# Aleksoid1978/VideoRenderer

Hardware: AMD Instinct MI355X
Metric: 4K frames/sec/GPU (P010->Lanczos3 2x->PQ-SDR->dither); % HBM roofline (higher is better)
Workload: dtype f32 (u16 in, u8 out)

## Files before the change

### include/mpcvr.h

```cpp
#ifndef MPCVR_H
#define MPCVR_H

#include <stddef.h>
#include <stdint.h>

#ifdef __cplusplus
extern "C" {
#endif

#define MPCVR_S_OK            0
#define MPCVR_S_FALSE         1
#define MPCVR_E_FAIL          ((int32_t)0x80004005)
#define MPCVR_E_POINTER       ((int32_t)0x80004003)
#define MPCVR_E_INVALIDARG    ((int32_t)0x80070057)
#define MPCVR_E_UNEXPECTED    ((int32_t)0x8000FFFF)
#define MPCVR_E_NOTIMPL       ((int32_t)0x80004001)
#define MPCVR_E_OUTOFMEMORY   ((int32_t)0x8007000E)
#define MPCVR_E_NOT_VALID_STATE ((int32_t)0x8007139F)

enum mpcvr_cformat {
    MPCVR_CF_NONE = 0,
    MPCVR_CF_NV12 = 1, MPCVR_CF_P010 = 2, MPCVR_CF_P016 = 3,
    MPCVR_CF_YUY2 = 4, MPCVR_CF_UYVY = 5,
    MPCVR_CF_P210 = 6, MPCVR_CF_P216 = 7,
// ... 95 lines not shown
typedef struct mpcvr_dovi_metadata {
    uint8_t  bl_bit_depth, coef_log2_denom;
    uint16_t source_max_pq;
    uint8_t  l1_present, l3_present;
    uint16_t l1_min_pq, l1_max_pq, l1_avg_pq, l3_min_pq_offset, l3_max_pq_offset, l3_avg_pq_offset;
    uint32_t n_l2;
    mpcvr_dovi_l2 l2[32];
    double   ycc_to_rgb_matrix[9], ycc_to_rgb_offset[3], rgb_to_lms_matrix[9];
    mpcvr_dovi_curve curves[3];
} mpcvr_dovi_metadata;
int32_t mpcvr_set_dovi_metadata(mpcvr_ctx *ctx, const mpcvr_dovi_metadata *md);

#define MPCVR_CORR_FIX_BT2020            1
#define MPCVR_CORR_FIX_YCGCO             2
#define MPCVR_CORR_FIXCONVERT_PQ_TO_SDR  3
#define MPCVR_CORR_FIXCONVERT_HLG_TO_SDR 4
#define MPCVR_CORR_CONVERT_PQ_TO_SDR     5
#define MPCVR_CORR_CONVERT_HLG_TO_PQ     6
int32_t mpcvr_correction_pass(int32_t kind, const void *src, int32_t src_pitch, int32_t src_fmt,
                              void *dst, int32_t dst_pitch, int32_t dst_fmt, int32_t w, int32_t h, int32_t sdr_nits, void *stream);
int32_t mpcvr_plan_correction_matrices(float fix_bt2020_16[16], float fix_ycgco_16[16], float gamut9[9]);

int32_t mpcvr_plan_encode(int32_t out_cformat, int32_t src_fmt, uint32_t extfmt, int32_t coef9[9], int32_t off3[3], int32_t *shift,
                          int32_t *siting, uint32_t *extfmt_out);
int32_t mpcvr_encode_pass(const void *src, int32_t src_pitch, int32_t src_fmt, int32_t w, int32_t h, int32_t out_cformat, uint32_t extfmt,
                          void *y_plane, int32_t y_pitch, void *uv_plane, int32_t uv_pitch, void *stream);
int32_t mpcvr_render_yuv(mpcvr_ctx *ctx, int32_t field, int32_t out_cformat, uint32_t extfmt, void *y_plane, int32_t y_pitch,
                         void *uv_plane, int32_t uv_pitch);

#define MPCVR_HIST_BINS 1024
int32_t mpcvr_measure_pass(const void *src, int32_t src_pitch, int32_t src_fmt, int32_t w, int32_t h,
                           const mpcvr_rect *rect, uint32_t *hist_dev, void *stream);
int32_t mpcvr_measure_backbuffer(mpcvr_ctx *ctx, uint32_t *hist_dev);
typedef struct mpcvr_light_level { uint64_t pixels; int32_t min_code, max_code; double max_nits, avg_nits; } mpcvr_light_level;
int32_t mpcvr_light_level_from_histogram(const uint32_t hist[MPCVR_HIST_BINS], int32_t src_fmt, mpcvr_light_level *out);
int32_t mpcvr_histogram_percentile(const uint32_t hist[MPCVR_HIST_BINS], uint32_t ppm, int32_t *code);

enum { MPCVR_TENSOR_F32 = 0, MPCVR_TENSOR_F16 = 1, MPCVR_TENSOR_BF16 = 2 };
enum { MPCVR_TENSOR_PLANAR = 0 , MPCVR_TENSOR_INTERLEAVED = 1  };
enum { MPCVR_TENSOR_RGB = 0, MPCVR_TENSOR_BGR = 1 };
typedef struct mpcvr_tensor_desc {
    int32_t dtype, layout, channel_order, reserved;
    int64_t row_pitch;
    int64_t plane_pitch;
    float   scale[3], bias[3];
} mpcvr_tensor_desc;
int32_t mpcvr_plan_tensor_value(int32_t dtype, int32_t src_fmt, uint32_t code, float scale, float bias, uint32_t *bits);
int32_t mpcvr_tensor_pass(const void *src, int32_t src_pitch, int32_t src_fmt, int32_t w, int32_t h, const mpcvr_tensor_desc *desc,
                          void *dst, void *stream);
int32_t mpcvr_render_tensor(mpcvr_ctx *ctx, int32_t field, const mpcvr_tensor_desc *desc, void *dst);

int32_t mpcvr_plan_sample_code(int32_t dtype, int32_t cformat, uint32_t element_bits, float scale, float bias, uint32_t *code);
int32_t mpcvr_sample_pass(const void *tensor, const mpcvr_tensor_desc *desc, int32_t w, int32_t h, int32_t cformat, void *sample,
                          int32_t pitch, void *stream);
int32_t mpcvr_copy_sample_tensor(mpcvr_ctx *ctx, const void *tensor, const mpcvr_tensor_desc *desc);

enum { MPCVR_DEINT_ADAPTIVE_EXT = 0, MPCVR_DEINT_ADAPTIVE_NOCHECK_EXT = 1 };
typedef struct mpcvr_deint_plane { size_t offset; int32_t pitch, comps, lines, bytes, cs, mask; } mpcvr_deint_plane;
int32_t mpcvr_plan_deint_planes(int32_t cformat, int32_t w, int32_t h, int32_t pitch, int32_t *planes, mpcvr_deint_plane out[3]);
int32_t mpcvr_deint_plane_host(const void *prev, const void *cur, const void *next, int64_t src_pitch, int32_t comps, int32_t lines,
                               int32_t bytes, int32_t cs, int32_t mask, int32_t keep, int32_t first, int32_t mode, void *dst, int64_t dst_pitch);
int32_t mpcvr_deint_pass(const void *prev, const void *cur, const void *next, int32_t cformat, int32_t w, int32_t h, int32_t pitch,
                         int32_t keep, int32_t first, int32_t mode, void *dst, int32_t dst_pitch, void *stream);
int32_t mpcvr_copy_sample_fields(mpcvr_ctx *ctx, const void *prev, const void *cur, const void *next, int32_t field_order, int32_t field, int32_t mode);

int32_t mpcvr_plan_lut3d_entries(const float *rgb, int32_t n, uint16_t *entries);
int32_t mpcvr_plan_lut3d_value(int32_t src_fmt, int32_t dst_fmt, const uint16_t *entries_host, int32_t n, uint32_t texel, uint32_t *out);
int32_t mpcvr_lut3d_pass(const void *src, int32_t src_pitch, int32_t src_fmt, int32_t w, int32_t h, const void *lut_dev, int32_t n,
                         void *dst, int32_t dst_pitch, int32_t dst_fmt, void *stream);
int32_t mpcvr_render_lut3d(mpcvr_ctx *ctx, int32_t field, const void *lut_dev, int32_t n, void *dst, int32_t dst_pitch, int32_t dst_fmt);

typedef struct mpcvr_deband_params {
    int32_t range;
    int32_t iterations;
    int32_t threshold;
    int32_t dither;
} mpcvr_deband_params;
int32_t mpcvr_deband_params_default(int32_t src_fmt, mpcvr_deband_params *params);
int32_t mpcvr_deband_host(const void *src_host, int64_t src_pitch, int32_t src_fmt, int32_t w, int32_t h, const mpcvr_deband_params *params,
                          uint32_t seed, void *dst_host, int64_t dst_pitch, int32_t dst_fmt);
int32_t mpcvr_plan_deband(int32_t src_fmt, const mpcvr_deband_params *params, int32_t w, int32_t h, int32_t *halo, int32_t *placement);
int32_t mpcvr_deband_pass(const void *src, int32_t src_pitch, int32_t src_fmt, int32_t w, int32_t h, const mpcvr_deband_params *params,
                          uint32_t seed, void *dst, int32_t dst_pitch, int32_t dst_fmt, void *stream);
int32_t mpcvr_render_deband(mpcvr_ctx *ctx, int32_t field, const mpcvr_deband_params *params, uint32_t seed, void *dst, int32_t dst_pitch, int32_t dst_fmt);

int32_t mpcvr_configure(mpcvr_ctx *ctx, const mpcvr_settings *settings);

int32_t mpcvr_set_procamp(mpcvr_ctx *ctx, uint32_t flags, float brightness, float contrast,
                          float hue, float saturation);

int32_t mpcvr_copy_sample(mpcvr_ctx *ctx, const void *data, int32_t pitch, int32_t mem_kind);

int32_t mpcvr_process(mpcvr_ctx *ctx, void *dst_dev, int32_t dst_pitch, const mpcvr_rect *src_rect,
                      const mpcvr_rect *dst_rect, int32_t second_field);

int32_t mpcvr_process_frames(mpcvr_ctx *ctx, int32_t n, const void *const *samples, int32_t pitch, int32_t mem_kind, void *const *dsts_dev, int32_t dst_pitch);

int32_t mpcvr_render(mpcvr_ctx *ctx, int32_t field);
int32_t mpcvr_get_backbuffer(mpcvr_ctx *ctx, void **dev_ptr, int32_t *pitch, int32_t *width, int32_t *height);

int32_t mpcvr_get_current_image(mpcvr_ctx *ctx, void *host_bgra, size_t *size);
int32_t mpcvr_get_displayed_image(mpcvr_ctx *ctx, void *host_pixels, size_t *size, int32_t deep_color, int32_t *width, int32_t *height, int32_t *bits_per_pixel);

int32_t mpcvr_flush(mpcvr_ctx *ctx);
int32_t mpcvr_reset(mpcvr_ctx *ctx);

int32_t mpcvr_process_batch(mpcvr_ctx *ctx, int32_t n, const void *const *srcs, void *const *dsts,
                            int32_t dst_pitch);
int32_t mpcvr_process_batch_dovi(mpcvr_ctx *ctx, int32_t n, const void *const *srcs, void *const *dsts,
                                 int32_t dst_pitch, const mpcvr_dovi_metadata *rpus);

#define MPCVR_BATCH_YUV_DEFAULT_BUDGET ((size_t)4 << 30)
int32_t mpcvr_plan_batch_yuv(int32_t window_w, int32_t window_h, int32_t n, size_t budget_bytes,
                             int32_t *surface_pitch, size_t *frame_stride, int32_t *frames_per_chunk, int32_t *chunks);
int32_t mpcvr_set_batch_yuv_budget(mpcvr_ctx *ctx, size_t bytes);
int32_t mpcvr_process_batch_yuv(mpcvr_ctx *ctx, int32_t n, const void *const *srcs, int32_t out_cformat, uint32_t extfmt,
                                void *const *y_planes, int32_t y_pitch, void *const *uv_planes, int32_t uv_pitch);
int32_t mpcvr_process_batch_yuv_stats(mpcvr_ctx *ctx, int32_t n, const void *const *srcs, int32_t out_cformat, uint32_t extfmt,
                                      void *const *y_planes, int32_t y_pitch, void *const *uv_planes, int32_t uv_pitch,
                                      uint32_t *hist_dev );
int32_t mpcvr_plan_batch_tensor(int32_t window_w, int32_t window_h, int32_t n, size_t budget_bytes,
                                int32_t *surface_pitch, size_t *frame_stride, int32_t *frames_per_chunk, int32_t *chunks);
int32_t mpcvr_process_batch_tensor(mpcvr_ctx *ctx, int32_t n, const void *const *srcs, const mpcvr_tensor_desc *desc, void *const *dsts);
int32_t mpcvr_plan_batch_from_tensors(int32_t pitch, int32_t h, int32_t n, size_t budget_bytes,
                                      size_t *frame_stride, int32_t *frames_per_chunk, int32_t *chunks);
int32_t mpcvr_process_batch_from_tensors(mpcvr_ctx *ctx, int32_t n, const void *const *tensors, const mpcvr_tensor_desc *desc,
                                         void *const *dsts, int32_t dst_pitch);
int32_t mpcvr_plan_batch_deint(int32_t pitch, int32_t lines, int32_t n_out, size_t budget_bytes,
                               size_t *frame_stride, int32_t *frames_per_chunk, int32_t *chunks);
int32_t mpcvr_process_batch_deint(mpcvr_ctx *ctx, int32_t n, const void *const *frames , int32_t field_order,
                                  int32_t fields_per_frame , int32_t mode, void *const *dsts ,
                                  int32_t dst_pitch);
int32_t mpcvr_plan_batch_lut3d(int32_t window_w, int32_t window_h, int32_t n, size_t budget_bytes,
                               int32_t *surface_pitch, size_t *frame_stride, int32_t *frames_per_chunk, int32_t *chunks);
int32_t mpcvr_process_batch_lut3d(mpcvr_ctx *ctx, int32_t n, const void *const *srcs, const void *lut_dev, int32_t lut_n,
                                  void *const *dsts, int32_t dst_pitch, int32_t dst_fmt);
int32_t mpcvr_plan_batch_deband(int32_t window_w, int32_t window_h, int32_t n, size_t budget_bytes,
                                int32_t *surface_pitch, size_t *frame_stride, int32_t *frames_per_chunk, int32_t *chunks);
int32_t mpcvr_process_batch_deband(mpcvr_ctx *ctx, int32_t n, const void *const *srcs, const mpcvr_deband_params *params, uint32_t seed,
                                   void *const *dsts, int32_t dst_pitch, int32_t dst_fmt);

int32_t mpcvr_get_param_blob(mpcvr_ctx *ctx, void *buf, size_t *size);
int32_t mpcvr_set_param_blob(mpcvr_ctx *ctx, const void *buf, size_t size);
int32_t mpcvr_broadcast_param_blob_begin(mpcvr_ctx *ctx, void *nccl_comm, int32_t root, int32_t rank);
int32_t mpcvr_broadcast_param_blob_end(mpcvr_ctx *ctx);
int32_t mpcvr_broadcast_param_blob(mpcvr_ctx *ctx, void *nccl_comm, int32_t root, int32_t rank);

int32_t mpcvr_get_color_matrix(mpcvr_ctx *ctx, float out12[12]);
int32_t mpcvr_get_extfmt(mpcvr_ctx *ctx, uint32_t *extfmt);
int32_t mpcvr_get_frame_bytes(mpcvr_ctx *ctx, size_t *bytes, int32_t *pitch);
int32_t mpcvr_get_fused_tables(mpcvr_ctx *ctx, void *buf, size_t *size);
int32_t mpcvr_get_path_info(mpcvr_ctx *ctx, char *buf, size_t buf_size);
int32_t mpcvr_get_last_batch_info(mpcvr_ctx *ctx, char *buf, size_t buf_size);
const char *mpcvr_last_error(mpcvr_ctx *ctx);
const char *mpcvr_version(void);

int32_t mpcvr_get_last_process_ms(mpcvr_ctx *ctx, float *ms);
int32_t mpcvr_get_last_timings(mpcvr_ctx *ctx, float *copy_host_ms, float *upload_ms, float *process_ms, float *readback_ms);

int32_t mpcvr_plan_frame_layout(int32_t cformat, int32_t width, int32_t height, int32_t *pitch, size_t *bytes);
int32_t mpcvr_plan_color_matrix(int32_t cformat, int32_t rect_w, int32_t rect_h, uint32_t extfmt,
                                float brightness, float contrast, float hue, float saturation,
                                float out12[12], uint32_t *extfmt_out);
int32_t mpcvr_plan_gamut_2020_to_709(float out9[9]);
int32_t mpcvr_plan_pq_lut(float lum_scale, float out4096[4096]);
int32_t mpcvr_plan_final_pass_multiplier(int32_t quant, int32_t maxv, uint32_t *multiplier);
int32_t mpcvr_plan_dovi(const mpcvr_dovi_metadata *md, int32_t display_nits, float *cb705, int32_t *has_mmr,
                        float lms9[9], float l2k[5], int32_t *l2_enabled, uint32_t l1_nits[3], int32_t *l1_present);
int32_t mpcvr_plan_upscale_weights(int32_t iUpscaling, float t, float w6[6]);
int32_t mpcvr_plan_axis_taps(int32_t kind, int32_t method, int32_t src_l, int32_t src_len, int32_t n_out,
                             int32_t tex_len, uint32_t flags, int32_t cap_taps, int32_t *idx, float *w,
                             float *wsum, int32_t *ntaps, int32_t *normalise);
int32_t mpcvr_plan_strip(int32_t kind_x, int32_t method_x, int32_t kind_y, int32_t method_y, int32_t src_w, int32_t src_h,
                         int32_t out_w, int32_t out_h, uint32_t flags, int32_t out8[8], int32_t *yrange, int32_t *xstrip,
                         int32_t *xi_t, float *xw_t, int32_t *yi, float *yw);
int32_t mpcvr_plan_period(int32_t method, int32_t src_w, int32_t src_h, int32_t out_w, int32_t out_h, uint32_t flags,
                          int32_t out6[6], int32_t *xi_t, float *xw_t, float *yw, int32_t *xstrip, int32_t *strip_w);
#define MPCVR_DRAW_TABLES_HEADER_WORDS 64
int32_t mpcvr_plan_draw_tables(const mpcvr_settings *s, int32_t cformat, int32_t src_w, int32_t src_h, const mpcvr_rect *src_rect,
                               const mpcvr_rect *video_rect, int32_t window_w, int32_t window_h, int32_t rotation, int32_t flip,
                               void *buf, size_t *size);
int32_t mpcvr_plan_hdr10_params(float min_mastering, float max_mastering, float max_cll, float max_fall, float display_max,
                                int32_t selection, uint32_t out6[6]);
int32_t mpcvr_plan_pq_eotf_table(float *out, int32_t capacity, int32_t *count);
int32_t mpcvr_plan_pq_eotf_lut(float out[4096]);
int32_t mpcvr_plan_describe(const mpcvr_settings *s, int32_t cformat, int32_t rect_w, int32_t rect_h,
                            const mpcvr_rect *video_rect, int32_t window_w, int32_t window_h,
                            char *buf, size_t buf_size);

int32_t mpcvr_bandwidth_probe(const void *src_dev, void *dst_dev, size_t src_bytes, int32_t fan, void *stream);
int32_t mpcvr_bandwidth_probe_up2x(int32_t mode, int32_t n, const void *const *srcs_dev, void *const *dsts_dev, int32_t src_w, int32_t src_h,
                                   int32_t seg_rows, int32_t strip_cols, void *stream);

int32_t mpcvr_eval_transcendental(int32_t fn, const float *x_dev, const float *y_dev, float *out_dev, size_t n, void *stream);
int32_t mpcvr_eval_dovi_tail(int32_t stage, const float *rgb_dev, float *out_dev, size_t n, const float lms9[9], const float l2k5[5], int32_t l2_enabled,
                             float lum_scale, void *stream);
int32_t mpcvr_eval_transcendental_host(int32_t fn, const float *x, const float *y, float *out, size_t n);

#ifdef __cplusplus
}
#endif
#endif
```

### videorenderer_amd/api.py

```python
import ctypes as C
import os
import sys

HERE = os.path.dirname(os.path.abspath(__file__))
LIB_PATH = os.path.join(HERE, "libmpcvr.so")

S_OK, S_FALSE = 0, 1
E_FAIL = -2147467259
E_POINTER = -2147467261
E_INVALIDARG = -2147024809
E_UNEXPECTED = -2147418113
E_NOTIMPL = -2147467263
E_OUTOFMEMORY = -2147024882
E_NOT_VALID_STATE = -2147019873

CF_NV12, CF_P010, CF_P016 = 1, 2, 3
CF_YUY2, CF_UYVY = 4, 5
CF_P210, CF_P216 = 6, 7
CF_Y210, CF_Y216, CF_V210, CF_AYUV, CF_Y410, CF_Y416 = 8, 9, 10, 11, 12, 13
CF_GBRP8, CF_GBRP10, CF_GBRP16 = 26, 27, 28
CF_Y8, CF_Y10, CF_Y16 = 37, 38, 39
CF_RGB24, CF_XRGB32, CF_ARGB32, CF_r210, CF_RGB48, CF_BGR48, CF_BGRA64, CF_B64A = 29, 30, 31, 32, 33, 34, 35, 36
CF_YV12, CF_YV16, CF_YV24 = 14, 15, 16
CF_YUV420P8, CF_YUV422P8, CF_YUV444P8 = 17, 18, 19
# ... 2 lines not shown
TEXFMT_AUTOINT, TEXFMT_8INT, TEXFMT_10INT, TEXFMT_16FLOAT = 0, 8, 10, 16
CHROMA_Nearest, CHROMA_Bilinear, CHROMA_CatmullRom = 0, 1, 2
UPSCALE_Nearest, UPSCALE_Mitchell, UPSCALE_CatmullRom, UPSCALE_Lanczos2, UPSCALE_Lanczos3, UPSCALE_Jinc2 = range(6)
UPSCALE_Spline36_EXT = 6
DOWNSCALE_Box, DOWNSCALE_Bilinear, DOWNSCALE_Hamming, DOWNSCALE_Bicubic, DOWNSCALE_BicubicSharp, DOWNSCALE_Lanczos = range(6)
OUT_BGRA8, OUT_RGB10A2 = 0, 1
DITHER_None, DITHER_Ordered, DITHER_ErrorDiffusion_EXT = 0, 1, 2
FLAG_LANCZOS3_FIXED, FLAG_NO_FUSED, FLAG_NO_LUT, FLAG_NO_FAST_CONVERT, FLAG_FUSED_VALU, FLAG_FUSED_MFMA, FLAG_NO_STRIP = 1, 2, 4, 8, 16, 32, 64
FLAG_NO_PERIOD = 128
FLAG_FORCE_PERIOD = 256
FLAG_NO_FRAME_LANES = 512
MEM_HOST, MEM_DEVICE, MEM_HOST_PINNED = 0, 1, 2
PROCAMP_BRIGHTNESS, PROCAMP_CONTRAST, PROCAMP_HUE, PROCAMP_SATURATION = 1, 2, 4, 8

CHROMA_LOC_MPEG1, CHROMA_LOC_MPEG2, CHROMA_LOC_COSITED = 1, 5, 7
RANGE_0_255, RANGE_16_235 = 1, 2
MATRIX_BT709, MATRIX_BT601, MATRIX_SMPTE240M, MATRIX_BT2020, MATRIX_YCGCO = 1, 2, 3, 4, 7
PRIM_BT709, PRIM_BT2020 = 2, 9
TRC_22, TRC_709, TRC_SRGB, TRC_PQ, TRC_HLG = 4, 5, 7, 15, 16


def make_extfmt(chroma=0, nominal_range=0, matrix=0, lighting=0, primaries=0, transfer=0, sample_format=0):
    return ((sample_format & 0xff) | ((chroma & 0xf) << 8) | ((nominal_range & 0x7) << 12) |
            ((matrix & 0x7) << 15) | ((lighting & 0xf) << 18) | ((primaries & 0x1f) << 22) |
            ((transfer & 0x1f) << 27))


class Settings(C.Structure):
    _fields_ = [("iTexFormat", C.c_int32), ("iChromaScaling", C.c_int32), ("iUpscaling", C.c_int32),
                ("iDownscaling", C.c_int32), ("bInterpolateAt50pct", C.c_int32), ("bUseDither", C.c_int32),
                ("bDeintBlend", C.c_int32), ("bConvertToSdr", C.c_int32), ("iSDRDisplayNits", C.c_int32),
                ("output_format", C.c_int32), ("flags", C.c_uint32)]

    def copy(self, **kw):
        s = Settings()
        C.memmove(C.byref(s), C.byref(self), C.sizeof(Settings))
        for k, v in kw.items():
            setattr(s, k, v)
        return s


class Rect(C.Structure):
    _fields_ = [("left", C.c_int32), ("top", C.c_int32), ("right", C.c_int32), ("bottom", C.c_int32)]


class DoviCurve(C.Structure):
    _fields_ = [
        ("num_pivots", C.c_uint8), ("mapping_idc", C.c_uint8 * 8), ("poly_order", C.c_uint8 * 8),
        ("mmr_order", C.c_uint8 * 8), ("pivots", C.c_uint16 * 9),
        ("poly_coef", (C.c_int64 * 3) * 8), ("mmr_constant", C.c_int64 * 8), ("mmr_coef", ((C.c_int64 * 7) * 3) * 8),
    ]


class DoviL2(C.Structure):
    _fields_ = [(n, C.c_uint16) for n in ("target_max_pq", "trim_slope", "trim_offset", "trim_power",
                                          "trim_chroma_weight", "trim_saturation_gain")]


class DoviMetadata(C.Structure):
    _fields_ = [
        ("bl_bit_depth", C.c_uint8), ("coef_log2_denom", C.c_uint8), ("source_max_pq", C.c_uint16),
        ("l1_present", C.c_uint8), ("l3_present", C.c_uint8),
        ("l1_min_pq", C.c_uint16), ("l1_max_pq", C.c_uint16), ("l1_avg_pq", C.c_uint16),
        ("l3_min_pq_offset", C.c_uint16), ("l3_max_pq_offset", C.c_uint16), ("l3_avg_pq_offset", C.c_uint16),
        ("n_l2", C.c_uint32), ("l2", DoviL2 * 32),
        ("ycc_to_rgb_matrix", C.c_double * 9), ("ycc_to_rgb_offset", C.c_double * 3), ("rgb_to_lms_matrix", C.c_double * 9),
        ("curves", DoviCurve * 3),
    ]

    @classmethod
    def from_dict(cls, d):
        st = cls()
        for k in ("bl_bit_depth", "coef_log2_denom", "source_max_pq", "l1_present", "l3_present", "l1_min_pq",
                  "l1_max_pq", "l1_avg_pq", "l3_min_pq_offset", "l3_max_pq_offset", "l3_avg_pq_offset"):
            setattr(st, k, int(d.get(k, 0)))
        l2 = d.get("l2", [])
        st.n_l2 = len(l2)
        for i, e in enumerate(l2[:32]):
            for k, v in e.items():
                setattr(st.l2[i], k, int(v))
        for k in ("ycc_to_rgb_matrix", "ycc_to_rgb_offset", "rgb_to_lms_matrix"):
            getattr(st, k)[:] = [float(x) for x in d[k]]
        for c, cv in enumerate(d["curves"]):
            o = st.curves[c]
            o.num_pivots = cv.get("num_pivots", len(cv["pivots"]))
            o.pivots[:len(cv["pivots"])] = [int(x) for x in cv["pivots"]]
            for i, piece in enumerate(cv["pieces"]):
                if "poly" in piece:
                    o.mapping_idc[i] = piece.get("idc", 0)
                    o.poly_order[i] = piece["order"]
                    for j, x in enumerate(piece["poly"]):
                        o.poly_coef[i][j] = int(x)
                else:
                    o.mapping_idc[i] = piece.get("idc", 1)
                    o.mmr_order[i] = piece["order"]
                    o.mmr_constant[i] = int(piece["constant"])
                    for j, row in enumerate(piece["mmr"]):
                        for k, x in enumerate(row):
                            o.mmr_coef[i][j][k] = int(x)
        return st


HIST_BINS = 1024


class LightLevel(C.Structure):
    _fields_ = [("pixels", C.c_uint64), ("min_code", C.c_int32), ("max_code", C.c_int32), ("max_nits", C.c_double), ("avg_nits", C.c_double)]


TENSOR_F32, TENSOR_F16, TENSOR_BF16 = 0, 1, 2
TENSOR_PLANAR, TENSOR_INTERLEAVED = 0, 1
TENSOR_RGB, TENSOR_BGR = 0, 1


class TensorDesc(C.Structure):
    _fields_ = [("dtype", C.c_int32), ("layout", C.c_int32), ("channel_order", C.c_int32), ("reserved", C.c_int32),
                ("row_pitch", C.c_int64), ("plane_pitch", C.c_int64), ("scale", C.c_float * 3), ("bias", C.c_float * 3)]


def tensor_desc(dtype, layout, row_pitch, plane_pitch=0, scale=(1 / 255,) * 3, bias=(0,) * 3, channel_order=TENSOR_RGB):
    d = TensorDesc(int(dtype), int(layout), int(channel_order), 0, int(row_pitch), int(plane_pitch))
    for k in range(3):
        d.scale[k], d.bias[k] = float(scale[k]), float(bias[k])
    return d


DEINT_ADAPTIVE_EXT, DEINT_ADAPTIVE_NOCHECK_EXT = 0, 1
FIELD_ORDER_TFF, FIELD_ORDER_BFF = 1, 2


class DeintPlane(C.Structure):
    _fields_ = [("offset", C.c_size_t), ("pitch", C.c_int32), ("comps", C.c_int32), ("lines", C.c_int32), ("bytes", C.c_int32),
                ("cs", C.c_int32), ("mask", C.c_int32)]


class DebandParams(C.Structure):
    _fields_ = [("range", C.c_int32), ("iterations", C.c_int32), ("threshold", C.c_int32), ("dither", C.c_int32)]


class MpcvrError(RuntimeError):
    def __init__(self, hr, msg):
        super().__init__(f"HRESULT 0x{hr & 0xffffffff:08X}: {msg}")
        self.hr = hr


EXPORTS = [
    "mpcvr_settings_default", "mpcvr_create", "mpcvr_destroy", "mpcvr_set_stream", "mpcvr_synchronize",
    "mpcvr_set_input", "mpcvr_set_video_rect", "mpcvr_set_window_rect", "mpcvr_set_rotation", "mpcvr_set_error_diffusion_patience", "mpcvr_set_flip", "mpcvr_set_sample_format", "mpcvr_set_hdr_output", "mpcvr_set_hdr_metadata",
    "mpcvr_set_dovi_metadata", "mpcvr_plan_dovi", "mpcvr_correction_pass", "mpcvr_plan_correction_matrices",
    "mpcvr_configure", "mpcvr_set_procamp", "mpcvr_copy_sample", "mpcvr_process", "mpcvr_process_frames", "mpcvr_render",
    "mpcvr_get_backbuffer", "mpcvr_get_current_image", "mpcvr_get_displayed_image", "mpcvr_flush", "mpcvr_reset", "mpcvr_process_batch", "mpcvr_process_batch_dovi",
    "mpcvr_get_param_blob", "mpcvr_set_param_blob", "mpcvr_broadcast_param_blob_begin", "mpcvr_broadcast_param_blob_end",
    "mpcvr_broadcast_param_blob", "mpcvr_get_color_matrix", "mpcvr_get_extfmt",
    "mpcvr_get_frame_bytes", "mpcvr_get_fused_tables", "mpcvr_get_path_info", "mpcvr_get_last_batch_info", "mpcvr_last_error", "mpcvr_version",
    "mpcvr_get_last_process_ms", "mpcvr_get_last_timings",
    "mpcvr_plan_frame_layout", "mpcvr_plan_color_matrix", "mpcvr_plan_gamut_2020_to_709", "mpcvr_plan_pq_lut",
    "mpcvr_plan_upscale_weights", "mpcvr_plan_axis_taps", "mpcvr_plan_describe", "mpcvr_plan_final_pass_multiplier",
    "mpcvr_plan_strip", "mpcvr_plan_pq_eotf_table", "mpcvr_plan_pq_eotf_lut", "mpcvr_bandwidth_probe", "mpcvr_plan_period", "mpcvr_plan_hdr10_params", "mpcvr_plan_draw_tables",
    "mpcvr_eval_transcendental", "mpcvr_eval_transcendental_host", "mpcvr_bandwidth_probe_up2x", "mpcvr_eval_dovi_tail",
    "mpcvr_plan_encode", "mpcvr_encode_pass", "mpcvr_render_yuv",
    "mpcvr_plan_batch_yuv", "mpcvr_set_batch_yuv_budget", "mpcvr_process_batch_yuv",
    "mpcvr_measure_pass", "mpcvr_measure_backbuffer", "mpcvr_process_batch_yuv_stats",
    "mpcvr_light_level_from_histogram", "mpcvr_histogram_percentile",
    "mpcvr_plan_tensor_value", "mpcvr_tensor_pass", "mpcvr_render_tensor", "mpcvr_plan_batch_tensor", "mpcvr_process_batch_tensor",
    "mpcvr_plan_sample_code", "mpcvr_sample_pass", "mpcvr_copy_sample_tensor", "mpcvr_plan_batch_from_tensors", "mpcvr_process_batch_from_tensors",
    "mpcvr_plan_deint_planes", "mpcvr_deint_plane_host", "mpcvr_deint_pass", "mpcvr_copy_sample_fields", "mpcvr_plan_batch_deint", "mpcvr_process_batch_deint",
    "mpcvr_plan_lut3d_entries", "mpcvr_plan_lut3d_value", "mpcvr_lut3d_pass", "mpcvr_render_lut3d", "mpcvr_plan_batch_lut3d", "mpcvr_process_batch_lut3d",
    "mpcvr_deband_params_default", "mpcvr_deband_host", "mpcvr_plan_deband", "mpcvr_deband_pass", "mpcvr_render_deband", "mpcvr_plan_batch_deband", "mpcvr_process_batch_deband",
]

_lib = None


def load_library():
    global _lib
    if _lib is not None:
        return _lib
    lib_path = os.environ.get("MPCVR_LIB") or LIB_PATH
    if not os.path.exists(lib_path):
        raise RuntimeError(f"{lib_path} is missing: run `python -m videorenderer_amd.build` "
                           "(or __graft_entry__.build()); there is no CPU fallback")
    if "torch" not in sys.modules and not os.environ.get("MPCVR_NO_TORCH_IMPORT"):
        try:
            import importlib.util
            if importlib.util.find_spec("torch") is not None:
                import torch
        except Exception:
            pass
    L = C.CDLL(lib_path)
    vp, i32, u32, f = C.c_void_p, C.c_int32, C.c_uint32, C.c_float
    P = C.POINTER
    sig = {
        "mpcvr_settings_default": [P(Settings)],
        "mpcvr_create": [P(Settings), i32, P(vp)],
        "mpcvr_destroy": [vp],
        "mpcvr_set_stream": [vp, vp],
        "mpcvr_synchronize": [vp],
        "mpcvr_set_input": [vp, i32, i32, i32, i32, P(Rect), u32],
        "mpcvr_set_video_rect": [vp, P(Rect)],
        "mpcvr_set_window_rect": [vp, P(Rect)],
        "mpcvr_set_rotation": [vp, i32],
        "mpcvr_set_error_diffusion_patience": [vp, i32],
        "mpcvr_set_flip": [vp, i32],
        "mpcvr_set_sample_format": [vp, i32],
        "mpcvr_set_hdr_output": [vp, i32, i32, f],
        "mpcvr_set_hdr_metadata": [vp, f, f, f, f],
        "mpcvr_set_dovi_metadata": [vp, P(DoviMetadata)],
        "mpcvr_plan_dovi": [P(DoviMetadata), i32, P(f), P(i32), P(f), P(f), P(i32), P(u32), P(i32)],
        "mpcvr_correction_pass": [i32, vp, i32, i32, vp, i32, i32, i32, i32, i32, vp],
        "mpcvr_plan_correction_matrices": [P(f), P(f), P(f)],
        "mpcvr_configure": [vp, P(Settings)],
        "mpcvr_set_procamp": [vp, u32, f, f, f, f],
        "mpcvr_copy_sample": [vp, vp, i32, i32],
        "mpcvr_process": [vp, vp, i32, P(Rect), P(Rect), i32],
        "mpcvr_render": [vp, i32],
        "mpcvr_process_frames": [vp, i32, P(C.c_void_p), i32, i32, P(C.c_void_p), i32],
        "mpcvr_get_backbuffer": [vp, P(vp), P(i32), P(i32), P(i32)],
        "mpcvr_get_displayed_image": [vp, C.c_void_p, P(C.c_size_t), i32, P(i32), P(i32), P(i32)],
        "mpcvr_get_current_image": [vp, vp, P(C.c_size_t)],
        "mpcvr_flush": [vp],
        "mpcvr_reset": [vp],
        "mpcvr_process_batch": [vp, i32, P(vp), P(vp), i32],
        "mpcvr_process_batch_dovi": [vp, i32, P(vp), P(vp), i32, P(DoviMetadata)],
        "mpcvr_get_param_blob": [vp, vp, P(C.c_size_t)],
        "mpcvr_set_param_blob": [vp, vp, C.c_size_t],
        "mpcvr_broadcast_param_blob_begin": [vp, vp, i32, i32],
        "mpcvr_broadcast_param_blob_end": [vp],
        "mpcvr_broadcast_param_blob": [vp, vp, i32, i32],
        "mpcvr_get_color_matrix": [vp, P(f)],
        "mpcvr_get_extfmt": [vp, P(u32)],
        "mpcvr_get_frame_bytes": [vp, P(C.c_size_t), P(i32)],
        "mpcvr_get_fused_tables": [vp, vp, P(C.c_size_t)],
        "mpcvr_get_path_info": [vp, C.c_char_p, C.c_size_t],
        "mpcvr_get_last_batch_info": [vp, C.c_char_p, C.c_size_t],
        "mpcvr_get_last_process_ms": [vp, P(f)],
        "mpcvr_get_last_timings": [vp, P(f), P(f), P(f), P(f)],
        "mpcvr_plan_frame_layout": [i32, i32, i32, P(i32), P(C.c_size_t)],
        "mpcvr_plan_color_matrix": [i32, i32, i32, u32, f, f, f, f, P(f), P(u32)],
        "mpcvr_plan_gamut_2020_to_709": [P(f)],
        "mpcvr_plan_pq_lut": [f, P(f)],
        "mpcvr_plan_final_pass_multiplier": [i32, i32, P(u32)],
        "mpcvr_plan_upscale_weights": [i32, f, P(f)],
        "mpcvr_plan_axis_taps": [i32, i32, i32, i32, i32, i32, u32, i32, P(i32), P(f), P(f), P(i32), P(i32)],
        "mpcvr_plan_strip": [i32, i32, i32, i32, i32, i32, i32, i32, u32, P(i32), P(i32), P(i32), P(i32), P(f), P(i32), P(f)],
        "mpcvr_plan_hdr10_params": [f, f, f, f, f, i32, P(u32)],
        "mpcvr_plan_period": [i32, i32, i32, i32, i32, u32, P(i32), P(i32), P(f), P(f), P(i32), P(i32)],
        "mpcvr_plan_pq_eotf_table": [P(f), i32, P(i32)],
        "mpcvr_plan_pq_eotf_lut": [P(f)],
        "mpcvr_bandwidth_probe": [C.c_void_p, C.c_void_p, C.c_size_t, i32, C.c_void_p],
        "mpcvr_bandwidth_probe_up2x": [i32, i32, P(C.c_void_p), P(C.c_void_p), i32, i32, i32, i32, C.c_void_p],
        "mpcvr_eval_transcendental": [i32, C.c_void_p, C.c_void_p, C.c_void_p, C.c_size_t, C.c_void_p],
        "mpcvr_eval_dovi_tail": [i32, C.c_void_p, C.c_void_p, C.c_size_t, P(f), P(f), i32, f, C.c_void_p],
        "mpcvr_eval_transcendental_host": [i32, C.c_void_p, C.c_void_p, C.c_void_p, C.c_size_t],
        "mpcvr_plan_describe": [P(Settings), i32, i32, i32, P(Rect), i32, i32, C.c_char_p, C.c_size_t],
        "mpcvr_plan_draw_tables": [P(Settings), i32, i32, i32, P(Rect), P(Rect), i32, i32, i32, i32, C.c_void_p, P(C.c_size_t)],
        "mpcvr_plan_encode": [i32, i32, u32, P(i32), P(i32), P(i32), P(i32), P(u32)],
        "mpcvr_encode_pass": [vp, i32, i32, i32, i32, i32, u32, vp, i32, vp, i32, vp],
        "mpcvr_render_yuv": [vp, i32, i32, u32, vp, i32, vp, i32],
        "mpcvr_plan_batch_yuv": [i32, i32, i32, C.c_size_t, P(i32), P(C.c_size_t), P(i32), P(i32)],
        "mpcvr_set_batch_yuv_budget": [vp, C.c_size_t],
        "mpcvr_process_batch_yuv": [vp, i32, P(vp), i32, u32, P(vp), i32, P(vp), i32],
        "mpcvr_measure_pass": [vp, i32, i32, i32, i32, P(Rect), vp, vp],
        "mpcvr_measure_backbuffer": [vp, vp],
        "mpcvr_process_batch_yuv_stats": [vp, i32, P(vp), i32, u32, P(vp), i32, P(vp), i32, vp],
        "mpcvr_light_level_from_histogram": [vp, i32, P(LightLevel)],
        "mpcvr_histogram_percentile": [vp, u32, P(i32)],
        "mpcvr_plan_tensor_value": [i32, i32, u32, f, f, P(u32)],
        "mpcvr_tensor_pass": [vp, i32, i32, i32, i32, P(TensorDesc), vp, vp],
        "mpcvr_render_tensor": [vp, i32, P(TensorDesc), vp],
        "mpcvr_plan_batch_tensor": [i32, i32, i32, C.c_size_t, P(i32), P(C.c_size_t), P(i32), P(i32)],
        "mpcvr_process_batch_tensor": [vp, i32, P(vp), P(TensorDesc), P(vp)],
        "mpcvr_plan_sample_code": [i32, i32, u32, f, f, P(u32)],
        "mpcvr_sample_pass": [vp, P(TensorDesc), i32, i32, i32, vp, i32, vp],
        "mpcvr_copy_sample_tensor": [vp, vp, P(TensorDesc)],
        "mpcvr_plan_batch_from_tensors": [i32, i32, i32, C.c_size_t, P(C.c_size_t), P(i32), P(i32)],
        "mpcvr_process_batch_from_tensors": [vp, i32, P(vp), P(TensorDesc), P(vp), i32],
        "mpcvr_plan_deint_planes": [i32, i32, i32, i32, P(i32), P(DeintPlane)],
        "mpcvr_deint_plane_host": [vp, vp, vp, C.c_int64, i32, i32, i32, i32, i32, i32, i32, i32, vp, C.c_int64],
        "mpcvr_deint_pass": [vp, vp, vp, i32, i32, i32, i32, i32, i32, i32, vp, i32, vp],
        "mpcvr_copy_sample_fields": [vp, vp, vp, vp, i32, i32, i32],
        "mpcvr_plan_batch_deint": [i32, i32, i32, C.c_size_t, P(C.c_size_t), P(i32), P(i32)],
        "mpcvr_process_batch_deint": [vp, i32, P(vp), i32, i32, i32, P(vp), i32],
        "mpcvr_plan_lut3d_entries": [vp, i32, vp],
        "mpcvr_plan_lut3d_value": [i32, i32, vp, i32, u32, P(u32)],
        "mpcvr_lut3d_pass": [vp, i32, i32, i32, i32, vp, i32, vp, i32, i32, vp],
        "mpcvr_render_lut3d": [vp, i32, vp, i32, vp, i32, i32],
        "mpcvr_plan_batch_lut3d": [i32, i32, i32, C.c_size_t, P(i32), P(C.c_size_t), P(i32), P(i32)],
        "mpcvr_process_batch_lut3d": [vp, i32, P(vp), vp, i32, P(vp), i32, i32],
        "mpcvr_deband_params_default": [i32, P(DebandParams)],
        "mpcvr_deband_host": [vp, C.c_int64, i32, i32, i32, P(DebandParams), u32, vp, C.c_int64, i32],
        "mpcvr_plan_deband": [i32, P(DebandParams), i32, i32, P(i32), P(i32)],
        "mpcvr_deband_pass": [vp, i32, i32, i32, i32, P(DebandParams), u32, vp, i32, i32, vp],
        "mpcvr_render_deband": [vp, i32, P(DebandParams), u32, vp, i32, i32],
        "mpcvr_plan_batch_deband": [i32, i32, i32, C.c_size_t, P(i32), P(C.c_size_t), P(i32), P(i32)],
        "mpcvr_process_batch_deband": [vp, i32, P(vp), P(DebandParams), u32, P(vp), i32, i32],
    }
    for name, args in sig.items():
        if lib_path != LIB_PATH and not hasattr(L, name):
            continue
        fn = getattr(L, name)
        fn.argtypes = args
        fn.restype = i32
    L.mpcvr_last_error.argtypes = [vp]
    L.mpcvr_last_error.restype = C.c_char_p
    L.mpcvr_version.argtypes = []
    L.mpcvr_version.restype = C.c_char_p
    _lib = L
    return L


def default_settings(**kw):
    s = Settings()
    load_library().mpcvr_settings_default(C.byref(s))
    for k, v in kw.items():
        setattr(s, k, v)
    return s


def plan_frame_layout(cformat, width, height):
    pitch, nbytes = C.c_int32(), C.c_size_t()
    hr = load_library().mpcvr_plan_frame_layout(cformat, width, height, C.byref(pitch), C.byref(nbytes))
    if hr < 0:
        raise MpcvrError(hr, "mpcvr_plan_frame_layout")
    return nbytes.value, pitch.value


def plan_color_matrix(cformat, rect_w, rect_h, extfmt=0, brightness=0.0, contrast=1.0, hue=0.0, saturation=1.0):
    out = (C.c_float * 12)()
    ex = C.c_uint32()
    hr = load_library().mpcvr_plan_color_matrix(cformat, rect_w, rect_h, extfmt, brightness, contrast, hue,
                                                saturation, out, C.byref(ex))
    if hr < 0:
        raise MpcvrError(hr, "mpcvr_plan_color_matrix")
    return list(out), ex.value


def plan_gamut_2020_to_709():
    out = (C.c_float * 9)()
    load_library().mpcvr_plan_gamut_2020_to_709(out)
    return list(out)


def plan_pq_lut(lum_scale):
    out = (C.c_float * 4096)()
    load_library().mpcvr_plan_pq_lut(lum_scale, out)
    return list(out)


def plan_final_pass_multiplier(quant, maxv):
    m = C.c_uint32(0)
    load_library().mpcvr_plan_final_pass_multiplier(quant, maxv, C.byref(m))
    return m.value


def plan_dovi(md, display_nits=1000):
    st = md if isinstance(md, DoviMetadata) else DoviMetadata.from_dict(md)
    cb = (C.c_float * 705)(); lms = (C.c_float * 9)(); l2k = (C.c_float * 5)(); l1 = (C.c_uint32 * 3)()
    has_mmr, l2on, l1on = C.c_int32(0), C.c_int32(0), C.c_int32(0)
    hr = load_library().mpcvr_plan_dovi(C.byref(st), int(display_nits), cb, C.byref(has_mmr), lms, l2k, C.byref(l2on),
                                        l1, C.byref(l1on))
    if hr:
        raise MpcvrError(hr, "mpcvr_plan_dovi")
    import numpy as np
    return dict(cb=np.array(cb, dtype=np.float32).reshape(3, 235), has_mmr=has_mmr.value,
                lms=np.array(lms, dtype=np.float32), l2k=np.array(l2k, dtype=np.float32), l2_enabled=l2on.value,
                l1_nits=np.array(l1, dtype=np.uint32), l1_present=l1on.value)


CORR_FIX_BT2020, CORR_FIX_YCGCO, CORR_FIXCONVERT_PQ_TO_SDR, CORR_FIXCONVERT_HLG_TO_SDR, CORR_CONVERT_PQ_TO_SDR, CORR_CONVERT_HLG_TO_PQ = range(1, 7)


def plan_correction_matrices():
    a, b, g = (C.c_float * 16)(), (C.c_float * 16)(), (C.c_float * 9)()
    hr = load_library().mpcvr_plan_correction_matrices(a, b, g)
    if hr:
        raise MpcvrError(hr, "mpcvr_plan_correction_matrices")
    return list(a), list(b), list(g)


def correction_pass(kind, src, src_pitch, src_fmt, dst, dst_pitch, dst_fmt, w, h, sdr_nits=125, stream=None):
    hr = load_library().mpcvr_correction_pass(int(kind), C.c_void_p(_ptr(src)), int(src_pitch), int(src_fmt), C.c_void_p(_ptr(dst)),
                                              int(dst_pitch), int(dst_fmt), int(w), int(h), int(sdr_nits),
                                              C.c_void_p(stream) if stream else None)
    if hr:
        raise MpcvrError(hr, "mpcvr_correction_pass")


def plan_encode(out_cformat, src_fmt, extfmt=0):
    import numpy as np
    coef, off = (C.c_int32 * 9)(), (C.c_int32 * 3)()
    shift, siting, ex = C.c_int32(), C.c_int32(), C.c_uint32()
    hr = load_library().mpcvr_plan_encode(int(out_cformat), int(src_fmt), int(extfmt), coef, off, C.byref(shift), C.byref(siting), C.byref(ex))
    if hr:
        raise MpcvrError(hr, "mpcvr_plan_encode")
    return dict(coef=np.array(coef, dtype=np.int32).reshape(3, 3), off=np.array(off, dtype=np.int32), shift=shift.value,
                siting=siting.value, extfmt=ex.value)


def encode_pass(src, src_pitch, src_fmt, w, h, out_cformat, extfmt, y_plane, y_pitch, uv_plane, uv_pitch, stream=None):
    hr = load_library().mpcvr_encode_pass(C.c_void_p(_ptr(src)), int(src_pitch), int(src_fmt), int(w), int(h), int(out_cformat), int(extfmt),
                                          C.c_void_p(_ptr(y_plane)), int(y_pitch), C.c_void_p(_ptr(uv_plane)), int(uv_pitch),
                                          C.c_void_p(stream) if stream else None)
    if hr:
        raise MpcvrError(hr, "mpcvr_encode_pass")


def measure_pass(src, src_pitch, src_fmt, w, h, hist, rect=None, stream=None):
    r = Rect(*[int(v) for v in rect]) if rect is not None else None
    hr = load_library().mpcvr_measure_pass(C.c_void_p(_ptr(src)), int(src_pitch), int(src_fmt), int(w), int(h), C.byref(r) if r is not None else None,
                                           C.c_void_p(_ptr(hist)), C.c_void_p(stream) if stream else None)
    if hr:
        raise MpcvrError(hr, "mpcvr_measure_pass")


def _host_hist(hist):
    import numpy as np
    h = np.ascontiguousarray(hist, dtype=np.uint32).reshape(-1)
    if h.size != HIST_BINS:
        raise ValueError("a histogram has %d bins" % HIST_BINS)
    return h


def light_level_from_histogram(hist, src_fmt):
    h = _host_hist(hist)
    out = LightLevel()
    hr = load_library().mpcvr_light_level_from_histogram(C.c_void_p(h.ctypes.data), int(src_fmt), C.byref(out))
    if hr:
        raise MpcvrError(hr, "mpcvr_light_level_from_histogram")
    return dict(pixels=out.pixels, min_code=out.min_code, max_code=out.max_code, max_nits=out.max_nits, avg_nits=out.avg_nits)


def histogram_percentile(hist, ppm):
    h = _host_hist(hist)
    code = C.c_int32()
    hr = load_library().mpcvr_histogram_percentile(C.c_void_p(h.ctypes.data), int(ppm), C.byref(code))
    if hr:
        raise MpcvrError(hr, "mpcvr_histogram_percentile")
    return code.value


def plan_tensor_value(dtype, src_fmt, code, scale, bias):
    bits = C.c_uint32()
    hr = load_library().mpcvr_plan_tensor_value(int(dtype), int(src_fmt), int(code), float(scale), float(bias), C.byref(bits))
    if hr:
        raise MpcvrError(hr, "mpcvr_plan_tensor_value")
    return bits.value


def tensor_pass(src, src_pitch, src_fmt, w, h, desc, dst, stream=None):
    hr = load_library().mpcvr_tensor_pass(C.c_void_p(_ptr(src)), int(src_pitch), int(src_fmt), int(w), int(h),
                                          C.byref(desc) if desc is not None else None, C.c_void_p(_ptr(dst)), C.c_void_p(stream) if stream else None)
    if hr:
        raise MpcvrError(hr, "mpcvr_tensor_pass")


def plan_batch_tensor(window_w, window_h, n, budget_bytes=0):
    pitch, fpc, chunks, stride = C.c_int32(), C.c_int32(), C.c_int32(), C.c_size_t()
    hr = load_library().mpcvr_plan_batch_tensor(int(window_w), int(window_h), int(n), int(budget_bytes), C.byref(pitch), C.byref(stride), C.byref(fpc), C.byref(chunks))
    if hr:
        raise MpcvrError(hr, "mpcvr_plan_batch_tensor")
    return dict(surface_pitch=pitch.value, frame_stride=stride.value, frames_per_chunk=fpc.value, chunks=chunks.value)


def plan_lut3d_entries(rgb, n):
    import numpy as np
    n = int(n)
    rgb = np.ascontiguousarray(rgb, dtype=np.float32).reshape(-1, 3)
    if rgb.shape[0] != n ** 3:
        raise ValueError("a table of size %d takes %d triplets, not %d" % (n, n ** 3, rgb.shape[0]))
    out = np.empty((rgb.shape[0], 4), dtype=np.uint16)
    hr = load_library().mpcvr_plan_lut3d_entries(C.c_void_p(rgb.ctypes.data), n, C.c_void_p(out.ctypes.data))
    if hr != S_OK:
        raise MpcvrError(hr, "mpcvr_plan_lut3d_entries")
    return out


def plan_lut3d_value(src_fmt, dst_fmt, entries, n, texel):
    import numpy as np
    entries = np.ascontiguousarray(entries, dtype=np.uint16)
# ... 582 lines not shown
    def GetCurentImage(self):
        import numpy as np
        size = C.c_size_t(0)
        self._check(self._L.mpcvr_get_current_image(self._ctx, None, C.byref(size)))
        buf = np.empty(size.value, dtype=np.uint8)
        self._check(self._L.mpcvr_get_current_image(self._ctx, C.c_void_p(buf.ctypes.data), C.byref(size)))
        return buf

    def GetDisplayedImage(self, deep_color=False):
        import numpy as np
        size, w, h, bits = C.c_size_t(0), C.c_int32(), C.c_int32(), C.c_int32()
        self._check(self._L.mpcvr_get_displayed_image(self._ctx, None, C.byref(size), int(deep_color), C.byref(w), C.byref(h), C.byref(bits)))
        buf = np.empty(size.value, dtype=np.uint8)
        self._check(self._L.mpcvr_get_displayed_image(self._ctx, C.c_void_p(buf.ctypes.data), C.byref(size), int(deep_color), C.byref(w), C.byref(h), C.byref(bits)))
        return buf, w.value, h.value, bits.value

    def CopySampleTensor(self, t, scale=(255.0,) * 3, bias=(0,) * 3, channel_order="rgb"):
        d, w, h = _frame_tensor_desc(t, scale, bias, channel_order)
        if not t.is_cuda:
            raise ValueError("a device tensor")
        self._keep = (t, d)
        return self._check(self._L.mpcvr_copy_sample_tensor(self._ctx, C.c_void_p(t.data_ptr()), C.byref(d)))

    def ProcessBatchFromTensors(self, ts, dsts, rt_pitch, scale=(255.0,) * 3, bias=(0,) * 3, channel_order="rgb"):
        frames = [ts[i] for i in range(len(ts))]
        n = len(frames)
        if n < 1 or n != len(dsts):
            raise ValueError("as many tensors as render targets, at least one")
        d, w, h = _frame_tensor_desc(frames[0], scale, bias, channel_order)
        for t in frames:
            if not t.is_cuda or t.dtype != frames[0].dtype or tuple(t.shape) != tuple(frames[0].shape) or t.stride() != frames[0].stride():
                raise ValueError("every frame a device tensor of one dtype, shape and strides")
        arr = C.c_void_p * n
        keep = (arr(*[t.data_ptr() for t in frames]), arr(*[_ptr(x) for x in dsts]), d, (ts, dsts))
        self._keep = keep
        return self._check(self._L.mpcvr_process_batch_from_tensors(self._ctx, n, keep[0], C.byref(d), keep[1], int(rt_pitch)))

    def CopySampleFields(self, prev, cur, nxt, field_order, field, mode=DEINT_ADAPTIVE_EXT):
        self._keep = (prev, cur, nxt)
        return self._check(self._L.mpcvr_copy_sample_fields(self._ctx, C.c_void_p(_ptr(prev)), C.c_void_p(_ptr(cur)), C.c_void_p(_ptr(nxt)),
                                                            int(field_order), int(field), int(mode)))

    def ProcessBatchDeint(self, frames, dsts, rt_pitch, field_order, fields_per_frame=2, mode=DEINT_ADAPTIVE_EXT):
        n = len(frames) - 2
        if n < 1 or len(dsts) != n * fields_per_frame:
            raise ValueError("n + 2 samples for n * fields_per_frame render targets, n at least one")
        keep = ((C.c_void_p * (n + 2))(*[_ptr(x) for x in frames]), (C.c_void_p * len(dsts))(*[_ptr(x) for x in dsts]), (frames, dsts))
        self._keep = keep
        return self._check(self._L.mpcvr_process_batch_deint(self._ctx, n, keep[0], int(field_order), int(fields_per_frame), int(mode), keep[1], int(rt_pitch)))

    def ProcessBatch(self, srcs, dsts, rt_pitch):
        if isinstance(srcs, PreparedBatch):
            return self._check(self._L.mpcvr_process_batch(self._ctx, srcs.n, srcs.sa, srcs.da, rt_pitch))
        b = self.PrepareBatch(srcs, dsts)
        self._keep = b
        return self._check(self._L.mpcvr_process_batch(self._ctx, b.n, b.sa, b.da, rt_pitch))

    def SetBatchYuvBudget(self, nbytes):
        return self._check(self._L.mpcvr_set_batch_yuv_budget(self._ctx, int(nbytes)))

    def ProcessBatchYuv(self, srcs, out_cformat, extfmt, y_planes, y_pitch, uv_planes, uv_pitch):
        n = len(srcs)
        assert n == len(y_planes) == len(uv_planes) and n > 0
        arr = C.c_void_p * n
        keep = (arr(*[_ptr(s) for s in srcs]), arr(*[_ptr(p) for p in y_planes]), arr(*[_ptr(p) for p in uv_planes]), (srcs, y_planes, uv_planes))
        self._keep = keep
        return self._check(self._L.mpcvr_process_batch_yuv(self._ctx, n, keep[0], int(out_cformat), int(extfmt), keep[1], int(y_pitch), keep[2], int(uv_pitch)))

    def ProcessBatchYuvStats(self, srcs, out_cformat, extfmt, y_planes, y_pitch, uv_planes, uv_pitch, hist):
        n = len(srcs)
        assert n == len(y_planes) == len(uv_planes) and n > 0
        arr = C.c_void_p * n
        keep = (arr(*[_ptr(s) for s in srcs]), arr(*[_ptr(p) for p in y_planes]), arr(*[_ptr(p) for p in uv_planes]), (srcs, y_planes, uv_planes, hist))
        self._keep = keep
        return self._check(self._L.mpcvr_process_batch_yuv_stats(self._ctx, n, keep[0], int(out_cformat), int(extfmt), keep[1], int(y_pitch), keep[2],
                                                                 int(uv_pitch), C.c_void_p(_ptr(hist))))

    def ProcessBatchDovi(self, srcs, dsts, rt_pitch, rpus):
        b = srcs if isinstance(srcs, PreparedBatch) else self.PrepareBatch(srcs, dsts)
        self._keep = b
        assert len(rpus) == b.n
        arr = (DoviMetadata * b.n)(*[m if isinstance(m, DoviMetadata) else DoviMetadata.from_dict(m) for m in rpus])
        return self._check(self._L.mpcvr_process_batch_dovi(self._ctx, b.n, b.sa, b.da, rt_pitch, arr))

    @staticmethod
    def PrepareBatch(srcs, dsts):
        n = len(srcs)
        assert n == len(dsts) and n > 0
        return PreparedBatch(n, (C.c_void_p * n)(*[_ptr(s) for s in srcs]), (C.c_void_p * n)(*[_ptr(d) for d in dsts]), (srcs, dsts))

    def Flush(self):
        return self._check(self._L.mpcvr_flush(self._ctx))

    def Reset(self):
        return self._check(self._L.mpcvr_reset(self._ctx))

    def GetParamBlob(self):
        size = C.c_size_t(0)
        self._check(self._L.mpcvr_get_param_blob(self._ctx, None, C.byref(size)))
        buf = (C.c_uint8 * size.value)()
        self._check(self._L.mpcvr_get_param_blob(self._ctx, buf, C.byref(size)))
        return bytes(buf)

    def GetFusedTables(self):
        size = C.c_size_t(0)
        self._check(self._L.mpcvr_get_fused_tables(self._ctx, None, C.byref(size)))
        buf = (C.c_uint8 * size.value)()
        self._check(self._L.mpcvr_get_fused_tables(self._ctx, buf, C.byref(size)))
        return bytes(buf)

    def SetParamBlob(self, blob):
        buf = (C.c_uint8 * len(blob)).from_buffer_copy(blob)
        return self._check(self._L.mpcvr_set_param_blob(self._ctx, buf, len(blob)))

    def GetColorMatrix(self):
        out = (C.c_float * 12)()
        self._check(self._L.mpcvr_get_color_matrix(self._ctx, out))
        return list(out)

    def GetExtFmt(self):
        v = C.c_uint32()
        self._check(self._L.mpcvr_get_extfmt(self._ctx, C.byref(v)))
        return v.value

    def GetFrameBytes(self):
        n, p = C.c_size_t(), C.c_int32()
        self._check(self._L.mpcvr_get_frame_bytes(self._ctx, C.byref(n), C.byref(p)))
        return n.value, p.value

    def GetVPInfo(self):
        buf = C.create_string_buffer(256)
        self._check(self._L.mpcvr_get_path_info(self._ctx, buf, 256))
        return buf.value.decode()

    def GetLastBatchInfo(self):
        buf = C.create_string_buffer(512)
        self._check(self._L.mpcvr_get_last_batch_info(self._ctx, buf, 512))
        d = dict(kv.split("=", 1) for kv in buf.value.decode().split(";"))
        out = dict(frames=int(d["frames"]), launches=int(d["launches"]), dovi_runs=d.get("dovi_runs", ""), lane=int(d.get("lane", -1)), waits=int(d.get("waits", 0)), uploads=int(d.get("uploads", -1)))
        if "yuv_chunks" in d:
            out.update(yuv_chunks=int(d["yuv_chunks"]), yuv_lanes=[int(x) for x in d["yuv_lanes"].split(",") if x])
        if "tensor_chunks" in d:
            out.update(tensor_chunks=int(d["tensor_chunks"]), tensor_lanes=[int(x) for x in d["tensor_lanes"].split(",") if x])
        if "sample_chunks" in d:
            out.update(sample_chunks=int(d["sample_chunks"]))
        if "deint_chunks" in d:
            out.update(deint_chunks=int(d["deint_chunks"]))
        if "lut3d_chunks" in d:
            out.update(lut3d_chunks=int(d["lut3d_chunks"]), lut3d_lanes=[int(x) for x in d["lut3d_lanes"].split(",") if x], lut3d_table=d.get("lut3d_table", ""))
        if "deband_chunks" in d:
            out.update(deband_chunks=int(d["deband_chunks"]), deband_lanes=[int(x) for x in d["deband_lanes"].split(",") if x], deband_taps=d.get("deband_taps", ""))
        return out

    def GetLastProcessMs(self):
        ms = C.c_float()
        self._check(self._L.mpcvr_get_last_process_ms(self._ctx, C.byref(ms)))
        return ms.value

    def GetLastTimings(self):
        v = [C.c_float(-1.0) for _ in range(4)]
        self._check(self._L.mpcvr_get_last_timings(self._ctx, *(C.byref(x) for x in v)))
        return dict(zip(("copy_host_ms", "upload_ms", "process_ms", "readback_ms"), (x.value for x in v)))
```

### videorenderer_amd/build.py

```python
import os
import shutil
import subprocess
import sys

HERE = os.path.dirname(os.path.abspath(__file__))
CSRC = os.path.join(HERE, "csrc")
OUT = os.path.join(HERE, "libmpcvr.so")
BUILD = os.path.join(HERE, "_build")
ARCH = "gfx950"

SOURCES = [
    ("vp_plan.cpp", ["-ffp-contract=off"]),
    ("vp_plan_tables.cpp", ["-ffp-contract=off"]),
    ("vp_dovi.cpp", ["-ffp-contract=off", "-std=c++20"]),
    ("hip_video_processor.cpp", []),
    ("hip_video_processor_ext.cpp", []),
    ("vp_lanes.cpp", []),
    ("mpcvr_capi.cpp", []),
    ("vp_kernels.hip", ["-ffp-contract=off", "-DMPCVR_EXACT_FP"]),
    ("vp_fused.hip", []),
    ("vp_fused_up2x_nt4.hip", []),
    ("vp_fused_up2x_nt5.hip", []),
    ("vp_fused_up2x_nt6.hip", []),
    ("vp_fused_strip.hip", []),
    ("vp_fused_strip_nt4.hip", []),
    ("vp_fused_strip_nt6.hip", []),
    ("vp_fused_strip_nt8.hip", []),
    ("vp_fused_strip_nt16.hip", []),
    ("vp_fused_period.hip", []),
    ("vp_fused_period_4_3.hip", []),
    ("vp_fused_period_3_2.hip", []),
    ("vp_fused_period_2_3.hip", []),
    ("vp_fused_period_1_2.hip", []),
    ("vp_fused_period_3_1.hip", []),
    ("vp_jinc.hip", []),
    ("vp_fused_jinc.hip", []),
    ("vp_errdiff.hip", []),
    ("vp_encode.hip", []),
    ("vp_measure.hip", []),
    ("vp_tensor.hip", []),
    ("vp_tensor_in.hip", []),
    ("vp_deint.hip", []),
    ("vp_lut3d.hip", []),
    ("vp_deband.hip", []),
    ("vp_probe.hip", []),
]


def _hipcc():
    for cand in (os.environ.get("HIPCC"), shutil.which("hipcc"), "/opt/rocm/bin/hipcc"):
        if cand and os.path.exists(cand):
            return cand
    raise RuntimeError("hipcc not found")


def _newer(src, dst):
    return not os.path.exists(dst) or os.path.getmtime(src) > os.path.getmtime(dst)


def _project_deps(path, seen=None):
    import re
    seen = set() if seen is None else seen
    try:
        text = open(path, encoding="utf-8", errors="replace").read()
    except OSError:
        return seen
    for inc in re.findall(r'^\s*#\s*include\s+"([^"]+)"', text, flags=re.M):
        dep = os.path.normpath(os.path.join(os.path.dirname(path), inc))
        if os.path.exists(dep) and dep not in seen:
            seen.add(dep)
            _project_deps(dep, seen)
    return seen


def build(force=False, verbose=False):
    hipcc = _hipcc()
    os.makedirs(BUILD, exist_ok=True)
    objs = []
    common = ["-O3", "-std=c++17", "-fPIC", f"--offload-arch={ARCH}", "-Wall", "-Wno-unused-function"]
    jobs = []
    for name, extra in SOURCES:
        src = os.path.join(CSRC, name)
        obj = os.path.join(BUILD, name + ".o")
        objs.append(obj)
        if force or _newer(src, obj) or any(_newer(h, obj) for h in _project_deps(src)):
            cmd = [hipcc, "-x", "hip", "-c", src, "-o", obj] + common + extra
            if verbose:
                print(" ".join(cmd), file=sys.stderr)
            jobs.append(cmd)
    if jobs:
        from concurrent.futures import ThreadPoolExecutor
        with ThreadPoolExecutor(max_workers=min(len(jobs), os.cpu_count() or 1)) as pool:
            for rc in pool.map(lambda c: subprocess.run(c).returncode, jobs):
                if rc != 0:
                    raise subprocess.CalledProcessError(rc, "hipcc")
    if force or any(_newer(o, OUT) for o in objs):
        cmd = [hipcc, "-shared", "-fPIC", f"--offload-arch={ARCH}", "-o", OUT] + objs
        if verbose:
            print(" ".join(cmd), file=sys.stderr)
        subprocess.check_call(cmd)
    return OUT


if __name__ == "__main__":
    print(build(force="--force" in sys.argv, verbose=True))
```

### videorenderer_amd/csrc/hip_video_processor.cpp

```cpp
#include "hip_video_processor.h"

#include <hip/hip_runtime.h>

#include <dlfcn.h>

#include <algorithm>
#include <cstdlib>

#include <cmath>
#include <chrono>
#include <cstdio>
#include <cstring>

namespace mpcvr {

static const uint16_t kDitherTable[1024] = {
#include "dither_table.inc"
};

struct ParamBlob {
    uint32_t magic;
    uint32_t version;
    float cm[12];
    float lum_scale;
// ... 730 lines not shown
    }
    if (u.inFlight && (hr = CheckHip(hipEventSynchronize(u.consumedRecorded ? u.consumed : u.uploaded), "upload slot wait"))) return hr;
    return CheckHip(u.dev.CheckCreate(bytes), "upload buffer");
}

HRESULT CHipVideoProcessor::PublishUploadSlot(int si, hipStream_t recordedOn)
{
    UploadSlot &u = m_up[si];
    HRESULT hr;
    if ((hr = CheckHip(hipEventRecord(u.uploaded, recordedOn), "upload event"))) return hr;
    if (recordedOn != m_stream && (hr = CheckHip(hipStreamWaitEvent(m_stream, u.uploaded, 0), "stream wait"))) return hr;
    u.inFlight = true; u.consumedRecorded = false;
    m_curSlot = si;
    return PrepareSample((const uint8_t *)u.dev.ptr, &m_curSample);
}

void CHipVideoProcessor::MarkConsumed()
{
    if (m_curSlot < 0) return;
    UploadSlot &u = m_up[m_curSlot];
    if (!u.consumed) return;
    hipStream_t const s = m_lastRun ? m_lastRun : m_stream;
    if (u.consumedRecorded && u.consumedOn != s) (void)hipStreamWaitEvent(s, u.consumed, 0);
    if (hipEventRecord(u.consumed, s) == hipSuccess) { u.consumedRecorded = true; u.consumedOn = s; }
}

FusedParams CHipVideoProcessor::ConvertOutputParams(const uint8_t *sample, void *out, int inflight) const
{
    const int pitch = (int)(m_srcRectWidth * SurfBytesPerPixel(m_plan.internal_fmt));
    FusedParams fp{};
    FillFusedParams(sample, out, pitch, &fp, inflight);
    fp.store = MakeStore(out, pitch, m_plan.internal_fmt, false);
    fp.dst_aligned16 = 1;
    fp.exact_convert = 1;
    return fp;
}

HRESULT CHipVideoProcessor::ConvertColorPass(const uint8_t *sample, const RunOn &on)
{
    ConvertParams P;
    FillConvertParams(sample, &P);
    Surface out{m_TexConvertOutput.ptr, (int)(m_srcRectWidth * SurfBytesPerPixel(m_plan.internal_fmt)),
                m_srcRectWidth, m_srcRectHeight, m_plan.internal_fmt};
    if (!(m_cfg.flags & MPCVR_FLAG_NO_FUSED)) {
        const FusedParams fp = ConvertOutputParams(sample, out.ptr, on.inflight);
        if (ConvertBlocksSupported(fp, false))
            return CheckHip(LaunchConvertBlocks(fp, LaunchFrames::One(sample, out.ptr), on.stream), "k_convert_blocks");
    }
    return CheckHip(LaunchConvert(P, out, on.stream, (m_cfg.flags & MPCVR_FLAG_NO_FUSED) != 0), "k_convert");
}

HRESULT CHipVideoProcessor::ResizeShaderPass(const uint8_t *sample, void *rt, int rtPitch, const DrawFrames &df, const RunOn &on)
{
    const int w1 = m_srcRectWidth, h1 = m_srcRectHeight, w2 = m_videoRect.Width(), h2 = m_videoRect.Height();
    Surface conv{df.conv, (int)(w1 * SurfBytesPerPixel(m_plan.internal_fmt)), w1, h1, m_plan.internal_fmt};
    if (!m_plan.convert)
        conv = Surface{(void *)sample, TexPitch(), m_srcWidth, m_srcHeight, RgbTexFmt(*m_srcParams)};
    const StoreParams final = MakeStore(rt, rtPitch, m_plan.swap_fmt, true);
    Surface post{df.post, (int)(w2 * SurfBytesPerPixel(m_plan.internal_fmt)), w2, h2, m_plan.internal_fmt};
    const StoreParams last = m_plan.hdr_tonemap ? MakeStore(post.ptr, post.pitch, m_plan.internal_fmt, false) : final;
    ResizeBatch b; b.n = df.n; b.in_stride = df.convStride; b.frames = df.lastTab; b.dst_aligned8 = df.aligned;
    HRESULT hr = MPCVR_S_OK;
    bool drawn = true;
    const bool plain = (m_cfg.flags & MPCVR_FLAG_NO_FUSED) != 0;
    const bool jfast = !(m_cfg.flags & (MPCVR_FLAG_NO_FUSED | MPCVR_FLAG_NO_FAST_CONVERT));
    FusedStripParams ssp{};
    const bool surfStrip = m_stripSurf && FillStripSurfParams(conv, last, &ssp);
    if (m_stripSurf) m_fusedAside = !surfStrip;
    if (surfStrip) {
        ssp.surf_stride = df.convStride;
        if (df.lastTab) ssp.fp.dst_aligned16 = df.aligned;
        const LaunchFrames frames = df.lastTab ? LaunchFrames::Device(df.lastTab, df.n) : LaunchFrames::One((const uint8_t *)conv.ptr, last.dst);
        hr = CheckHip(LaunchFusedStrip(ssp, frames, on.stream), "k_fused_strip<surface>");
    } else if (m_plan.two_pass && !plain && !m_tables.firstJinc && !m_tables.secondJinc && m_tables.firstAxis == 0 && !m_tables.firstSwap &&
        Resize2DSupported(conv, m_tapsX, m_tapsY, last)) {
        hr = CheckHip(LaunchResize2D(conv, m_tapsX, m_tapsY, m_otherX, m_plan.mid_h, w2, h2, last, on.stream, &b), "k_resize_2d");
    } else if (m_plan.two_pass) {
        Surface mid{df.mid, w2 * 8, w2, m_plan.mid_h, SF_RGBA16F};
        StoreParams st = MakeStore(mid.ptr, mid.pitch, SF_RGBA16F, false);
        ResizeBatch b1; b1.n = df.n; b1.in_stride = df.convStride; b1.dst_stride = df.midStride;
        if (m_tables.firstJinc) hr = CheckHip(LaunchJinc2(conv, m_tables.firstCoords, w2, m_plan.mid_h, st, on.stream, m_jincFirstTab, jfast, &b1, m_jincFirstCtr), "k_jinc2");
        else hr = CheckHip(LaunchResize(m_tables.firstAxis, m_tables.firstSwap, conv, m_tapsX, m_otherX, w2, m_plan.mid_h, st, on.stream, plain, &b1), "k_resize<first>");
        if (hr) return hr;
        ResizeBatch b2 = b; b2.in_stride = df.midStride;
        if (m_tables.secondJinc) hr = CheckHip(LaunchJinc2(mid, m_tables.secondCoords, w2, h2, last, on.stream, m_jincSecondTab, jfast, &b2, m_jincSecondCtr), "k_jinc2");
        else hr = CheckHip(LaunchResize(1, false, mid, m_tapsY, m_otherY, w2, h2, last, on.stream, plain, &b2), "k_resize<Y>");
    } else if (m_plan.one_pass) {
        if (m_tables.firstJinc) hr = CheckHip(LaunchJinc2(conv, m_tables.firstCoords, w2, h2, last, on.stream, m_jincFirstTab, jfast, &b, m_jincFirstCtr), "k_jinc2");
        else hr = CheckHip(LaunchResize(m_tables.firstAxis, m_tables.firstSwap, conv, m_tapsX, m_otherX, w2, h2, last, on.stream, plain, &b), "k_resize<one>");
    } else {
        drawn = false;
        if (!m_plan.convert) {
            const int bpp = conv.fmt == SF_RGBA16 ? 8 : 4;
            conv.ptr = (uint8_t *)conv.ptr + (size_t)m_srcRect.top * conv.pitch + (size_t)m_srcRect.left * bpp;
            conv.w = w1; conv.h = h1;
        }
        if (!m_plan.hdr_tonemap) {
            StoreParams direct = final;
            if (!m_plan.convert) direct.mid_fmt = conv.fmt;
            return CheckHip(LaunchCopy(conv, w2, h2, direct, on.stream), "k_copy");
        }
    }
    if (hr || !m_plan.hdr_tonemap) return hr;
    ResizeBatch tb; tb.n = df.n; tb.in_stride = drawn ? df.postStride : df.convStride; tb.frames = df.rtTab;
    return CheckHip(LaunchHdr10ToneMap(drawn ? post : conv, m_hdrTm, w2, h2, final, on.stream, &tb), "k_hdr10_tonemap");
}

bool CHipVideoProcessor::FillStripTables(const StoreParams &store, int perForce, FusedStripParams *sp) const
{
    sp->fp.store = store;
    sp->ran_period = &m_stripRan;
    if (!m_tables.stripPlanned) return false;
    const int32_t *tab = (const int32_t *)m_stripTab.ptr;
    const size_t *so = m_tables.stripPack.stripOff, *po = m_tables.stripPack.periodOff;
    sp->yrange = tab + so[0]; sp->xstrip = tab + so[1];
    sp->xi_t = tab + so[2]; sp->xw_t = tab + so[3];
    sp->yi = tab + so[4]; sp->yw = tab + so[5];
    sp->out_w = m_videoRect.Width(); sp->out_h = m_videoRect.Height();
    sp->nt = m_tables.strip.nt; sp->pxl = m_tables.strip.pxl; sp->strip_w = m_tables.strip.strip_w; sp->ring = m_tables.strip.ring; sp->acols = m_tables.strip.acols;
    sp->per_P = 0;
    if (m_tables.period.P && !(m_cfg.flags & MPCVR_FLAG_NO_PERIOD)) {
        sp->per_P = m_tables.period.P; sp->per_Q = m_tables.period.Q; sp->per_nt = m_tables.period.nt; sp->per_acols = m_tables.period.acols; sp->per_strip_w = m_tables.period.strip_w; sp->per_own = m_tables.period.own; sp->per_force = perForce;
        sp->per_xi_t = tab + po[0]; sp->per_xw_t = tab + po[1]; sp->per_yw = tab + po[2]; sp->per_xstrip = tab + po[3];
    }
    return FusedStripSupported(*sp) && FusedStripLdsBytes(*sp) <= DeviceLdsLimit();
}

bool CHipVideoProcessor::FillStripParams(const uint8_t *sample, void *dst, int dstPitch, const StoreParams &store, FusedStripParams *sp, int inflight) const
{
    FillFusedParams(sample, dst, dstPitch, &sp->fp, inflight);
    sp->fp.dst_aligned16 = (((uintptr_t)dst) & 7) == 0;
    return FillStripTables(store, (m_cfg.flags & MPCVR_FLAG_FORCE_PERIOD) ? 1 : 0, sp);
}

bool CHipVideoProcessor::FillStripSurfParams(const Surface &src, const StoreParams &store, FusedStripParams *sp) const
{
    *sp = FusedStripParams{};
    sp->fp.dst_aligned16 = (((uintptr_t)store.dst) & 7) == 0;
    sp->surface_mode = 1;
    sp->surf = src;
    sp->other = m_tapsX.other_identity ? nullptr : m_otherX;
    sp->mid_h = m_plan.mid_h;
    return FillStripTables(store, 1, sp);
}

HRESULT CHipVideoProcessor::ProcessOne(const uint8_t *sample, void *rt, int rtPitch, const RunOn &on)
{
    HRESULT hr;
    m_fusedAside = false;
    if (m_plan.fused_up2x) {
        FusedParams fp{};
        FillFusedParams(sample, rt, rtPitch, &fp, on.inflight);
        if (StoreRowsFit32(fp.store, fp.out_h))
            return CheckHip(LaunchFusedUp2x(fp, LaunchFrames::One(sample, rt), on.stream), "k_fused_up2x");
        m_fusedAside = true;
    }
    if (m_strip) {
        const int w2 = m_videoRect.Width(), h2 = m_videoRect.Height();
        Surface post{m_TexPost.ptr, (int)(w2 * SurfBytesPerPixel(m_plan.internal_fmt)), w2, h2, m_plan.internal_fmt};
        const StoreParams final = MakeStore(rt, rtPitch, m_plan.swap_fmt, true);
        const StoreParams last = m_plan.hdr_tonemap ? MakeStore(post.ptr, post.pitch, m_plan.internal_fmt, false) : final;
        FusedStripParams sp{};
        if (FillStripParams(sample, last.dst, last.dst_pitch, last, &sp, on.inflight)) {
            if ((hr = CheckHip(LaunchFusedStrip(sp, LaunchFrames::One(sample, last.dst), on.stream), "k_fused_strip"))) return hr;
            if (!m_plan.hdr_tonemap) return MPCVR_S_OK;
            return CheckHip(LaunchHdr10ToneMap(post, m_hdrTm, w2, h2, final, on.stream), "k_hdr10_tonemap");
        }
        m_fusedAside = true;
    }
    if (m_plan.direct_convert) {
        FusedParams fp{};
        FillFusedParams(sample, rt, rtPitch, &fp, on.inflight);
        if (ConvertBlocksSupported(fp, true))
            return CheckHip(LaunchConvertBlocks(fp, LaunchFrames::One(sample, rt), on.stream), "k_convert_blocks");
        ConvertParams P;
        FillConvertParams(sample, &P);
        return CheckHip(LaunchConvertDirect(P, MakeStore(rt, rtPitch, m_plan.swap_fmt, true), on.stream), "k_convert_direct");
    }
    if (m_plan.convert && (hr = ConvertColorPass(sample, on))) return hr;
    return ResizeShaderPass(sample, rt, rtPitch, DrawFrames{m_TexConvertOutput.ptr, m_TexResize.ptr, m_TexPost.ptr}, on);
}

HRESULT CHipVideoProcessor::CheckTargetLayout(int n, void *const *dsts, int rtPitch)
{
    if (rtPitch & 3) return Fail(MPCVR_E_INVALIDARG, "render-target pitch is not a multiple of 4");
    for (int i = 0; i < n; i++)
        if ((uintptr_t)dsts[i] & 3) return Fail(MPCVR_E_INVALIDARG, "render target does not start on a multiple of 4 bytes");
    return MPCVR_S_OK;
}

HRESULT CHipVideoProcessor::ProcessFrame(void *pRenderTarget, int rtPitch, const CRect *srcRect, const CRect *dstRect, size_t clearBytes, bool onContextStream)
{
    if (!m_bInit || !m_srcParams) return Fail(MPCVR_E_NOT_VALID_STATE, "InitMediaType has not been called");
    if (!pRenderTarget) return Fail(MPCVR_E_POINTER, "null render target");
    if (HRESULT bad = CheckTargetLayout(1, &pRenderTarget, rtPitch)) return bad;
    if (!m_curSample) return Fail(MPCVR_E_NOT_VALID_STATE, "no sample: call CopySample first");
    if (srcRect && !srcRect->IsRectNull() && *srcRect != m_srcRect)
        return Fail(MPCVR_E_INVALIDARG, "src_rect must equal the input's source rect");
    (void)hipSetDevice(m_device);
    HRESULT hr;
    if (dstRect && !dstRect->IsRectNull()) { if ((hr = SetVideoRect(*dstRect))) return hr; }
    if (rtPitch < m_windowRect.Width() * 4) return Fail(MPCVR_E_INVALIDARG, "render-target pitch smaller than a row");
    if (m_planDirty && (hr = UpdatePlan())) return hr;
    const RtSpan span = TargetSpan(pRenderTarget, rtPitch);
    const bool rows32 = StoreRowsFit32(MakeStore(pRenderTarget, rtPitch, m_plan.swap_fmt, true), m_videoRect.Height());
    const int lane = (onContextStream || !rows32 || !FrameLanesUsable()) ? -1 : m_lanes.PickFrameLane(span);
    const RunOn on{lane >= 0 ? m_lanes.Stream(lane) : m_stream, lane >= 0 ? FrameLanes::Count() : 1};
    if (lane >= 0) {
        m_lanes.LaneWaitsForStream(lane, m_stream);
        if (m_curSlot >= 0 && m_up[m_curSlot].uploaded) (void)hipStreamWaitEvent(on.stream, m_up[m_curSlot].uploaded, 0);
    } else OrderOnContextStream();
    if (clearBytes) (void)hipMemsetAsync(m_BackBuffer.ptr, 0, clearBytes, on.stream);
    static const int every = [] { const char *e = std::getenv("MPCVR_LANE_TIMING_EVERY"); const int v = e && *e ? std::atoi(e) : 8; return v < 1 ? 1 : v; }();
    const bool timeIt = lane < 0 || every == 1 || (m_laneFrames++ % (unsigned)every) == 0 || !m_timed;
    if (timeIt) (void)hipEventRecord(m_evStart, on.stream);
    if (m_plan.errdiff) {
        if (!(hr = PrepareErrDiff(1)) && !(hr = ProcessOne(m_curSample, m_edBase, m_edPitch, on)))
            hr = ErrDiffPass(LaunchFrames::One(m_edBase, pRenderTarget), rtPitch, on.stream);
    } else
        hr = ProcessOne(m_curSample, pRenderTarget, rtPitch, on);
    if (timeIt) (void)hipEventRecord(m_evStop, on.stream);
    m_lastRun = on.stream;
    MarkConsumed();
    if (lane >= 0) m_lanes.NoteLaneFrame(lane, span);
    m_timed = true;
    return hr;
}

HRESULT CHipVideoProcessor::CheckBatchArgs(int n, const void *const *srcs, void *const *dsts, int rtPitch)
{
    if (!m_bInit || !m_srcParams) return Fail(MPCVR_E_NOT_VALID_STATE, "InitMediaType has not been called");
    if (n <= 0 || !srcs || !dsts) return Fail(MPCVR_E_INVALIDARG, "empty batch");
    if (rtPitch < m_windowRect.Width() * 4) return Fail(MPCVR_E_INVALIDARG, "render-target pitch smaller than a row");
    if (HRESULT bad = CheckTargetLayout(n, dsts, rtPitch)) return bad;
    for (int i = 0; i < n; i++)
        if (!srcs[i] || !dsts[i]) return Fail(MPCVR_E_POINTER, "null frame in batch");
    return MPCVR_S_OK;
}

HRESULT CHipVideoProcessor::ProcessBatch(int n, const void *const *srcs, void *const *dsts, int rtPitch)
{
    const BatchRecord record(*this, n);
    if (HRESULT bad = CheckBatchArgs(n, srcs, dsts, rtPitch)) return bad;
    BatchRun run{n, srcs, dsts, rtPitch};
    return RunBatch(run);
}

HRESULT CHipVideoProcessor::RunBatch(BatchRun &run)
{
    (void)hipSetDevice(m_device);
    if (HRESULT bad = m_planDirty ? UpdatePlan() : MPCVR_S_OK) return bad;
    return m_plan.errdiff ? ProcessBatchErrDiff(run) : ProcessBatchRoutes(run);
}

HRESULT CHipVideoProcessor::ProcessBatchRoutes(BatchRun &run)
{
    BatchRoutePlan rp = ClassifyBatch(run);
    std::vector<RtSpan> targets((size_t)run.n);
    for (int i = 0; i < run.n; i++) targets[i] = TargetSpan(run.dsts[i], run.rtPitch);
    const int bl = PlaceBatch(rp, run, std::move(targets));
    const HRESULT hr = RunBatchRoute(rp, run);
    NoteBatchQueued(bl);
    return hr;
}

int CHipVideoProcessor::PlaceBatch(const BatchRoutePlan &rp, BatchRun &run, std::vector<RtSpan> &&writes)
{
    const int bl = BatchLaneEligible(rp, run) ? m_lanes.PickBatchLane(std::move(writes), &m_lastBatchWaits) : -1;
    run.on = RunOn{bl >= 0 ? m_lanes.Stream(bl) : m_stream};
    if (bl >= 0) {
        m_lastBatchLane = bl;
        m_lanes.LaneWaitsForStream(bl, m_stream);
    } else OrderOnContextStream();
    return bl;
}

bool CHipVideoProcessor::BatchLaneEligible(const BatchRoutePlan &rp, const BatchRun &run) const
{
    static const bool lanesOff = [] { const char *e = std::getenv("MPCVR_NO_BATCH_LANES"); return e && *e && *e != '0'; }();
    const bool laneRoute = rp.route == BatchRoute::FusedUp2x || rp.route == BatchRoute::Strip || rp.route == BatchRoute::DirectConvert;
    return laneRoute && !rp.repackSlot && !lanesOff && m_ownStream && run.n >= 2 && !m_doviValid && !run.dvFrames && !m_plan.errdiff && !m_plan.hdr_tonemap &&
           !(m_cfg.flags & (MPCVR_FLAG_NO_FRAME_LANES | MPCVR_FLAG_NO_FUSED | MPCVR_FLAG_NO_FAST_CONVERT | MPCVR_FLAG_NO_STRIP));
}

CHipVideoProcessor::BatchRoutePlan CHipVideoProcessor::ClassifyBatch(const BatchRun &run) const
{
    const int n = run.n, rtPitch = run.rtPitch;
    const void *const *const srcs = run.srcs;
    void *const *const dsts = run.dsts;
    BatchRoutePlan rp;
    const bool v210 = m_srcParams->cformat == MPCVR_CF_V210, rgb = m_srcParams->layout == LAY_RGB;
    const bool fast = !(m_cfg.flags & (MPCVR_FLAG_NO_FUSED | MPCVR_FLAG_NO_FAST_CONVERT)), fastStrip = fast && !(m_cfg.flags & MPCVR_FLAG_NO_STRIP);
    const size_t slot = ((size_t)TexPitch() * m_srcHeight + 255) & ~(size_t)255;
    if (v210 && n > 1 && fast && slot * (size_t)n <= ((size_t)1 << 30)) rp.repackSlot = slot;
    for (int i = 0; i < n; i++) {
        if (!rp.repackSlot && ((uintptr_t)srcs[i] & 15) != 0) rp.src16 = false;
        if (!rp.repackSlot && ((uintptr_t)srcs[i] & 3) != 0) rp.src4 = false;
        if (((uintptr_t)dsts[i] & 15) != 0) rp.aligned = false;
        if (((uintptr_t)dsts[i] & 7) != 0) rp.aligned8 = false;
    }
    if ((v210 && !rp.repackSlot) || rgb) rp.src4 = false;
    const uint8_t *const sample0 = rp.repackSlot ? nullptr : (const uint8_t *)srcs[0];
    const StoreParams target = MakeStore(dsts[0], rtPitch, m_plan.swap_fmt, true);
    FusedStripParams sp{};
    const bool up2x = m_plan.fused_up2x && StoreRowsFit32(target, m_videoRect.Height());
    const bool strip = m_strip && !up2x && !m_plan.hdr_tonemap && rp.src4 && !run.dvFrames && FillStripParams(sample0, dsts[0], rtPitch, target, &sp);
    m_fusedAside = m_plan.fused_up2x ? !up2x : (m_strip && !m_plan.hdr_tonemap && !strip);
    const bool batchable = !up2x && !strip && n > 1 && rp.src4 && fast && !(run.dvFrames && (!run.dvTab || m_plan.hdr_tonemap)) &&
                           BatchPlan(sample0, dsts[0], rtPitch, rp.aligned, rp.repackSlot != 0, rp.src16, &rp.conv, &rp.direct);
    auto take = [&rp](BatchRoute r) { rp.route = r; return rp; };
    if (batchable && m_plan.direct_convert) return take(BatchRoute::DirectConvert);
    if (rgb && !m_plan.convert && m_stripSurf && m_plan.two_pass && !m_plan.hdr_tonemap && n > 1 && fastStrip &&
        FillStripSurfParams(Surface{nullptr, TexPitch(), m_srcWidth, m_srcHeight, RgbTexFmt(*m_srcParams)}, target, &sp)) {
        rp.strip = sp;
        return take(BatchRoute::RgbSurfaceStrip);
    }
    if (m_plan.hdr_tonemap && m_strip && !up2x && rp.src4 && n > 1 && fastStrip) {
        const int postPitch = (int)(m_videoRect.Width() * SurfBytesPerPixel(m_plan.internal_fmt));
        if (FillStripParams(sample0, nullptr, postPitch, MakeStore(nullptr, postPitch, m_plan.internal_fmt, false), &sp)) {
            rp.strip = sp;
            return take(BatchRoute::StripToneMap);
        }
    }
    if ((!up2x && !strip && !batchable) || !rp.src4 || n == 1) return take(BatchRoute::FrameByFrame);
    if (batchable) return take(BatchRoute::WholeBatchLaunches);
    if (strip) {
        rp.strip = sp;
        return take(BatchRoute::Strip);
    }
    return take(BatchRoute::FusedUp2x);
}

HRESULT CHipVideoProcessor::RunBatchRoute(BatchRoutePlan &rp, BatchRun &run)
{
    const int n = run.n, rtPitch = run.rtPitch;
    const void *const *srcs = run.srcs;
    void *const *const dsts = run.dsts;
    hipStream_t const stream = run.on.stream;
    HRESULT hr = MPCVR_S_OK;
    bool started = run.started;
    auto start = [&] { if (!started) (void)hipEventRecord(m_evStart, stream); started = true; };
    std::vector<const void *> slots;
    if (rp.repackSlot) {
        if ((hr = CheckHip(m_batchTex.CheckCreate(rp.repackSlot * n), "batch source texture"))) return hr;
        start();
        if ((hr = CheckHip(LaunchRepackV210(nullptr, m_srcPitch, (uint8_t *)m_batchTex.ptr, TexPitch(), m_srcHeight, stream, srcs, n, rp.repackSlot), "k_repack_v210"))) return hr;
        m_batchTexZeroed = false;
        slots.resize(n);
        for (int i = 0; i < n; i++) slots[i] = (uint8_t *)m_batchTex.ptr + (size_t)i * rp.repackSlot;
        srcs = slots.data();
    }
    if (run.dvFrames && (rp.route == BatchRoute::DirectConvert || rp.route == BatchRoute::WholeBatchLaunches)) {
        run.usedTables = true;
        rp.direct.conv.dovi = rp.conv.conv.dovi = run.dvTab; rp.direct.dovi_cm = rp.conv.dovi_cm = run.dvCm;
    }
    SlotLease table;
    FusedFrame rows[kHostTableMax]; LaunchFrames frames;
    switch (rp.route) {
    case BatchRoute::DirectConvert:
        if ((hr = BatchFrames(n, srcs, dsts, ConvertBlocksByValueMax(rp.direct), stream, rows, &table, &frames))) break;
        start();
        hr = CheckHip(LaunchConvertBlocks(rp.direct, frames, stream), "k_convert_blocks");
        break;
    case BatchRoute::RgbSurfaceStrip: {
        const int tp = TexPitch();
        const size_t texBytes = (size_t)tp * m_srcHeight;
        const int chunk = FramesPerChunk(n, texBytes, (size_t)1 << 30);
        const bool fresh = m_batchTex.size < texBytes * chunk || !m_batchTex.ptr || !m_batchTexZeroed;
        if ((hr = CheckHip(m_batchTex.CheckCreate(texBytes * chunk), "batch source texture"))) break;
        if (fresh && (hr = CheckHip(hipMemsetAsync(m_batchTex.ptr, 0, texBytes * chunk, stream), "clear batch texture"))) break;
        m_batchTexZeroed = true;
        if ((hr = UploadFrameTable(n, srcs, dsts, nullptr, 0, stream, &table))) break;
        rp.strip.surf.ptr = m_batchTex.ptr;
        rp.strip.surf_stride = texBytes;
        rp.strip.fp.dst_aligned16 = rp.aligned8 ? 1 : 0;
        start();
        for (int at = 0; at < n && !hr; at += chunk) {
            const int m = std::min(chunk, n - at);
            hr = CheckHip(LaunchRepackRgb(m_srcParams->repack, nullptr, m_srcBottomUp ? -m_srcPitch : m_srcPitch, (uint8_t *)m_batchTex.ptr, tp,
                                          m_srcWidth, m_srcHeight, stream, srcs + at, m, texBytes), "k_repack_rgb");
            if (!hr) hr = CheckHip(LaunchFusedStrip(rp.strip, LaunchFrames::Device(table.frames() + at, m), stream), "k_fused_strip<surface>");
        }
        break;
    }
    case BatchRoute::StripToneMap: {
        const int w2 = m_videoRect.Width(), h2 = m_videoRect.Height();
        const size_t postStride = PostStride();
        const int chunk = FramesPerChunk(n, postStride, (size_t)4 << 30);
        if ((hr = CheckHip(m_batchPost.CheckCreate(postStride * chunk), "batch post-scale textures"))) break;
        const Surface post{m_batchPost.ptr, (int)(w2 * SurfBytesPerPixel(m_plan.internal_fmt)), w2, h2, m_plan.internal_fmt};
        rp.strip.fp.store.dst = post.ptr;
        rp.strip.fp.dst_aligned16 = 1;
        start();
        for (int at = 0; at < n && !hr; at += chunk) {
            const int m = std::min(chunk, n - at);
            SlotLease drawTab, realTab;
            if ((hr = UploadFrameTable(m, srcs + at, nullptr, (uint8_t *)m_batchPost.ptr, postStride, stream, &drawTab))) break;
            if ((hr = UploadFrameTable(m, srcs + at, dsts + at, nullptr, 0, stream, &realTab))) break;
            ResizeBatch tb; tb.n = m; tb.in_stride = postStride; tb.frames = realTab.frames();
            if (!(hr = CheckHip(LaunchFusedStrip(rp.strip, LaunchFrames::Device(drawTab.frames(), m), stream), "k_fused_strip")))
                hr = CheckHip(LaunchHdr10ToneMap(post, m_hdrTm, w2, h2, MakeStore(dsts[at], rtPitch, m_plan.swap_fmt, true), stream, &tb), "k_hdr10_tonemap");
        }
        break;
    }
    case BatchRoute::FrameByFrame:
        start();
        for (int i = 0; i < n && !hr; i++) {
            const uint8_t *tex = (const uint8_t *)srcs[i];
            if (!rp.repackSlot && (hr = PrepareSample((const uint8_t *)srcs[i], &tex))) break;
            if (run.dvFrames && (hr = ApplyDoviFrame(run.dvFrames[i]))) break;
            hr = ProcessOne(tex, dsts[i], rtPitch, run.on);
        }
        break;
    case BatchRoute::WholeBatchLaunches:
        if ((hr = UploadFrameTable(n, srcs, dsts, nullptr, 0, stream, &table))) break;
        start();
        hr = ProcessBatchLaunches(run, table.frames(), rp.aligned, rp.conv);
        break;
    case BatchRoute::Strip:
        if ((hr = UploadFrameTable(n, srcs, dsts, nullptr, 0, stream, &table))) break;
        rp.strip.fp.dst_aligned16 = rp.aligned8 ? 1 : 0;
        start();
        hr = CheckHip(LaunchFusedStrip(rp.strip, LaunchFrames::Device(table.frames(), n), stream), "k_fused_strip");
        break;
    case BatchRoute::FusedUp2x: {
        FusedParams fp{};
        FillFusedParams((const uint8_t *)srcs[0], nullptr, rtPitch, &fp);
        fp.dst_aligned16 = rp.aligned ? 1 : 0;
        if ((hr = BatchFrames(n, srcs, dsts, FusedUp2xByValueMax(fp), stream, rows, &table, &frames))) break;
        start();
        hr = CheckHip(LaunchFusedUp2x(fp, frames, stream), "k_fused_up2x");
        break;
    }
    }
    (void)hipEventRecord(m_evStop, stream);
    m_timed = true;
    return hr;
}

HRESULT CHipVideoProcessor::PrepareErrDiff(int frames)
{
    m_edPitch = (m_windowRect.Width() * 4 + 255) & ~255;
    m_edStride = (size_t)m_edPitch * (size_t)m_windowRect.Height();
    const HRESULT hr = CheckHip(m_edPost.CheckCreate(m_edStride * (size_t)frames + 512), "error-diffusion intermediates");
    m_edBase = hr ? nullptr : (uint8_t *)m_edPost.ptr + 256;
    return hr;
}

HRESULT CHipVideoProcessor::ErrDiffPass(const LaunchFrames &frames, int rtPitch, hipStream_t s)
{
    ErrDiffParams P{};
    P.x0 = std::max((int)m_videoRect.left, 0); P.y0 = std::max((int)m_videoRect.top, 0);
    P.x1 = std::min((int)m_videoRect.right, m_windowRect.Width()); P.y1 = std::min((int)m_videoRect.bottom, m_windowRect.Height());
    if (P.x1 <= P.x0 || P.y1 <= P.y0) return MPCVR_S_OK;
    P.src_pitch = m_edPitch; P.dst_pitch = rtPitch;
    static const int order = [] { const char *e = std::getenv("MPCVR_ERRDIFF_ORDER"); return e ? std::atoi(e) : 1; }();
    P.order = order;
    const char *stall = std::getenv("MPCVR_ERRDIFF_TEST_STALL"), *spin = std::getenv("MPCVR_ERRDIFF_SPIN");
    P.test_stall = stall && *stall && *stall != '0' ? 1 : 0;
    P.spin_limit = spin && *spin ? std::atoi(spin) : m_edPatience;
    HRESULT hr;
    if (!m_edStatus) {
        if ((hr = CheckHip(hipHostMalloc((void **)&m_edStatus, sizeof(int), hipHostMallocDefault), "error-diffusion status word"))) return hr;
        *m_edStatus = 0;
    }
    if (*m_edStatus) { *m_edStatus = 0; return Fail(MPCVR_E_FAIL, "error diffusion: a band of an earlier pass gave up waiting for the band above"); }
    if (s != m_stream) (void)hipStreamSynchronize(m_stream);
    const size_t need = ErrorDiffusionHandoffBytes(P, frames.n);
    if ((hr = CheckHip(m_edHandoff.CheckCreate(need), "error-diffusion hand-off rows"))) return hr;
    P.handoff = (uint32_t *)m_edHandoff.ptr; P.status = m_edStatus;
    const EdLayout key{P.x0, P.x1, P.y0, P.y1, frames.n, (const void *)P.handoff};
    if (!(key == m_edKey) || m_edGen >= 4095 || m_edGen <= 0 || P.test_stall) { P.gen = 0; m_edGen = 1; m_edKey = P.test_stall ? EdLayout{} : key; }
    else P.gen = ++m_edGen;
    return CheckHip(LaunchErrorDiffusion(P, frames, s), "k_error_diffusion");
}

HRESULT CHipVideoProcessor::ProcessBatchErrDiff(BatchRun &run)
{
    const int n = run.n;
    HRESULT hr;
    const size_t one = ((size_t)((m_windowRect.Width() * 4 + 255) & ~255)) * (size_t)m_windowRect.Height();
    static const int cap = [] { const char *e = std::getenv("MPCVR_ERRDIFF_CHUNK"); return e ? std::atoi(e) : 0; }();
    int most = FramesPerChunk(n, one, (size_t)4 << 30);
    if (cap > 0) most = std::min(most, cap);
    const int chunks = (n + most - 1) / most;
    const int chunk = (n + chunks - 1) / chunks;
    if ((hr = PrepareErrDiff(chunk))) return hr;
    std::vector<void *> mids(chunk);
    for (int i = 0; i < chunk; i++) mids[i] = m_edBase + (size_t)i * m_edStride;
    (void)JoinFrameLanes(false);
    (void)hipEventRecord(m_evStart, m_stream);
    for (int at = 0; at < n; at += chunk) {
        const int m = std::min(chunk, n - at);
        BatchRun part = run.Slice(at, m);
        part.dsts = mids.data(); part.rtPitch = m_edPitch; part.started = true;
        hr = ProcessBatchRoutes(part);
        run.usedTables = run.usedTables || part.usedTables;
        if (hr) return hr;
        SlotLease tab;
        if ((hr = UploadFrameTable(m, (const void *const *)mids.data(), run.dsts + at, nullptr, 0, m_stream, &tab))) return hr;
        if ((hr = ErrDiffPass(LaunchFrames::Device(tab.frames(), m), run.rtPitch, m_stream))) return hr;
    }
    (void)hipEventRecord(m_evStop, m_stream);
    m_timed = true;
    return MPCVR_S_OK;
}

void CHipVideoProcessor::TableRing::Release()
{
    for (Slot &slot : m_slots) {
        slot.dev.Release();
        if (slot.pinned) (void)hipHostFree(slot.pinned);
        if (slot.done) (void)hipEventDestroy(slot.done);
    }
}

HRESULT CHipVideoProcessor::TableRing::Next(size_t bytes, size_t atLeast, void **pinned)
{
    Slot &slot = m_slots[m_sent % m_slots.size()];
    HRESULT hr = slot.done ? m_owner->CheckHip(hipEventSynchronize(slot.done), "table slot wait")
                           : m_owner->CheckHip(hipEventCreateWithFlags(&slot.done, hipEventDisableTiming), "table slot event");
    if (hr) return hr;
    if (bytes > slot.cap) {
        if (slot.pinned) (void)hipHostFree(slot.pinned);
        slot.pinned = nullptr; slot.cap = 0;
        const size_t cap = std::max(bytes, atLeast);
        if ((hr = m_owner->CheckHip(hipHostMalloc(&slot.pinned, cap, hipHostMallocDefault), "table slot pinned"))) return hr;
        if ((hr = m_owner->CheckHip(slot.dev.CheckCreate(cap), "table slot"))) return hr;
        slot.cap = cap;
    }
    *pinned = slot.pinned;
    return MPCVR_S_OK;
}

HRESULT CHipVideoProcessor::TableRing::Send(size_t bytes, hipStream_t stream, const char *what, SlotLease *lease)
{
    Slot &slot = m_slots[m_sent % m_slots.size()];
    *lease = SlotLease(slot.dev.ptr, slot.done, stream);
    if (HRESULT hr = m_owner->CheckHip(hipMemcpyAsync(slot.dev.ptr, slot.pinned, bytes, hipMemcpyHostToDevice, stream), what)) return hr;
    m_sent++;
    return MPCVR_S_OK;
}

HRESULT CHipVideoProcessor::UploadFrameTable(int n, const void *const *srcs, void *const *dsts, uint8_t *dst_base, size_t dst_stride, hipStream_t stream, SlotLease *lease)
{
    return m_tableRing.SendRows<FusedFrame>(n, stream, "frame table", lease, [&](FusedFrame *fr) {
        for (int i = 0; i < n; i++) { fr[i].src = srcs ? (const uint8_t *)srcs[i] : nullptr; fr[i].dst = dsts ? dsts[i] : (void *)(dst_base + (size_t)i * dst_stride); }
    });
}

HRESULT CHipVideoProcessor::BatchFrames(int n, const void *const *srcs, void *const *dsts, int byValueMax, hipStream_t stream, FusedFrame *rows, SlotLease *lease, LaunchFrames *frames)
{
    if (n <= byValueMax) {
        for (int i = 0; i < n; i++) rows[i] = FusedFrame{(const uint8_t *)srcs[i], dsts[i]};
        *frames = LaunchFrames::Host(rows, n);
        return MPCVR_S_OK;
    }
    const HRESULT hr = UploadFrameTable(n, srcs, dsts, nullptr, 0, stream, lease);
    if (!hr) *frames = LaunchFrames::Device(lease->frames(), n);
    return hr;
}

void BakeFusedTables(const uint16_t *dither, const float *lut, void *out)
{
    auto half_bits_to_float = [](uint16_t h) {
        const uint32_t sign = (uint32_t)(h & 0x8000u) << 16, e = (h >> 10) & 31u, m = h & 1023u;
        float mag;
        if (e == 31) { uint32_t b = 0x7f800000u | (m << 13); std::memcpy(&mag, &b, 4); }
        else if (e == 0) mag = (float)m * (1.0f / 16777216.0f);
        else { uint32_t b = ((e + 112u) << 23) | (m << 13); std::memcpy(&mag, &b, 4); }
        uint32_t b;
        std::memcpy(&b, &mag, 4);
        b |= sign;
        std::memcpy(&mag, &b, 4);
        return mag;
    };
    unsigned char *o = (unsigned char *)out;
    uint16_t *D = (uint16_t *)o;
    uint32_t *Di = (uint32_t *)(o + 1024 * 2);
    float *T = (float *)(o + kBakedDitherBytes);
    for (int i = 0; i < 1024; i++) {
        D[i] = dither[i];
        const float x = half_bits_to_float(dither[i]) * 1024.0f + 0.5f;
        const uint32_t j = x >= 4294967296.0f ? 0xffffffffu : x > 0.0f ? (uint32_t)x : 0u;
// ... 16 lines not shown
    m_fusedTabHost.resize(kBakedTableBytes);
    BakeFusedTables(m_ditherHost, host, m_fusedTabHost.data());
    HRESULT hr;
    if ((hr = CheckHip(m_fusedTab.CheckCreate(kBakedTableBytes), "fused tables"))) return hr;
    if ((hr = CheckHip(hipMemcpy(m_fusedTab.ptr, m_fusedTabHost.data(), kBakedTableBytes, hipMemcpyHostToDevice), "fused tables upload"))) return hr;
    m_fusedTabValid = true;
    return MPCVR_S_OK;
}

HRESULT CHipVideoProcessor::GetFusedTables(void *buf, size_t *size)
{
    if (!size) return Fail(MPCVR_E_POINTER, "null size");
    if (!m_srcParams) return Fail(MPCVR_E_NOT_VALID_STATE, "InitMediaType has not been called");
    if (!buf) { *size = kBakedTableBytes; return MPCVR_S_OK; }
    if (*size < (size_t)kBakedTableBytes) { *size = kBakedTableBytes; return Fail(MPCVR_E_INVALIDARG, "buffer too small"); }
    HRESULT hr;
    if (m_planDirty && (hr = UpdatePlan())) return hr;
    if (!m_fusedTabValid) return Fail(MPCVR_E_NOT_VALID_STATE, "no baked tables");
    std::memcpy(buf, m_fusedTabHost.data(), kBakedTableBytes);
    *size = kBakedTableBytes;
    return MPCVR_S_OK;
}

bool CHipVideoProcessor::BatchPlan(const uint8_t *sample0, void *rt0, int rtPitch, bool aligned, bool repacked, bool src16, FusedParams *conv, FusedParams *direct) const
{
    if (!m_plan.convert) return false;
    if ((m_srcParams->cformat == MPCVR_CF_V210 && !repacked) || m_srcParams->layout == LAY_RGB) return false;
    if (m_plan.direct_convert) {
        FillFusedParams(sample0, rt0, rtPitch, direct);
        direct->dst_aligned16 = aligned ? 1 : 0;
        direct->src_aligned16 = src16 ? 1 : 0;
        return ConvertBlocksSupported(*direct, true);
    }
    if (!m_plan.two_pass && !m_plan.one_pass && !m_plan.hdr_tonemap) return false;
    *conv = ConvertOutputParams(sample0, nullptr);
    conv->src_aligned16 = src16 ? 1 : 0;
    return ConvertBlocksSupported(*conv, false);
}

HRESULT CHipVideoProcessor::ProcessBatchLaunches(const BatchRun &run, const FusedFrame *table, bool aligned, FusedParams conv)
{
    const int n = run.n;
    HRESULT hr;
    const bool hdr = m_plan.hdr_tonemap;
    const size_t postStride = hdr ? PostStride() : 0;
    const size_t per = m_convBytes + m_midBytes + postStride;
    const int chunk = FramesPerChunk(n, per, (size_t)4 << 30);
    if ((hr = CheckHip(m_batchConv.CheckCreate(m_convBytes * chunk), "batch convert output"))) return hr;
    if (m_midBytes && (hr = CheckHip(m_batchMid.CheckCreate(m_midBytes * chunk), "batch resize texture"))) return hr;
    if (hdr && (hr = CheckHip(m_batchPost.CheckCreate(postStride * chunk), "batch post-scale textures"))) return hr;
    DrawFrames df{m_batchConv.ptr, m_batchMid.ptr, m_batchPost.ptr, m_convBytes, m_midBytes, postStride};
    SlotLease postTab;
    if (hdr) {
        if ((hr = UploadFrameTable(chunk, nullptr, nullptr, (uint8_t *)m_batchPost.ptr, postStride, run.on.stream, &postTab))) return hr;
        df.lastTab = postTab.frames();
        aligned = true;
    }
    df.aligned = aligned ? 1 : 0;
    for (int at = 0; at < n; at += chunk) {
        const int m = std::min(chunk, n - at);
        conv.store.dst = m_batchConv.ptr;
        const BatchRun part = run.Slice(at, m);
        if (part.dvTab) { conv.conv.dovi = part.dvTab; conv.dovi_cm = part.dvCm; }
        if ((hr = CheckHip(LaunchConvertBlocks(conv, LaunchFrames::Device(table + at, m), run.on.stream, m_convBytes), "k_convert_blocks"))) return hr;
        df.n = m;
        df.rtTab = table + at;
        if (!hdr) df.lastTab = df.rtTab;
        if ((hr = ResizeShaderPass(nullptr, run.dsts[0], run.rtPitch, df, run.on))) return hr;
    }
    return MPCVR_S_OK;
}

void CHipVideoProcessor::SaveDoviWalk(DoviWalkState *s) const
{
    s->valid = m_doviValid; s->l1Present = m_doviL1Present; s->l2Present = m_doviL2Present; s->blobOverride = m_blobOverride; s->planDirty = m_planDirty;
    s->md = m_doviMd; s->host = m_doviHost;
    std::memcpy(s->l1, m_doviL1, sizeof(m_doviL1)); std::memcpy(s->l2raw, m_doviL2Raw, sizeof(m_doviL2Raw)); std::memcpy(s->cm, m_cm, sizeof(m_cm));
    s->tail = m_tail; s->gamma = m_gamma; s->tm = m_hdrTm;
}
void CHipVideoProcessor::RestoreDoviWalk(const DoviWalkState &s)
{
    m_doviValid = s.valid; m_doviL1Present = s.l1Present; m_doviL2Present = s.l2Present; m_blobOverride = s.blobOverride; m_planDirty = s.planDirty;
    m_doviMd = s.md; m_doviHost = s.host;
    std::memcpy(m_doviL1, s.l1, sizeof(m_doviL1)); std::memcpy(m_doviL2Raw, s.l2raw, sizeof(m_doviL2Raw)); std::memcpy(m_cm, s.cm, sizeof(m_cm));
    m_tail = s.tail; m_gamma = s.gamma; m_hdrTm = s.tm;
}

HRESULT CHipVideoProcessor::ApplyDoviFrame(const DoviFrameState &f)
{
    m_doviHost = f.p;
    std::memcpy(m_cm, f.cm, sizeof(m_cm));
    m_hdrTm = f.tm;
    return UploadDoviParams();
}

HRESULT CHipVideoProcessor::UploadDoviTables(BatchRun *run, hipStream_t stream, SlotLease *lease)
{
    const int n = run->n;
    const size_t each = sizeof(DoviParams) + 12 * sizeof(float), need = each * n;
    DoviParams *tp;
    if (HRESULT hr = m_dvTableRing.Next(need, each * 64, (void **)&tp)) return hr;
    float *tc = (float *)(tp + n);
    for (int i = 0; i < n; i++) {
        tp[i] = run->dvFrames[i].p;
        std::memcpy(tc + (size_t)12 * i, run->dvFrames[i].cm, 12 * sizeof(float));
    }
    if (HRESULT hr = m_dvTableRing.Send(need, stream, "dovi tables upload", lease)) return hr;
    run->dvTab = (const DoviParams *)lease->dev;
    run->dvCm = (const float *)(run->dvTab + n);
    return MPCVR_S_OK;
}

HRESULT CHipVideoProcessor::ProcessBatchDovi(int n, const void *const *srcs, void *const *dsts, int rtPitch, const mpcvr_dovi_metadata *rpus)
{
    const BatchRecord record(*this, n);
    if (HRESULT bad = CheckBatchArgs(n, rpus ? srcs : nullptr, dsts, rtPitch)) return bad;
    for (int i = 0; i < n; i++)
        if (!CheckDoviCurves(rpus[i])) return Fail(MPCVR_E_INVALIDARG, "Dolby Vision curves: num_pivots outside [2,9], mapping_idc > 1 or more than 32 level-2 blocks");
    (void)hipSetDevice(m_device);
    HRESULT hr = MPCVR_S_OK;
    std::vector<DoviFrameState> fs((size_t)n);
    auto collect = [&](int i) { fs[i].p = m_doviHost; std::memcpy(fs[i].cm, m_cm, sizeof(m_cm)); fs[i].tm = m_hdrTm; };
    DoviWalkState back;
    for (int i = 0; i < n && !hr;) {
        if ((hr = ApplyDoviMetadata(&rpus[i]))) break;
        if (m_planDirty && (hr = UpdatePlan())) break;
        collect(i);
        if ((hr = UploadDoviParams())) break;
        int j = i + 1;
        for (; j < n; j++) {
            SaveDoviWalk(&back);
            if ((hr = ApplyDoviMetadata(&rpus[j]))) break;
            if (m_planDirty || m_doviHost.l2_enabled != fs[i].p.l2_enabled) { RestoreDoviWalk(back); break; }
            collect(j);
        }
        if (hr) break;
        const int len = j - i;
        BatchRun run{len, srcs + i, dsts + i, rtPitch, fs.data() + i};
        SlotLease tables;
        if (len > 1 && !m_plan.hdr_tonemap) hr = UploadDoviTables(&run, m_stream, &tables);
        if (!hr) hr = RunBatch(run);
        m_dvLastInfo += (m_dvLastInfo.empty() ? "" : ",") + std::to_string(len) + (run.usedTables ? ":tables" : ":frames");
        if (!hr && run.usedTables) hr = UploadDoviParams();
        i = j;
    }
    return hr;
}

std::string CHipVideoProcessor::GetLastBatchInfo() const
{
    std::string s = "frames=" + std::to_string(m_lastBatchFrames) + ";launches=" + std::to_string(m_lastBatchLaunches) + ";lane=" + std::to_string(m_lastBatchLane) + ";waits=" + std::to_string(m_lastBatchWaits) +
                    ";uploads=" + std::to_string(m_lastBatchUploads);
    if (!m_dvLastInfo.empty()) s += ";dovi_runs=" + m_dvLastInfo;
    s += m_yuvLastInfo;
    return s;
}

HRESULT CHipVideoProcessor::RenderBackBuffer(bool onContextStream)
{
    if (!m_bInit || !m_srcParams) return Fail(MPCVR_E_NOT_VALID_STATE, "InitMediaType has not been called");
    if (!m_curSample) return MPCVR_S_FALSE;
    (void)hipSetDevice(m_device);
    const int w = m_windowRect.Width(), h = m_windowRect.Height();
    const size_t bytes = (size_t)w * 4 * h;
    HRESULT hr;
    const bool fresh = m_BackBuffer.size < bytes || !m_BackBuffer.ptr;
    if ((hr = CheckHip(m_BackBuffer.CheckCreate(bytes), "back buffer"))) return hr;
    const size_t clearBytes = (fresh || m_videoRect != CRect(0, 0, w, h)) ? bytes : 0;
    hr = ProcessFrame(m_BackBuffer.ptr, w * 4, nullptr, nullptr, clearBytes, onContextStream);
    if (hr >= 0) { m_backW = w; m_backH = h; m_backFmt = m_cfg.output_format; }
    return hr;
}

HRESULT CHipVideoProcessor::GetBackBuffer(void **ptr, int *pitch, int *w, int *h)
{
    if (!m_BackBuffer.ptr) return Fail(MPCVR_E_NOT_VALID_STATE, "Render has not been called");
    if (ptr) *ptr = m_BackBuffer.ptr;
    if (pitch) *pitch = m_windowRect.Width() * 4;
    if (w) *w = m_windowRect.Width();
    if (h) *h = m_windowRect.Height();
    return MPCVR_S_OK;
}

HRESULT CHipVideoProcessor::GetDisplayedImage(void *hostPixels, size_t *size, bool deepColor, int *width, int *height, int *bits)
{
    if (!size) return Fail(MPCVR_E_POINTER, "null size");
    if (!m_BackBuffer.ptr || m_backW <= 0 || m_backH <= 0) return Fail(MPCVR_E_NOT_VALID_STATE, "Render has not been called");
    const int w = m_backW, h = m_backH;
    const bool ten = m_backFmt == MPCVR_OUT_RGB10A2;
    const int bpp = (ten && deepColor) ? 48 : 32;
    const size_t dibPitch = (((size_t)w * bpp + 31) & ~(size_t)31) / 8, need = dibPitch * h;
    if (width) *width = w;
    if (height) *height = h;
    if (bits) *bits = bpp;
    if (!hostPixels) { *size = need; return MPCVR_S_OK; }
    if (*size < need) { *size = need; return Fail(MPCVR_E_INVALIDARG, "buffer too small"); }
    HRESULT hr = Synchronize();
    if (hr) return hr;
    const size_t srcPitch = (size_t)w * 4;
    if (!ten) {
        if ((hr = CheckHip(hipMemcpy(hostPixels, m_BackBuffer.ptr, need, hipMemcpyDeviceToHost), "displayed image read-back"))) return hr;
    } else {
        std::vector<uint32_t> staging((size_t)w * h);
        if ((hr = CheckHip(hipMemcpy(staging.data(), m_BackBuffer.ptr, srcPitch * h, hipMemcpyDeviceToHost), "displayed image read-back"))) return hr;
        for (int y = 0; y < h; y++) {
            const uint32_t *src = staging.data() + (size_t)y * w;
            uint8_t *row = (uint8_t *)hostPixels + (size_t)y * dibPitch;
            if (bpp == 32) {
                uint32_t *d = (uint32_t *)row;
                for (int x = 0; x < w; x++) {
                    const uint32_t t = src[x];
                    d[x] = ((t & 0x3fc00000u) >> 22) | ((t & 0x000ff000u) >> 4) | ((t & 0x000003fcu) << 14) | 0xff000000u;
                }
            } else {
                uint16_t *d = (uint16_t *)row;
                for (int x = 0; x < w; x++) {
                    const uint32_t t = src[x];
                    *d++ = (uint16_t)((t & 0x3ff00000u) >> 14); *d++ = (uint16_t)((t & 0x000ffc00u) >> 4); *d++ = (uint16_t)((t & 0x000003ffu) << 6);
                }
            }
        }
    }
    *size = need;
    return MPCVR_S_OK;
}

HRESULT CHipVideoProcessor::GetCurentImage(void *hostBGRA, size_t *size)
{
    if (!size) return Fail(MPCVR_E_POINTER, "null size");
    if (!m_bInit || !m_srcParams) return Fail(MPCVR_E_NOT_VALID_STATE, "InitMediaType has not been called");
    int w = m_srcRectWidth, h = m_srcRectHeight;
    if (m_iRotation == 90 || m_iRotation == 270) std::swap(w, h);
    const size_t need = (size_t)w * 4 * h;
    if (!hostBGRA) { *size = need; return MPCVR_S_OK; }
    if (*size < need) { *size = need; return Fail(MPCVR_E_INVALIDARG, "buffer too small"); }
    if (!m_curSample) return Fail(MPCVR_E_NOT_VALID_STATE, "no sample");
    (void)hipSetDevice(m_device);
    HRESULT hr;
    if ((hr = CheckHip(m_Snapshot.CheckCreate(need), "snapshot"))) return hr;
    const CRect backupVid = m_videoRect, backupWnd = m_windowRect;
    const int backupOut = m_cfg.output_format;
    const bool backupHdr = m_hdrOutput;
    const bool backupOverride = m_blobOverride;
    struct { float cm[12]; float lum; float gamut[9]; int tail; float gamma; Up2xWeights ux, uy; } keep{};
    std::vector<uint16_t> keepDither;
    std::vector<float> keepLut;
    if (m_hdrOutput && backupOverride) {
        std::memcpy(keep.cm, m_cm, sizeof(m_cm)); keep.lum = m_lumScale; std::memcpy(keep.gamut, m_gamut, sizeof(m_gamut));
        keep.tail = m_tail; keep.gamma = m_gamma; keep.ux = m_upX; keep.uy = m_upY;
        keepDither.assign(m_ditherHost, m_ditherHost + sizeof(m_ditherHost) / sizeof(m_ditherHost[0]));
        keepLut.assign(m_pqLutHost, m_pqLutHost + sizeof(m_pqLutHost) / sizeof(m_pqLutHost[0]));
    }
    if (m_hdrOutput) { m_hdrOutput = false; m_blobOverride = false; SetShaderConvertColorParams(); UpdateHdrToneMapParams(); }
    m_videoRect = CRect(0, 0, w, h); m_windowRect = m_videoRect; m_cfg.output_format = MPCVR_OUT_BGRA8;
    m_planDirty = true;
    hr = ProcessFrame(m_Snapshot.ptr, w * 4, nullptr, nullptr, 0, true);
    m_videoRect = backupVid; m_windowRect = backupWnd; m_cfg.output_format = backupOut;
    if (backupHdr) {
        m_hdrOutput = true; SetShaderConvertColorParams(); UpdateHdrToneMapParams();
        if (backupOverride) {
            std::memcpy(m_cm, keep.cm, sizeof(m_cm)); m_lumScale = keep.lum; std::memcpy(m_gamut, keep.gamut, sizeof(m_gamut));
            m_tail = keep.tail; m_gamma = keep.gamma; m_upX = keep.ux; m_upY = keep.uy;
            std::memcpy(m_ditherHost, keepDither.data(), sizeof(m_ditherHost));
            std::memcpy(m_pqLutHost, keepLut.data(), sizeof(m_pqLutHost));
            m_blobOverride = true;
        }
    }
    m_planDirty = true;
    if (hr) return hr;
    if (!m_evRb0 && ((hr = CheckHip(hipEventCreate(&m_evRb0), "read-back timer")) || (hr = CheckHip(hipEventCreate(&m_evRb1), "read-back timer")))) return hr;
    (void)hipEventRecord(m_evRb0, m_stream);
    if ((hr = CheckHip(hipMemcpyAsync(hostBGRA, m_Snapshot.ptr, need, hipMemcpyDeviceToHost, m_stream), "readback"))) return hr;
    (void)hipEventRecord(m_evRb1, m_stream);
    m_rbTimed = true;
    if ((hr = CheckHip(hipStreamSynchronize(m_stream), "readback sync"))) return hr;
    if (m_edStatus && *m_edStatus) { *m_edStatus = 0; return Fail(MPCVR_E_FAIL, "error diffusion: a band gave up waiting for the band above"); }
    *size = need;
    return MPCVR_S_OK;
}

void CHipVideoProcessor::Flush()
{
    if (m_bInit) { (void)hipSetDevice(m_device); (void)JoinFrameLanes(true); (void)hipStreamSynchronize(m_stream); }
    m_curSample = nullptr;
    m_doviL1Present = m_doviL2Present = false;
    std::memset(m_doviL1, 0, sizeof(m_doviL1));
}

HRESULT CHipVideoProcessor::Reset()
{
    Flush();
    m_planDirty = true;
    return MPCVR_S_OK;
}

HRESULT CHipVideoProcessor::GetParamBlob(void *buf, size_t *size)
{
    if (!size) return Fail(MPCVR_E_POINTER, "null size");
    if (!m_srcParams) return Fail(MPCVR_E_NOT_VALID_STATE, "InitMediaType has not been called");
    if (!buf) { *size = sizeof(ParamBlob); return MPCVR_S_OK; }
    if (*size < sizeof(ParamBlob)) { *size = sizeof(ParamBlob); return Fail(MPCVR_E_INVALIDARG, "buffer too small"); }
    HRESULT hr;
    if (m_planDirty && (hr = UpdatePlan())) return hr;
    ParamBlob b{};
    b.magic = kBlobMagic; b.version = 1;
    std::memcpy(b.cm, m_cm, sizeof(m_cm));
// ... 166 lines not shown
```

### videorenderer_amd/csrc/hip_video_processor.h

```cpp
#pragma once
#include <hip/hip_runtime_api.h>

#include <string>
#include <utility>
#include <vector>

#include "../../include/mpcvr.h"
#include "vp_encode.h"
#include "vp_lanes.h"
#include "vp_measure.h"
#include "vp_tensor.h"
#include "vp_tensor_in.h"
#include "vp_deint.h"
#include "vp_lut3d.h"
#include "vp_deband.h"
#include "vp_launch.h"
#include "vp_params.h"
#include "vp_plan.h"
#include "vp_plan_tables.h"

namespace mpcvr {

typedef int32_t HRESULT;

// ... 77 lines not shown
    HRESULT ProcessBatchDeint(int n, const void *const *frames, int fieldOrder, int fieldsPerFrame, int mode, void *const *dsts, int rtPitch);
    HRESULT RenderLut3d(int field, const void *lutDev, int n, void *dst, int dstPitch, int dstFmt);
    HRESULT ProcessBatchLut3d(int n, const void *const *srcs, const void *lutDev, int lutN, void *const *dsts, int dstPitch, int dstFmt);
    HRESULT RenderDeband(int field, const mpcvr_deband_params *params, uint32_t seed, void *dst, int dstPitch, int dstFmt);
    HRESULT ProcessBatchDeband(int n, const void *const *srcs, const mpcvr_deband_params *params, uint32_t seed, void *const *dsts, int dstPitch, int dstFmt);
    HRESULT SetBatchYuvBudget(size_t bytes) { m_yuvBudget = bytes; return MPCVR_S_OK; }
    std::string GetLastBatchInfo() const;
    HRESULT ProcessBatchDovi(int n, const void *const *srcs, void *const *dsts, int rtPitch, const mpcvr_dovi_metadata *rpus);
    void Flush();
    HRESULT Reset();

    HRESULT GetParamBlob(void *buf, size_t *size);
    HRESULT SetParamBlob(const void *buf, size_t size);
    HRESULT GetFusedTables(void *buf, size_t *size);
    HRESULT BroadcastParamBlobBegin(void *ncclComm, int root, int rank);
    HRESULT BroadcastParamBlobEnd();
    HRESULT GetColorMatrix(float out[12]);
    HRESULT GetExtFmt(uint32_t *v);
    HRESULT GetFrameBytes(size_t *bytes, int *pitch);
    std::string GetPathInfo();
    HRESULT GetLastProcessMs(float *ms);
    HRESULT GetLastTimings(float *copy_host_ms, float *upload_ms, float *process_ms, float *readback_ms);
    const char *LastError() const { return m_lastError.c_str(); }

private:
    HRESULT Fail(HRESULT hr, const std::string &msg);
    HRESULT RenderBackBuffer(bool onContextStream);
    HRESULT CheckHip(hipError_t e, const char *what);

    void SetShaderConvertColorParams();
    void SetShaderLuminanceParams();
    HRESULT UpdatePlan();
    struct RunOn { hipStream_t stream = nullptr; int inflight = 1; };
    HRESULT ConvertColorPass(const uint8_t *sample, const RunOn &on);
    FusedParams ConvertOutputParams(const uint8_t *sample, void *out, int inflight = 1) const;
    struct DrawFrames {
        void *conv = nullptr, *mid = nullptr, *post = nullptr;
        size_t convStride = 0, midStride = 0, postStride = 0;
        int n = 1;
        const FusedFrame *lastTab = nullptr;
        const FusedFrame *rtTab = nullptr;
        int aligned = 1;
    };
    HRESULT ResizeShaderPass(const uint8_t *sample, void *rt, int rtPitch, const DrawFrames &df, const RunOn &on);
    HRESULT ProcessOne(const uint8_t *sample, void *rt, int rtPitch, const RunOn &on);
    HRESULT ProcessFrame(void *pRenderTarget, int rtPitch, const CRect *srcRect, const CRect *dstRect, size_t clearBytes, bool onContextStream);
    HRESULT UploadPlanTables(const PlanTables &t);
    bool ConvertEnabled() const;
    int TexPitch() const;
    HRESULT PrepareSample(const uint8_t *dev_sample, const uint8_t **tex);
    void FillConvertParams(const uint8_t *sample, ConvertParams *P) const;
    StoreParams MakeStore(void *dst, int pitch, int dstFmt, bool rt) const;
    void FillFusedParams(const uint8_t *sample, void *rt, int rtPitch, FusedParams *fp, int inflight = 1) const;

    bool m_bInit = false;
    int m_device = 0;
    hipStream_t m_stream = nullptr;
    bool m_ownStream = false;
    hipEvent_t m_evStart = nullptr, m_evStop = nullptr;
    bool m_timed = false;
    hipEvent_t m_evUp0 = nullptr, m_evUp1 = nullptr, m_evRb0 = nullptr, m_evRb1 = nullptr;
    bool m_upTimed = false, m_rbTimed = false;
    float m_copyHostMs = -1.0f;
    std::string m_lastError;

    mpcvr_settings m_cfg{};
    ProcAmp m_procAmp;
    int m_iRotation = 0;
    bool m_bFlip = false;
    int m_SampleFormat = 0;
    bool m_hdrOutput = false, m_hdrMetaValid = false;
    int m_hdrToneMapType = 0;
    float m_hdrDisplayMaxNits = 1000.0f, m_hdrMeta[4] = {0, 0, 0, 0};
    HdrToneMapParams m_hdrTm{};
    void UpdateHdrToneMapParams();
    struct DoviSlot { DoviParams *pinned = nullptr; hipEvent_t copied = nullptr; };
    bool m_doviValid = false;
    mpcvr_dovi_metadata m_doviMd{};
    DoviParams m_doviHost{};
    bool m_doviL1Present = false, m_doviL2Present = false;
    uint32_t m_doviL1[3] = {0, 0, 0};
    float m_doviL2Raw[5] = {0, 0, 0, 0, 0};
    DevBuffer m_doviDev;
    DoviSlot m_doviSlots[4];
    unsigned m_doviSlotNext = 0;
    HRESULT UploadDoviParams();
    HRESULT ApplyDoviMetadata(const mpcvr_dovi_metadata *md);
    struct DoviFrameState { DoviParams p; float cm[12]; HdrToneMapParams tm; };
    struct DoviWalkState {
        bool valid, l1Present, l2Present, blobOverride, planDirty;
        mpcvr_dovi_metadata md; DoviParams host; uint32_t l1[3]; float l2raw[5]; float cm[12]; int tail; float gamma; HdrToneMapParams tm;
    };
    void SaveDoviWalk(DoviWalkState *s) const;
    void RestoreDoviWalk(const DoviWalkState &s);
    struct BatchRun {
        int n = 0;
        const void *const *srcs = nullptr;
        void *const *dsts = nullptr;
        int rtPitch = 0;
        const DoviFrameState *dvFrames = nullptr;
        const DoviParams *dvTab = nullptr;
        const float *dvCm = nullptr;
        bool started = false;
        bool usedTables = false;
        RunOn on;
        BatchRun Slice(int at, int m) const {
            BatchRun r = *this;
            r.n = m; r.srcs += at; r.dsts += at;
            if (dvFrames) r.dvFrames += at;
            if (dvTab) { r.dvTab += at; r.dvCm += (size_t)12 * at; }
            r.usedTables = false;
            return r;
        }
    };
    struct SlotLease {
        const void *dev = nullptr; hipEvent_t done = nullptr; hipStream_t stream = nullptr;
        SlotLease() = default;
        SlotLease(const void *d, hipEvent_t e, hipStream_t s) : dev(d), done(e), stream(s) {}
        SlotLease(SlotLease &&o) noexcept : dev(o.dev), done(o.done), stream(o.stream) { o.done = nullptr; }
        SlotLease &operator=(SlotLease &&o) noexcept { std::swap(dev, o.dev); std::swap(done, o.done); std::swap(stream, o.stream); return *this; }
        ~SlotLease() { if (done) (void)hipEventRecord(done, stream); }
        const FusedFrame *frames() const { return (const FusedFrame *)dev; }
    };
    class TableRing {
    public:
        TableRing(CHipVideoProcessor *owner, int slots) : m_owner(owner), m_slots((size_t)slots) {}
        HRESULT Next(size_t bytes, size_t atLeast, void **pinned);
        HRESULT Send(size_t bytes, hipStream_t stream, const char *what, SlotLease *lease);
        template <class Row, class Fill>
        HRESULT SendRows(int n, hipStream_t stream, const char *what, SlotLease *lease, Fill fill)
        {
            Row *rows;
            if (HRESULT hr = Next(sizeof(Row) * n, sizeof(Row) * 64, (void **)&rows)) return hr;
            fill(rows);
            return Send(sizeof(Row) * n, stream, what, lease);
        }
        size_t Sent() const { return m_sent; }
        void Release();
    private:
        struct Slot { void *pinned = nullptr; size_t cap = 0; DevBuffer dev; hipEvent_t done = nullptr; };
        CHipVideoProcessor *m_owner;
        std::vector<Slot> m_slots;
        size_t m_sent = 0;
    };
    TableRing m_dvTableRing{this, 2};
    HRESULT UploadDoviTables(BatchRun *run, hipStream_t stream, SlotLease *lease);
    HRESULT ApplyDoviFrame(const DoviFrameState &f);
    std::string m_dvLastInfo;
    unsigned m_laneFrames = 0;
    unsigned m_launches = 0;
    int m_lastBatchLane = -1;
    int m_lastBatchUploads = 0;
    int m_lastBatchFrames = 0, m_lastBatchLaunches = 0;
    HRESULT CheckTargetLayout(int n, void *const *dsts, int rtPitch);
    struct BatchRecord {
        CHipVideoProcessor &vp; const unsigned launches; const size_t uploads;
        BatchRecord(CHipVideoProcessor &v, int frames) : vp(v), launches(v.m_launches), uploads(v.m_tableRing.Sent())
        {
            vp.m_lastBatchFrames = frames; vp.m_lastBatchLaunches = vp.m_lastBatchUploads = 0; vp.m_lastBatchLane = -1; vp.m_lastBatchWaits = 0;
            vp.m_dvLastInfo.clear(); vp.m_yuvLastInfo.clear();
        }
        ~BatchRecord() { vp.m_lastBatchLaunches = (int)(vp.m_launches - launches); vp.m_lastBatchUploads = (int)(vp.m_tableRing.Sent() - uploads); }
    };
    HRESULT CheckBatchArgs(int n, const void *const *srcs, void *const *dsts, int rtPitch);
    HRESULT RunBatch(BatchRun &run);
    HRESULT ProcessBatchRoutes(BatchRun &run);
    bool ToneMapActive() const;

    const FmtConvParams *m_srcParams = nullptr;
    int m_srcWidth = 0, m_srcHeight = 0, m_srcPitch = 0, m_srcLines = 0;
    bool m_srcBottomUp = false;
    CRect m_srcRect;
    int m_srcRectWidth = 0, m_srcRectHeight = 0;
    ExtFmt m_decExFmt{0}, m_srcExFmt{0};
    CRect m_videoRect, m_windowRect;

    float m_cm[12] = {0};
    float m_lumScale = 80.0f;
    float m_gamut[9] = {0};
    int m_tail = TAIL_NONE;
    float m_gamma = 1.0f;
    bool m_blobOverride = false;
    DevBuffer m_bcast;
    bool m_bcastPending = false, m_bcastIsRoot = false;
    std::vector<unsigned char> m_bcastHost;

    bool m_planDirty = true;
    PassPlan m_plan;
    Up2xWeights m_upX{}, m_upY{};

    DevBuffer m_TexSrcVideo;
    DevBuffer m_TexRaw;
    DevBuffer m_TexPost;
    struct UploadSlot {
        void *pinned = nullptr; size_t pinnedSize = 0;
        DevBuffer dev;
        hipEvent_t uploaded = nullptr, consumed = nullptr;
        bool inFlight = false;
        bool consumedRecorded = false;
        hipStream_t consumedOn = nullptr;
    };
    static constexpr int kUploadSlots = 3;
    UploadSlot m_up[kUploadSlots];
    int m_upNext = 0, m_curSlot = -1;
    hipStream_t m_copyStream = nullptr;
    void MarkConsumed();
    HRESULT AcquireUploadSlot(size_t bytes, int *si);
    HRESULT PublishUploadSlot(int si, hipStream_t recordedOn);
    const uint8_t *m_curSample = nullptr;
    DevBuffer m_TexConvertOutput, m_TexResize, m_BackBuffer, m_Snapshot;
    int m_backW = 0, m_backH = 0, m_backFmt = 0;
    DevBuffer m_dither;
    DevBuffer m_pqLut;
    DevBuffer m_hlgLut;
    DevBuffer m_eotfLut;
    float m_pqLutHost[kPqLutSize];
    bool m_pqLutValid = false;
    DevBuffer m_fusedTab;
    std::vector<unsigned char> m_fusedTabHost;
    std::vector<float> m_hlgLutHost;
    const float *m_fusedTabLut = nullptr;
    bool m_fusedTabValid = false;
    HRESULT UploadFusedTables();
    PlanTables m_tables;
    DevBuffer m_axisX, m_axisY;
    AxisTaps m_tapsX{}, m_tapsY{};
    const int32_t *m_otherX = nullptr, *m_otherY = nullptr;
    TableRing m_tableRing{this, 8};
    uint16_t m_ditherHost[1024];
    FrameLanes m_lanes;
    int m_lastBatchWaits = 0;
    hipStream_t m_lastRun = nullptr;
    bool FrameLanesUsable() const;
    RtSpan TargetSpan(const void *rt, int rtPitch) const { return RowsSpan(rt, (size_t)rtPitch, m_windowRect.Height(), (size_t)m_windowRect.Width() * 4); }
    HRESULT JoinFrameLanes(bool host_wait) { return CheckHip(m_lanes.Join(host_wait, m_stream), "frame lane sync"); }
    void OrderOnContextStream() { (void)JoinFrameLanes(false); m_lanes.NoteStreamWork(); }
    size_t m_convBytes = 0, m_midBytes = 0, m_postBytes = 0;
    DevBuffer m_batchConv, m_batchMid;
    DevBuffer m_batchPost;
    DevBuffer m_edPost;
    DevBuffer m_edHandoff;
    struct EdLayout {
        int x0 = 0, x1 = 0, y0 = 0, y1 = 0, n = 0; const void *rows = nullptr;
        bool operator==(const EdLayout &o) const { return x0 == o.x0 && x1 == o.x1 && y0 == o.y0 && y1 == o.y1 && n == o.n && rows == o.rows; }
    };
    int m_edGen = 0; EdLayout m_edKey;
    int m_edPatience = 0;
    int *m_edStatus = nullptr;
    uint8_t *m_edBase = nullptr;
    int m_edPitch = 0;
    size_t m_edStride = 0;
    HRESULT PrepareErrDiff(int frames);
    HRESULT ErrDiffPass(const LaunchFrames &frames, int rtPitch, hipStream_t s);
    HRESULT ProcessBatchErrDiff(BatchRun &run);
    size_t PostStride() const { return (m_postBytes + 255) & ~(size_t)255; }
    HRESULT UploadFrameTable(int n, const void *const *srcs, void *const *dsts, uint8_t *dst_base, size_t dst_stride, hipStream_t stream, SlotLease *lease);
    HRESULT BatchFrames(int n, const void *const *srcs, void *const *dsts, int byValueMax, hipStream_t stream, FusedFrame *rows, SlotLease *lease, LaunchFrames *frames);
    DevBuffer m_batchTex;
    bool m_texSrcZeroed = false, m_batchTexZeroed = false;
    DevBuffer m_jincFirst, m_jincSecond, m_jincFused;
    const float *m_jincFusedTab = nullptr;
    const void *m_jincFirstTab = nullptr, *m_jincSecondTab = nullptr;
    const float *m_jincFirstCtr = nullptr, *m_jincSecondCtr = nullptr;
    HRESULT UploadJincPhases(const DrawCoords &dc, DevBuffer &buf, const void **tab, const float **ctr);
    bool m_strip = false;
    bool m_stripSurf = false;
    bool FillStripSurfParams(const Surface &src, const StoreParams &store, FusedStripParams *sp) const;
    DevBuffer m_stripTab;
    bool FillStripParams(const uint8_t *sample, void *dst, int dstPitch, const StoreParams &store, FusedStripParams *sp, int inflight = 1) const;
    bool FillStripTables(const StoreParams &store, int perForce, FusedStripParams *sp) const;
    mutable int m_stripRan = -1;
    mutable bool m_fusedAside = false;
    bool m_period = false;
    enum class BatchRoute { DirectConvert, RgbSurfaceStrip, StripToneMap, FrameByFrame, WholeBatchLaunches, Strip, FusedUp2x };
    struct BatchRoutePlan {
        BatchRoute route = BatchRoute::FrameByFrame;
        size_t repackSlot = 0;
        bool aligned = true, aligned8 = true, src16 = true, src4 = true;
        FusedStripParams strip{};
        FusedParams conv{}, direct{};
    };
    BatchRoutePlan ClassifyBatch(const BatchRun &run) const;
    bool BatchLaneEligible(const BatchRoutePlan &rp, const BatchRun &run) const;
    int PlaceBatch(const BatchRoutePlan &rp, BatchRun &run, std::vector<RtSpan> &&writes);
    void NoteBatchQueued(int lane) { if (lane >= 0) m_lanes.NoteLaneBatch(lane); }
    struct YuvSurface {
        DevBuffer buf;
        CRect window, video;
        bool cleared = false;
    };
    YuvSurface m_yuvSurf[FrameLanes::kFrameLanes];
    size_t m_yuvBudget = 0;
    std::string m_yuvLastInfo;
    DevBuffer m_sampleSurf;
    template <class WritesOf, class Pass>
    HRESULT RunSurfaceChunks(int n, const void *const *srcs, const BatchYuvLayout &lay, const char *tag, WritesOf writesOf, Pass pass);
    template <class Pass>
    HRESULT RunSampleChunks(int n, const ChunkLayout &lay, void *const *dsts, int rtPitch, const char *tag, Pass pass);
    HRESULT RenderChunk(BatchRoutePlan &rp, BatchRun &run, YuvSurface &surf);
    HRESULT EncodeChunk(BatchRun &run, const EncodeParams &encode, const EncodePlan &plan, void *const *yPlanes, void *const *uvPlanes, uint32_t *histRows);
    mpcvr_rect ActiveRect() const;
    HRESULT RunBatchRoute(BatchRoutePlan &rp, BatchRun &run);
    bool BatchPlan(const uint8_t *sample0, void *rt0, int rtPitch, bool aligned, bool repacked, bool src16, FusedParams *conv, FusedParams *direct) const;
    HRESULT ProcessBatchLaunches(const BatchRun &run, const FusedFrame *table, bool aligned, FusedParams conv);
};

}
```

### videorenderer_amd/csrc/vp_fused_up2x.h

```cpp
#pragma once
#include "vp_fused_dev.h"
#include "vp_fused_prefetch.h"

namespace mpcvr {

namespace {

#ifndef MPCVR_UP2X_WAVES
#define MPCVR_UP2X_WAVES 3
#endif
#ifndef MPCVR_UP2X_COMPILER_WAITS
#define MPCVR_UP2X_COMPILER_WAITS 0
#endif
static_assert(LDS_D + LDS_DB == kBakedDitherBytes && LDS_D + LDS_DB + LDS_T == kBakedTableBytes, "the baked image is the LDS layout");
static_assert(LDS_A % 16 == 0 && LDS_D + LDS_DB == 256 * 16 + 256 * 8 && LDS_T == 8 * 256 * 16, "stage_baked_tables: pieces per thread");

template <bool WITH_LUT>
__device__ __forceinline__ void stage_baked_tables(unsigned char *tables, const unsigned char *__restrict__ img)
{
    typedef uint32_t u32x4 __attribute__((ext_vector_type(4)));
    typedef uint32_t u32x2 __attribute__((ext_vector_type(2)));
    const int t = threadIdx.x;
    const u32x4 d0 = ((const u32x4 *)img)[t];
    const u32x2 d1 = ((const u32x2 *)(img + 256 * 16))[t];
    u32x4 l[8];
    if (WITH_LUT) {
#pragma unroll
        for (int k = 0; k < 8; k++) l[k] = ((const u32x4 *)(img + LDS_D + LDS_DB))[t + 256 * k];
    }
    ((u32x4 *)tables)[t] = d0;
    ((u32x2 *)(tables + 256 * 16))[t] = d1;
    if (WITH_LUT) {
#pragma unroll
        for (int k = 0; k < 8; k++) ((u32x4 *)(tables + LDS_D + LDS_DB))[t + 256 * k] = l[k];
    }
}

template <int NT, int TAIL, int SRC, int EPI, int XC>
__device__ __forceinline__ void fused_up2x_body(const FusedArgs &P, const FusedFrame *__restrict__ frames, const unsigned char *__restrict__ baked,
                                                const FrameTable32 &tab)
{
    extern __shared__ __attribute__((aligned(16))) unsigned char smem[];
    float *Aall = (float *)smem;
    unsigned short *D = (unsigned short *)(smem + LDS_A);
    uint32_t *Di = (uint32_t *)(smem + LDS_A + LDS_D);
    f2 *T = (f2 *)(smem + LDS_A + LDS_D + LDS_DB);

    if (baked) stage_baked_tables<tail_has_table(TAIL)>(smem + LDS_A, baked);
    else {
        for (int i = threadIdx.x; i < 1024; i += 256) {
            const unsigned short d = P.dither[i];
            D[i] = d;
            Di[i] = (uint32_t)(__half2float(__ushort_as_half(d)) * 1024.0f + 0.5f) << 14;
        }
        if (tail_has_table(TAIL))
            for (int i = threadIdx.x; i < LUT_N; i += 256) {
                const float v = P.lut[i], n = P.lut[min(i + 1, LUT_N - 1)];
                T[i] = f2{v, n - v};
            }
    }
    __syncthreads();

    const int wave = __builtin_amdgcn_readfirstlane((int)(threadIdx.x >> 6)), lane = threadIdx.x & 63;
    const int W = P.W, H = P.H;
    const int x0 = (blockIdx.x * WAVES + wave) * S;
    const int s0 = blockIdx.y * P.seg_rows;
    if (x0 >= W || s0 >= H) return;
    const int s1 = min(s0 + P.seg_rows, H);
    float *A = Aall + wave * A_FLOATS;

    uint64_t tab_src = (uint64_t)tab.f[blockIdx.z & 31].src, tab_dst = (uint64_t)tab.f[blockIdx.z & 31].dst;
    asm volatile("" : "+s"(tab_src), "+s"(tab_dst));
    FusedFrame frame{(const uint8_t *)tab_src, (void *)tab_dst};
    if (frames) frame = frames[blockIdx.z];
    auto uniform_ptr = [](const void *q) {
        const uint64_t v = (uint64_t)q;
        return ((uint64_t)(uint32_t)__builtin_amdgcn_readfirstlane((int)(v >> 32)) << 32) | (uint32_t)__builtin_amdgcn_readfirstlane((int)(uint32_t)v);
    };
    const uint64_t src_u = uniform_ptr(frame.src), dst_u = uniform_ptr(frame.dst);
    const gcptr py = (gcptr)src_u;
    const gptr pdst = (gptr)dst_u;

    const int X = x0 - 4 + 2 * lane;
    const int Xg = clampi(X, 0, W - 2);
    const bool edge_wave = x0 == 0 || x0 + 2 * 63 - 4 > W - 2;
    const bool xy_active = lane < 60;
    const int ox = 2 * x0 + 4 * lane;
    const bool store_ok = xy_active && ox < 2 * W;
    const int wx0 = P.off_x + ox;
    const bool d_aligned = (wx0 & 3) == 0;
    const bool st_aligned = d_aligned && (((uintptr_t)dst_u | (uintptr_t)P.dst_pitch) & 15) == 0;
    const uint32_t lane_off = (uint32_t)wx0 * 4u;

    const f2 WT[2][3] = {{f2{P.we[0], P.we[1]}, f2{P.we[2], P.we[3]}, f2{P.we[4], P.we[5]}},
                        {f2{P.wo[0], P.wo[1]}, f2{P.wo[2], P.wo[3]}, f2{P.wo[4], P.wo[5]}}};
    const f2 MM[5] = {f2{P.m[0], P.m[1]}, f2{P.m[2], P.m[3]}, f2{P.m[4], P.m[5]}, f2{P.m[6], P.m[7]}, f2{P.m[8], 0.0f}};
    const f2 GG[5] = {f2{P.gamut[0], P.gamut[1]}, f2{P.gamut[2], P.gamut[3]}, f2{P.gamut[4], P.gamut[5]}, f2{P.gamut[6], P.gamut[7]}, f2{P.gamut[8], 0.0f}};
    constexpr bool FASTEPI = EPI == EPI_DITHER8;
    const f2 maxv2 = splat((FASTEPI || P.final_pass) ? P.maxv : P.quant);
    const f2 cmax2 = splat(P.maxv), cinv2 = splat(P.inv_maxv);
    f2 big2 = splat(8388608.0f);
    asm volatile("" : "+v"(big2));
    f2 CC[3] = {splat(P.c[0]), splat(P.c[1]), splat(P.c[2])};
    asm volatile("" : "+v"(CC[0]), "+v"(CC[1]), "+v"(CC[2]));

    f2 win[8][3][2];
#pragma unroll
    for (int i = 0; i < 8; i++)
#pragma unroll
        for (int c = 0; c < 3; c++) win[i][c][0] = win[i][c][1] = splat(0.0f);

    const int n_iter = (s1 - s0 + 1) / 2 + 3;
    constexpr int NL = MPCVR_UP2X_COMPILER_WAITS ? 0 : raw_unseen_loads<SRC>();
    constexpr bool UNSEEN = NL != 0;
    Raw raw2[2];
    RawUnseen<raw_unseen_loads<SRC>() ? raw_unseen_loads<SRC>() : 1> pend2[2];
    RawAddr ra;
    make_raw_addr<SRC>(P, Xg, ra);
    auto prefetch = [&](int ar, int b) __attribute__((always_inline)) {
        if constexpr (UNSEEN) load_raw_unseen<SRC>(P, py, ra, clampi(ar, 0, H - 1), clampi(ar + 1, 0, H - 1), pend2[b]);
        else load_raw<SRC>(P, py, ra, clampi(ar, 0, H - 1), clampi(ar + 1, 0, H - 1), raw2[b]);
    };
    prefetch(s0 - 3, 0);
    prefetch(s0 - 1, 1);

    auto stage_c = [&](int ar, int b, int tw) {
        f2 rc[2][3];
        if constexpr (UNSEEN) {
            raw_unseen_arrived<NL>(tw);
            raw_unseen_finish<SRC>(P, pend2[b], raw2[b]);
        }
        convert_block<TAIL, SRC, DV_NONE, XC, XC == XC_ALWAYS ? OUT_CODE_F : OUT_NORM>(P, MM, GG, CC, raw2[b], P.rect_t + clampi(ar, 0, H - 1), P.rect_t + clampi(ar + 1, 0, H - 1), T, rc);
        prefetch(ar + 4, b);
#pragma unroll
        for (int c = 0; c < 3; c++) {
            f2 qe = (XC == XC_ALWAYS ? rc[0][c] : unorm_round2(rc[0][c], cmax2, big2)) * cinv2;
            f2 qo = (XC == XC_ALWAYS ? rc[1][c] : unorm_round2(rc[1][c], cmax2, big2)) * cinv2;
            *(f4 *)(A + (c * AW + 2 * lane) * 2) = f4{qe.x, qe.y, qo.x, qo.y};
            if (edge_wave) {
                if (X < 0) *(f2 *)(A + (c * AW + 2 * lane + 1) * 2) = qe;
                else if (X > W - 2) *(f2 *)(A + (c * AW + 2 * lane) * 2) = qo;
            }
        }
    };
    stage_c(s0 - 3, 0, 0);

    for (int tb = 0; tb < n_iter; tb += 4) {
#pragma unroll
        for (int u = 0; u < 4; u++) {
            const int t = tb + u;
            if (t >= n_iter) break;
            const int a = s0 - 3 + 2 * t;

            __builtin_amdgcn_fence(__ATOMIC_RELEASE, "wavefront");
            __builtin_amdgcn_wave_barrier();
            __builtin_amdgcn_fence(__ATOMIC_ACQUIRE, "wavefront");

            if (xy_active) {
                f4 abuf[2][5];
#pragma unroll
                for (int i = 0; i < 5; i++) abuf[0][i] = ((const f4 *)(A + (0 * AW + 2 * lane) * 2))[i];
#pragma unroll
                for (int c = 0; c < 3; c++) {
                    if (c < 2) {
#pragma unroll
                        for (int i = 0; i < 5; i++) abuf[(c + 1) & 1][i] = ((const f4 *)(A + ((c + 1) * AW + 2 * lane) * 2))[i];
                    }
                    f2 av[10];
#pragma unroll
                    for (int i = 0; i < 5; i++) { const f4 p4 = abuf[c & 1][i]; av[2 * i] = f2{p4.x, p4.y}; av[2 * i + 1] = f2{p4.z, p4.w}; }
                    f2 o[4];
                    tapsN<NT, false, 4>([&](int i) -> const f2 (&)[3] { return WT[i & 1]; },
                                        [&](int i, int tt) { return av[4 + (i >> 1) + ((i & 1) ? 0 : -1) + tap_off<NT>(tt)]; }, o);
                    const int sa = (2 * u) & 7, sb = (2 * u + 1) & 7;
                    const f2 h0 = half_round2(o[0]), h1 = half_round2(o[1]), h2 = half_round2(o[2]), h3 = half_round2(o[3]);
                    win[sa][c][0] = f2{h0.x, h1.x};
                    win[sa][c][1] = f2{h2.x, h3.x};
                    win[sb][c][0] = f2{h0.y, h1.y};
                    win[sb][c][1] = f2{h2.y, h3.y};
                }
            }
            __builtin_amdgcn_fence(__ATOMIC_RELEASE, "wavefront");
            __builtin_amdgcn_wave_barrier();
            __builtin_amdgcn_fence(__ATOMIC_ACQUIRE, "wavefront");

            if (t + 1 < n_iter) stage_c(a + 2, (u + 1) & 1, t);

            if (t >= 3 && store_ok) {
#pragma unroll
                for (int kk = 0; kk < 2; kk++) {
                    const int k = a - 3 + kk;
#pragma unroll
                    for (int par = 0; par < 2; par++) {
                        const int wy = P.off_y + 2 * k + par;
                        uint32_t dj[4] = {0, 0, 0, 0};
                        if (FASTEPI) {
                            typedef uint32_t u32x4 __attribute__((ext_vector_type(4)));
                            const u32x4 dd = *(const u32x4 *)(Di + (wy & 31) * 32 + (wx0 & 31));
                            dj[0] = dd.x; dj[1] = dd.y; dj[2] = dd.z; dj[3] = dd.w;
                        }
                        f2 res6[6];
                        tapsN<NT, true, 6>([&](int) -> const f2 (&)[3] { return WT[par]; },
                                           [&](int i, int tt) { return win[(2 * u + 2 + kk + 2 + par + tap_off<NT>(tt)) & 7][i >> 1][i & 1]; }, res6);
                        f2 res[3][2];
#pragma unroll
                        for (int c = 0; c < 3; c++) { res[c][0] = res6[2 * c]; res[c][1] = res6[2 * c + 1]; }
                        uint32_t pk[4];
                        if (FASTEPI) {
                            f2 uq[3][2];
#pragma unroll
                            for (int c = 0; c < 3; c++)
#pragma unroll
                                for (int pp = 0; pp < 2; pp++) uq[c][pp] = pk_fma(res[c][pp], maxv2, big2);
#pragma unroll
                            for (int px = 0; px < 4; px++) {
                                const uint32_t ib = __umul24(__float_as_uint(uq[2][px >> 1][px & 1]), P.epi_mul) + dj[px];
                                const uint32_t ig = __umul24(__float_as_uint(uq[1][px >> 1][px & 1]), P.epi_mul) + dj[px];
                                const uint32_t ir = __umul24(__float_as_uint(uq[0][px >> 1][px & 1]), P.epi_mul) + dj[px];
                                const uint32_t bg = __builtin_amdgcn_perm(ig, ib, 0x0c0c0703u);
                                pk[px] = __builtin_amdgcn_perm(ir, bg, 0x0d070100u);
                            }
                        } else if (EPI == EPI_DIRECT8) {
                            f2 uq[3][2];
#pragma unroll
                            for (int c = 0; c < 3; c++)
#pragma unroll
                                for (int pp = 0; pp < 2; pp++) uq[c][pp] = pk_fma(res[c][pp], maxv2, big2);
#pragma unroll
                            for (int px = 0; px < 4; px++) {
                                const uint32_t cr = __float_as_uint(uq[0][px >> 1][px & 1]), cg = __float_as_uint(uq[1][px >> 1][px & 1]), cb = __float_as_uint(uq[2][px >> 1][px & 1]);
                                if (P.out10) {
                                    pk[px] = (cb << 20) | ((cg << 10) | (cr + 0x75000000u));
                                } else {
                                    const uint32_t bg = __builtin_amdgcn_perm(cg, cb, 0x0c0c0400u);
                                    pk[px] = __builtin_amdgcn_perm(cr, bg, 0x0d040100u);
                                }
                            }
                        } else {
#pragma unroll
                            for (int px = 0; px < 4; px++) {
                                float c3[3];
#pragma unroll
                                for (int c = 0; c < 3; c++) {
                                    const float q = floorf(fmaf(res[c][px >> 1][px & 1], P.final_pass ? P.maxv : P.quant, 0.5f));
                                    float v = q;
                                    if (P.final_pass) {
                                        const float d = __half2float(__ushort_as_half(D[(wy & 31) * 32 + ((wx0 + px) & 31)]));
                                        v = fminf(fmaxf(floorf(fmaf(q, P.q_over_maxv, d)), 0.0f), P.quant);
                                    }
                                    c3[c] = v;
                                }
                                pk[px] = P.out10 ? pack_rgb10a2(c3[0], c3[1], c3[2]) : pack_bgra8(c3[0], c3[1], c3[2]);
                            }
                        }
                        const gptr rowp = pdst + (uint32_t)wy * (uint32_t)P.dst_pitch;
                        if (EPI != EPI_GENERIC || st_aligned) {
                            typedef uint32_t u32x4 __attribute__((ext_vector_type(4)));
                            u32x4 v4 = {pk[0], pk[1], pk[2], pk[3]};
                            __attribute__((address_space(1))) u32x4 *sp = (__attribute__((address_space(1))) u32x4 *)(rowp + opaque(lane_off));
                            *sp = v4;
                        } else {
                            __attribute__((address_space(1))) uint32_t *dst = (__attribute__((address_space(1))) uint32_t *)(rowp + lane_off);
                            dst[0] = pk[0]; dst[1] = pk[1]; dst[2] = pk[2]; dst[3] = pk[3];
                        }
                    }
                }
            }
        }
    }
}

template <int NT, int TAIL, int SRC, int EPI, int XC = XC_NEVER>
__global__ __launch_bounds__(256, MPCVR_UP2X_WAVES) void k_fused_up2x(FusedArgs P, const FusedFrame *__restrict__ frames, const unsigned char *__restrict__ baked,
                                                                      FrameTable32 tab)
{
    fused_up2x_body<NT, TAIL, SRC, EPI, XC>(P, frames, baked, tab);
}
template <int NT, int TAIL, int SRC, int EPI>
inline auto fused_up2x_kernel(bool exact) -> decltype(&k_fused_up2x<NT, TAIL, SRC, EPI, XC_NEVER>)
{
    if constexpr (exact_capable<TAIL, SRC, EPI == EPI_DITHER8>() == XC_RUNTIME) { if (exact) return k_fused_up2x<NT, TAIL, SRC, EPI, XC_ALWAYS>; }
    return k_fused_up2x<NT, TAIL, SRC, EPI, XC_NEVER>;
}

}

template <int NT>
hipError_t LaunchFusedUp2xNT(const FusedParams &P, const FusedArgs &a_in, int strips, int seg, const LaunchFrames &F, hipStream_t s)
{
    const ConvertParams &c = P.conv;
    const dim3 grid((strips + WAVES - 1) / WAVES, (c.out_h + seg - 1) / seg, F.n);
    const dim3 block(256, 1, 1);
    const int tailk = FusedTailKind(P);
    static const int lds_pad = EnvInt("MPCVR_FUSED_LDS_PAD", 0);
    const FusedArgs &a = a_in;
    const size_t lds = LDS_A + LDS_D + LDS_DB + (tail_has_table(tailk) ? LDS_T : 0) + (size_t)lds_pad;
    const int srck = FusedSourceKind(P);
    const unsigned char *baked = (P.baked && (((uintptr_t)P.baked) & 15) == 0 && (!tail_has_table(tailk) || (P.baked_lut && P.baked_lut == a.lut)))
                                     ? (const unsigned char *)P.baked : nullptr;
    FrameTable32 tab{};
    if (F.host) F.ByValue(&tab);
    else if (!F.dev) { tab.n = 1; tab.f[0] = F.one; }
    const bool aligned = P.dst_aligned16 && (a.off_x & 3) == 0 && (a.dst_pitch & 15) == 0;
    const int epik = !aligned ? EPI_GENERIC
                   : (!a.out10 && a.final_pass && a.epi_mul != 0) ? EPI_DITHER8
                   : (!a.final_pass && P.store.dst_fmt == SF_BGRA8 && P.store.quant == 255) ? EPI_DIRECT8
                   : (!a.final_pass && P.store.dst_fmt == SF_RGB10A2 && P.store.quant == 1023) ? EPI_DIRECT8 : EPI_GENERIC;
#define MPCVR_LAUNCH3(NTK, TK, SK, EK) hipLaunchKernelGGL((fused_up2x_kernel<NTK, TK, SK, EK>(a.exact_cv != 0)), grid, block, lds, s, a, F.dev, baked, tab)
#define MPCVR_LAUNCH(NT, TK) do { \
        if (srck == SRC_P01X && epik == EPI_DITHER8) MPCVR_LAUNCH3(NT, TK, SRC_P01X, EPI_DITHER8); \
        else if (srck == SRC_P01X && epik == EPI_DIRECT8) MPCVR_LAUNCH3(NT, TK, SRC_P01X, EPI_DIRECT8); \
        else if (srck == SRC_P01X) MPCVR_LAUNCH3(NT, TK, SRC_P01X, EPI_GENERIC); \
        else if (srck == SRC_PLANAR16 && epik == EPI_DITHER8) MPCVR_LAUNCH3(NT, TK, SRC_PLANAR16, EPI_DITHER8); \
        else if (epik == EPI_DITHER8) MPCVR_LAUNCH3(NT, TK, SRC_GENERIC, EPI_DITHER8); \
        else MPCVR_LAUNCH3(NT, TK, SRC_GENERIC, EPI_GENERIC); } while (0)
#define MPCVR_LAUNCH_8(NT) do { \
        if (srck == SRC_NV12 && epik == EPI_DIRECT8) MPCVR_LAUNCH3(NT, TAILK_NONE, SRC_NV12, EPI_DIRECT8); \
        else if (srck == SRC_NV12) MPCVR_LAUNCH3(NT, TAILK_NONE, SRC_NV12, EPI_GENERIC); \
        else if (srck == SRC_PLANAR8 && epik == EPI_DIRECT8) MPCVR_LAUNCH3(NT, TAILK_NONE, SRC_PLANAR8, EPI_DIRECT8); \
        else MPCVR_LAUNCH(NT, TAILK_NONE); } while (0)
#define MPCVR_LAUNCH_NT(NT) \
    do { if (tailk == TAILK_NONE) MPCVR_LAUNCH_8(NT); else if (tailk == TAILK_PQ_LUT) MPCVR_LAUNCH(NT, TAILK_PQ_LUT); \
         else if (tailk == TAILK_HLG) MPCVR_LAUNCH(NT, TAILK_HLG); else MPCVR_LAUNCH(NT, TAILK_ALU); } while (0)
#ifdef MPCVR_UP2X_HEADLINE_ONLY
    MPCVR_LAUNCH3(NT, TAILK_PQ_LUT, SRC_P01X, EPI_DITHER8);
#else
    MPCVR_LAUNCH_NT(NT);
#endif
#undef MPCVR_LAUNCH_NT
#undef MPCVR_LAUNCH_8
#undef MPCVR_LAUNCH
#undef MPCVR_LAUNCH3
    return hipGetLastError();
}

}
```

### videorenderer_amd/csrc/vp_launch.h

```cpp
#pragma once
#include <hip/hip_runtime_api.h>

#include "vp_params.h"

namespace mpcvr {

hipError_t LaunchConvert(const ConvertParams &P, const Surface &out, hipStream_t s, bool generic = false);
hipError_t LaunchConvertDirect(const ConvertParams &P, const StoreParams &st, hipStream_t s);
struct SrcTable32 { const uint8_t *p[32]; int n; };
hipError_t LaunchRepackRgb(int kind, const uint8_t *src, int src_pitch, uint8_t *dst, int dst_pitch, int width, int lines, hipStream_t s,
                           const void *const *srcs = nullptr, int n = 1, size_t dst_stride = 0);
hipError_t LaunchRepackV210(const uint8_t *src, int src_pitch, uint8_t *dst, int dst_pitch, int lines, hipStream_t s,
                            const void *const *srcs = nullptr, int n = 1, size_t dst_stride = 0);
struct FusedFrame;
struct ResizeBatch { int n = 1; size_t in_stride = 0, dst_stride = 0; const FusedFrame *frames = nullptr; int dst_aligned8 = 1;  };
hipError_t LaunchResize(int axis, bool swap, const Surface &in, const AxisTaps &taps, const int32_t *other,
                        int out_w, int out_h, const StoreParams &st, hipStream_t s, bool generic = false,
                        const ResizeBatch *batch = nullptr);
bool ResizeHasFoldedKernel(int axis, bool swap, const Surface &in, const AxisTaps &taps, const StoreParams &st);
bool Resize2DSupported(const Surface &in, const AxisTaps &tx, const AxisTaps &ty, const StoreParams &st);
hipError_t LaunchResize2D(const Surface &in, const AxisTaps &tx, const AxisTaps &ty, const int32_t *other, int mid_h, int out_w, int out_h,
                          const StoreParams &st, hipStream_t s, const ResizeBatch *batch = nullptr);
hipError_t LaunchCopy(const Surface &in, int out_w, int out_h, const StoreParams &st, hipStream_t s);
hipError_t LaunchCorrection(int kind, const Surface &in, const Surface &out, const float fix16[16], const float gamut9[9], float lum_scale, hipStream_t s);
hipError_t LaunchHdr10ToneMap(const Surface &in, const HdrToneMapParams &tm, int out_w, int out_h, const StoreParams &st, hipStream_t s,
                              const ResizeBatch *batch = nullptr);
hipError_t LaunchJinc2(const Surface &in, const DrawCoords &dc, int out_w, int out_h, const StoreParams &st, hipStream_t s,
                       const void *phases_dev = nullptr, bool fast = false, const ResizeBatch *batch = nullptr, const float *centres_dev = nullptr);
void BuildDrawCentres(const DrawCoords &dc, float *out);
bool Jinc2QuadSupported(const Surface &in, const DrawCoords &dc, int out_w, int out_h, const StoreParams &st);
hipError_t LaunchJinc2Quad(const Surface &in, const DrawCoords &dc, int out_w, int out_h, const StoreParams &st, hipStream_t s, const void *phases_dev,
                           const ResizeBatch *batch = nullptr);
bool BuildJincPhases(const DrawCoords &dc, void *out_table, float max_drift);
size_t JincPhasesBytes();

struct FusedFrame {
    const uint8_t *src;
    void *dst;
};
template <class Table> constexpr int TableRows() { return (int)(sizeof(Table::f) / sizeof(FusedFrame)); }
struct LaunchFrames {
    int n = 1;
    FusedFrame one{nullptr, nullptr};
    const FusedFrame *host = nullptr;
    const FusedFrame *dev = nullptr;
    static LaunchFrames One(const uint8_t *src, void *dst) { LaunchFrames f; f.one = FusedFrame{src, dst}; return f; }
    static LaunchFrames Host(const FusedFrame *rows, int n) { LaunchFrames f; f.n = n; f.host = rows; return f; }
    static LaunchFrames Device(const FusedFrame *rows, int n) { LaunchFrames f; f.n = n; f.dev = rows; return f; }
    bool Valid(int by_value_max) const { return n >= 1 && (host ? !dev && !one.src && n <= by_value_max : dev ? !one.src : n == 1); }
    template <class Table> void ByValue(Table *t) const
    {
        t->n = host ? n : 0;
        if (!host) return;
        for (int i = 0; i < TableRows<Table>(); i++) t->f[i] = i < n ? host[i] : FusedFrame{nullptr, nullptr};
    }
};
struct FusedParams {
    ConvertParams conv;
    size_t plane_off[3];
    Up2xWeights wx, wy;
    StoreParams store;
    int out_w, out_h;
    const float *pq_lut;
    int fast_convert;
    int dst_aligned16;
    int src_aligned16;
    int literal_tail;
    const float *hlg_lut;
    const float *eotf_lut;
    int dovi_l2;
    const float *dovi_cm;
    const float *jinc_tab;
    int exact_wide;
    int exact_convert;
    int inflight;
    const void *baked;
    const float *baked_lut;
};
enum { kBakedDitherBytes = 1024 * 2 + 1024 * 4, kBakedTableBytes = kBakedDitherBytes + kPqLutSize * 8 };
void BakeFusedTables(const uint16_t *dither, const float *lut, void *out);
struct ErrDiffParams {
    int x0, y0, x1, y1;
    int src_pitch, dst_pitch;
    int order;
    int gen;
    int spin_limit;
    int test_stall;
    uint32_t *handoff;
    int *status;
};
size_t ErrorDiffusionHandoffBytes(const ErrDiffParams &P, int n_frames);
hipError_t LaunchErrorDiffusion(const ErrDiffParams &P, const LaunchFrames &F, hipStream_t s);
bool FusedUp2xSupported(const FusedParams &P);
hipError_t LaunchEvalDoviTail(const float *rgb_dev, float *out_dev, size_t n, const float lms[9], const float k[5], const float gamut[9], int l2, float lum_scale, int stage, hipStream_t s);
size_t FusedJincTableBytes();
size_t FusedJincLdsBytes(const FusedParams &P);
void BuildFusedJincTable(const void *phases, float *out);
bool BlockConvertLayout(const FusedParams &P, bool catmull_420);
bool ConvertBlocksSupported(const FusedParams &P, bool to_rt);
struct FrameTable32 { FusedFrame f[32]; int n; };
struct FrameTable128 { FusedFrame f[128]; int n; };
enum { kHostTableMax = 128 };
static_assert(TableRows<FrameTable128>() == kHostTableMax, "the callers' row arrays (kHostTableMax) hold the largest by-value table");
int ConvertBlocksByValueMax(const FusedParams &P);
inline int FusedUp2xByValueMax(const FusedParams &P) { return P.jinc_tab ? 0 : TableRows<FrameTable32>(); }
hipError_t LaunchConvertBlocks(const FusedParams &P, const LaunchFrames &F, hipStream_t s, size_t batch_stride = 0);
hipError_t LaunchFusedUp2x(const FusedParams &P, const LaunchFrames &F, hipStream_t s);

struct FusedStripParams {
    FusedParams fp;
    const void *xi_t, *xw_t;
    const void *yi, *yw;
    const void *yrange;
    const void *xstrip;
    int out_w, out_h;
    int nt, pxl, strip_w, ring, acols;
    Surface surf;
    const int32_t *other;
    int mid_h;
    size_t surf_stride;
    int surface_mode;
    int per_P, per_Q, per_nt, per_acols, per_strip_w, per_own;
    int *ran_period;
    int per_force;
    const void *per_xi_t, *per_xw_t, *per_yw, *per_xstrip;
};
bool FusedStripSupported(const FusedStripParams &S);
hipError_t LaunchFusedStrip(const FusedStripParams &S, const LaunchFrames &F, hipStream_t s);
size_t FusedStripLdsBytes(const FusedStripParams &S);
size_t DeviceLdsLimit();
bool FusedPeriodTakes(const FusedStripParams &S);

}
```

Measured before the change: 23750.

## Add bi-planar up2x kernel twin that carries chroma rows and shares chroma via DPP

Adds a specialised variant of the fused 2x upscale kernel for P010/NV12 sources. It carries the lower chroma row of each step into the next, so each step loads three words instead of four, and builds the horizontal chroma interpolation from the neighbouring lane through a DPP move instead of extra loads. A host predicate checks that the vertical chroma row sequence really carries over, and the variant is taken only for planned tail and epilogue combinations with even-aligned rects. This adds four new compiled translation units and an environment switch to disable the path, and edge-column handling changes in the variant.

```diff
diff --git a/include/mpcvr.h b/include/mpcvr.h
--- a/include/mpcvr.h
+++ b/include/mpcvr.h
@@ -271,6 +271,7 @@
 int32_t mpcvr_get_fused_tables(mpcvr_ctx *ctx, void *buf, size_t *size);
 int32_t mpcvr_get_path_info(mpcvr_ctx *ctx, char *buf, size_t buf_size);
 int32_t mpcvr_get_last_batch_info(mpcvr_ctx *ctx, char *buf, size_t buf_size);
+int32_t mpcvr_plan_up2x_row_carry(int32_t vk1, int32_t vk2, int32_t vk3, int32_t rect_t, int32_t h, int32_t ch);
 const char *mpcvr_last_error(mpcvr_ctx *ctx);
 const char *mpcvr_version(void);
 
diff --git a/videorenderer_amd/api.py b/videorenderer_amd/api.py
--- a/videorenderer_amd/api.py
+++ b/videorenderer_amd/api.py
@@ -178,7 +178,7 @@
     "mpcvr_get_backbuffer", "mpcvr_get_current_image", "mpcvr_get_displayed_image", "mpcvr_flush", "mpcvr_reset", "mpcvr_process_batch", "mpcvr_process_batch_dovi",
     "mpcvr_get_param_blob", "mpcvr_set_param_blob", "mpcvr_broadcast_param_blob_begin", "mpcvr_broadcast_param_blob_end",
     "mpcvr_broadcast_param_blob", "mpcvr_get_color_matrix", "mpcvr_get_extfmt",
-    "mpcvr_get_frame_bytes", "mpcvr_get_fused_tables", "mpcvr_get_path_info", "mpcvr_get_last_batch_info", "mpcvr_last_error", "mpcvr_version",
+    "mpcvr_get_frame_bytes", "mpcvr_get_fused_tables", "mpcvr_get_path_info", "mpcvr_get_last_batch_info", "mpcvr_plan_up2x_row_carry", "mpcvr_last_error", "mpcvr_version",
     "mpcvr_get_last_process_ms", "mpcvr_get_last_timings",
     "mpcvr_plan_frame_layout", "mpcvr_plan_color_matrix", "mpcvr_plan_gamut_2020_to_709", "mpcvr_plan_pq_lut",
     "mpcvr_plan_upscale_weights", "mpcvr_plan_axis_taps", "mpcvr_plan_describe", "mpcvr_plan_final_pass_multiplier",
@@ -259,6 +259,7 @@
         "mpcvr_get_fused_tables": [vp, vp, P(C.c_size_t)],
         "mpcvr_get_path_info": [vp, C.c_char_p, C.c_size_t],
         "mpcvr_get_last_batch_info": [vp, C.c_char_p, C.c_size_t],
+        "mpcvr_plan_up2x_row_carry": [i32, i32, i32, i32, i32, i32],
         "mpcvr_get_last_process_ms": [vp, P(f)],
         "mpcvr_get_last_timings": [vp, P(f), P(f), P(f), P(f)],
         "mpcvr_plan_frame_layout": [i32, i32, i32, P(i32), P(C.c_size_t)],
@@ -351,6 +352,10 @@
     return nbytes.value, pitch.value
 
 
+def plan_up2x_row_carry(vk1, vk2, vk3, rect_t, h, ch):
+    return bool(load_library().mpcvr_plan_up2x_row_carry(vk1, vk2, vk3, rect_t, h, ch))
+
+
 def plan_color_matrix(cformat, rect_w, rect_h, extfmt=0, brightness=0.0, contrast=1.0, hue=0.0, saturation=1.0):
     out = (C.c_float * 12)()
     ex = C.c_uint32()
@@ -1239,6 +1244,11 @@
             out.update(deband_chunks=int(d["deband_chunks"]), deband_lanes=[int(x) for x in d["deband_lanes"].split(",") if x], deband_taps=d.get("deband_taps", ""))
         return out
 
+    def GetUp2xForm(self):
+        buf = C.create_string_buffer(512)
+        self._check(self._L.mpcvr_get_last_batch_info(self._ctx, buf, 512))
+        return dict(kv.split("=", 1) for kv in buf.value.decode().split(";")).get("up2x")
+
     def GetLastProcessMs(self):
         ms = C.c_float()
         self._check(self._L.mpcvr_get_last_process_ms(self._ctx, C.byref(ms)))
diff --git a/videorenderer_amd/build.py b/videorenderer_amd/build.py
--- a/videorenderer_amd/build.py
+++ b/videorenderer_amd/build.py
@@ -22,6 +22,10 @@
     ("vp_fused_up2x_nt4.hip", []),
     ("vp_fused_up2x_nt5.hip", []),
     ("vp_fused_up2x_nt6.hip", []),
+    ("vp_fused_up2x_bp.hip", []),
+    ("vp_fused_up2x_bp_nt4.hip", []),
+    ("vp_fused_up2x_bp_nt5.hip", []),
+    ("vp_fused_up2x_bp_nt6.hip", []),
     ("vp_fused_strip.hip", []),
     ("vp_fused_strip_nt4.hip", []),
     ("vp_fused_strip_nt6.hip", []),
diff --git a/videorenderer_amd/csrc/hip_video_processor.cpp b/videorenderer_amd/csrc/hip_video_processor.cpp
--- a/videorenderer_amd/csrc/hip_video_processor.cpp
+++ b/videorenderer_amd/csrc/hip_video_processor.cpp
@@ -906,7 +906,12 @@
         FusedParams fp{};
         FillFusedParams(sample, rt, rtPitch, &fp, on.inflight);
         if (StoreRowsFit32(fp.store, fp.out_h))
-            return CheckHip(LaunchFusedUp2x(fp, LaunchFrames::One(sample, rt), on.stream), "k_fused_up2x");
+        {
+            FusedUp2xLastForm() = -1;
+            const hipError_t e = LaunchFusedUp2x(fp, LaunchFrames::One(sample, rt), on.stream);
+            if (FusedUp2xLastForm() >= 0) m_up2xForm = FusedUp2xLastForm();
+            return CheckHip(e, "k_fused_up2x");
+        }
         m_fusedAside = true;
     }
     if (m_strip) {
@@ -1183,7 +1188,9 @@
         fp.dst_aligned16 = rp.aligned ? 1 : 0;
         if ((hr = BatchFrames(n, srcs, dsts, FusedUp2xByValueMax(fp), stream, rows, &table, &frames))) break;
         start();
+        FusedUp2xLastForm() = -1;
         hr = CheckHip(LaunchFusedUp2x(fp, frames, stream), "k_fused_up2x");
+        if (FusedUp2xLastForm() >= 0) m_up2xForm = FusedUp2xLastForm();
         break;
     }
     }
@@ -1506,6 +1513,7 @@
     std::string s = "frames=" + std::to_string(m_lastBatchFrames) + ";launches=" + std::to_string(m_lastBatchLaunches) + ";lane=" + std::to_string(m_lastBatchLane) + ";waits=" + std::to_string(m_lastBatchWaits) +
                     ";uploads=" + std::to_string(m_lastBatchUploads);
     if (!m_dvLastInfo.empty()) s += ";dovi_runs=" + m_dvLastInfo;
+    if (m_up2xForm >= 0) s += m_up2xForm == 1 ? ";up2x=bp" : ";up2x=generic";
     s += m_yuvLastInfo;
     return s;
 }
diff --git a/videorenderer_amd/csrc/hip_video_processor.h b/videorenderer_amd/csrc/hip_video_processor.h
--- a/videorenderer_amd/csrc/hip_video_processor.h
+++ b/videorenderer_amd/csrc/hip_video_processor.h
@@ -253,13 +253,14 @@
     int m_lastBatchLane = -1;
     int m_lastBatchUploads = 0;
     int m_lastBatchFrames = 0, m_lastBatchLaunches = 0;
+    int m_up2xForm = -1;
     HRESULT CheckTargetLayout(int n, void *const *dsts, int rtPitch);
     struct BatchRecord {
         CHipVideoProcessor &vp; const unsigned launches; const size_t uploads;
         BatchRecord(CHipVideoProcessor &v, int frames) : vp(v), launches(v.m_launches), uploads(v.m_tableRing.Sent())
         {
             vp.m_lastBatchFrames = frames; vp.m_lastBatchLaunches = vp.m_lastBatchUploads = 0; vp.m_lastBatchLane = -1; vp.m_lastBatchWaits = 0;
-            vp.m_dvLastInfo.clear(); vp.m_yuvLastInfo.clear();
+            vp.m_dvLastInfo.clear(); vp.m_yuvLastInfo.clear(); vp.m_up2xForm = -1;
         }
         ~BatchRecord() { vp.m_lastBatchLaunches = (int)(vp.m_launches - launches); vp.m_lastBatchUploads = (int)(vp.m_tableRing.Sent() - uploads); }
     };
diff --git a/videorenderer_amd/csrc/vp_fused_up2x.h b/videorenderer_amd/csrc/vp_fused_up2x.h
--- a/videorenderer_amd/csrc/vp_fused_up2x.h
+++ b/videorenderer_amd/csrc/vp_fused_up2x.h
@@ -1,6 +1,9 @@
 #pragma once
+#include <type_traits>
+
 #include "vp_fused_dev.h"
 #include "vp_fused_prefetch.h"
+#include "vp_fused_up2x_bp.h"
 
 namespace mpcvr {
 
@@ -36,7 +39,7 @@
     }
 }
 
-template <int NT, int TAIL, int SRC, int EPI, int XC>
+template <int NT, int TAIL, int SRC, int EPI, int XC, int BP = 0>
 __device__ __forceinline__ void fused_up2x_body(const FusedArgs &P, const FusedFrame *__restrict__ frames, const unsigned char *__restrict__ baked,
                                                 const FrameTable32 &tab)
 {
@@ -111,26 +114,34 @@
         for (int c = 0; c < 3; c++) win[i][c][0] = win[i][c][1] = splat(0.0f);
 
     const int n_iter = (s1 - s0 + 1) / 2 + 3;
-    constexpr int NL = MPCVR_UP2X_COMPILER_WAITS ? 0 : raw_unseen_loads<SRC>();
+    static_assert(!BP || (!MPCVR_UP2X_COMPILER_WAITS && XC == XC_NEVER && bp_planned<TAIL, SRC, EPI>()), "the twin: counted waits, the fast convert form, a planned instantiation");
+    constexpr int NL = MPCVR_UP2X_COMPILER_WAITS ? 0 : BP ? BP_LOADS : raw_unseen_loads<SRC>();
     constexpr bool UNSEEN = NL != 0;
     Raw raw2[2];
     RawUnseen<raw_unseen_loads<SRC>() ? raw_unseen_loads<SRC>() : 1> pend2[2];
+    RawUnseenBp pendb[2];
+    ChromaCarry keep{0.0f, 0.0f};
     RawAddr ra;
     make_raw_addr<SRC>(P, Xg, ra);
     auto prefetch = [&](int ar, int b) __attribute__((always_inline)) {
-        if constexpr (UNSEEN) load_raw_unseen<SRC>(P, py, ra, clampi(ar, 0, H - 1), clampi(ar + 1, 0, H - 1), pend2[b]);
+        if constexpr (BP) load_raw_unseen_bp<SRC, false>(P, py, ra, clampi(ar, 0, H - 1), clampi(ar + 1, 0, H - 1), pendb[b]);
+        else if constexpr (UNSEEN) load_raw_unseen<SRC>(P, py, ra, clampi(ar, 0, H - 1), clampi(ar + 1, 0, H - 1), pend2[b]);
         else load_raw<SRC>(P, py, ra, clampi(ar, 0, H - 1), clampi(ar + 1, 0, H - 1), raw2[b]);
     };
-    prefetch(s0 - 3, 0);
+    if constexpr (BP) load_raw_unseen_bp<SRC, true>(P, py, ra, clampi(s0 - 3, 0, H - 1), clampi(s0 - 2, 0, H - 1), pendb[0]);
+    else prefetch(s0 - 3, 0);
     prefetch(s0 - 1, 1);
 
-    auto stage_c = [&](int ar, int b, int tw) {
+    auto stage_c = [&](int ar, int b, int tw, auto first) {
         f2 rc[2][3];
-        if constexpr (UNSEEN) {
+        if constexpr (BP) {
+            raw_unseen_arrived<NL>(tw);
+            convert_block_bp<TAIL, SRC, decltype(first)::value>(P, MM, GG, CC, pendb[b], keep, P.rect_t + clampi(ar, 0, H - 1), P.rect_t + clampi(ar + 1, 0, H - 1), T, rc);
+        } else if constexpr (UNSEEN) {
             raw_unseen_arrived<NL>(tw);
             raw_unseen_finish<SRC>(P, pend2[b], raw2[b]);
         }
-        convert_block<TAIL, SRC, DV_NONE, XC, XC == XC_ALWAYS ? OUT_CODE_F : OUT_NORM>(P, MM, GG, CC, raw2[b], P.rect_t + clampi(ar, 0, H - 1), P.rect_t + clampi(ar + 1, 0, H - 1), T, rc);
+        if constexpr (!BP) convert_block<TAIL, SRC, DV_NONE, XC, XC == XC_ALWAYS ? OUT_CODE_F : OUT_NORM>(P, MM, GG, CC, raw2[b], P.rect_t + clampi(ar, 0, H - 1), P.rect_t + clampi(ar + 1, 0, H - 1), T, rc);
         prefetch(ar + 4, b);
 #pragma unroll
         for (int c = 0; c < 3; c++) {
@@ -139,11 +150,14 @@
             *(f4 *)(A + (c * AW + 2 * lane) * 2) = f4{qe.x, qe.y, qo.x, qo.y};
             if (edge_wave) {
                 if (X < 0) *(f2 *)(A + (c * AW + 2 * lane + 1) * 2) = qe;
+                else if constexpr (BP) {
+                    if (X >= W - 2 && lane != 63) *(f2 *)(A + (c * AW + 2 * lane + 2) * 2) = qo;
+                }
                 else if (X > W - 2) *(f2 *)(A + (c * AW + 2 * lane) * 2) = qo;
             }
         }
     };
-    stage_c(s0 - 3, 0, 0);
+    stage_c(s0 - 3, 0, 0, std::true_type{});
 
     for (int tb = 0; tb < n_iter; tb += 4) {
 #pragma unroll
@@ -184,7 +198,7 @@
             __builtin_amdgcn_wave_barrier();
             __builtin_amdgcn_fence(__ATOMIC_ACQUIRE, "wavefront");
 
-            if (t + 1 < n_iter) stage_c(a + 2, (u + 1) & 1, t);
+            if (t + 1 < n_iter) stage_c(a + 2, (u + 1) & 1, t, std::false_type{});
 
             if (t >= 3 && store_ok) {
 #pragma unroll
@@ -325,7 +339,10 @@
 #ifdef MPCVR_UP2X_HEADLINE_ONLY
     MPCVR_LAUNCH3(NT, TAILK_PQ_LUT, SRC_P01X, EPI_DITHER8);
 #else
-    MPCVR_LAUNCH_NT(NT);
+    const bool twin = !EnvInt("MPCVR_UP2X_NO_BP", 0) && FusedUp2xBpTakes(a, srck, epik, tailk);
+    FusedUp2xLastForm() = twin ? 1 : 0;
+    if (twin) LaunchFusedUp2xBpNT<NT>(a, grid, lds, tailk, srck, epik, F.dev, baked, tab, s);
+    else MPCVR_LAUNCH_NT(NT);
 #endif
 #undef MPCVR_LAUNCH_NT
 #undef MPCVR_LAUNCH_8
diff --git a/videorenderer_amd/csrc/vp_fused_up2x_bp.h b/videorenderer_amd/csrc/vp_fused_up2x_bp.h
--- /dev/null
+++ b/videorenderer_amd/csrc/vp_fused_up2x_bp.h
@@ -0,0 +1,182 @@
+#pragma once
+#include "vp_fused_dev.h"
+#include "vp_fused_prefetch.h"
+
+namespace mpcvr {
+
+inline void FusedUp2xChromaRows(int vk1, int vk2, int vk3, int rect_t, int H, int ch, int a, int *rowA, int *rowB)
+{
+    const int y0 = a < 0 ? 0 : a > H - 1 ? H - 1 : a;
+    const int sy0 = rect_t + y0;
+    const int n = (vk1 * sy0 + vk2 * (sy0 & ~1) + vk3) >> 2;
+    *rowA = n < 0 ? 0 : n > ch - 1 ? ch - 1 : n;
+    *rowB = n + 1 < 0 ? 0 : n + 1 > ch - 1 ? ch - 1 : n + 1;
+}
+bool FusedUp2xRowCarryHolds(int vk1, int vk2, int vk3, int rect_t, int H, int ch);
+bool FusedUp2xBpTakes(const FusedArgs &a, int srck, int epik, int tailk);
+template <int NT>
+void LaunchFusedUp2xBpNT(const FusedArgs &a, dim3 grid, size_t lds, int tailk, int srck, int epik, const FusedFrame *frames_dev, const unsigned char *baked,
+                         const FrameTable32 &tab, hipStream_t s);
+
+namespace {
+
+template <int TAIL, int SRC, int EPI>
+__host__ __device__ constexpr bool bp_planned()
+{
+    return (SRC == SRC_P01X && (EPI == EPI_DITHER8 || EPI == EPI_DIRECT8) && (TAIL == TAILK_PQ_LUT || TAIL == TAILK_HLG || TAIL == TAILK_NONE)) ||
+           (SRC == SRC_NV12 && EPI == EPI_DIRECT8 && TAIL == TAILK_NONE);
+}
+
+constexpr int BP_LOADS = 3;
+struct RawUnseenBp { uint32_t v[4]; };
+struct ChromaCarry { float u, v; };
+
+#define MPCVR_LD_(op, d, o, b) "\n\t" op " %[" d "], %[" o "], %[" b "]"
+#define MPCVR_UNSEEN3(YOP, COP) \
+    asm volatile("s_nop 4" MPCVR_LD_(YOP, "d0", "yo", "r0") MPCVR_LD_(YOP, "d1", "yo", "r1") MPCVR_LD_(COP, "d2", "c1", "ub") \
+                 : [d0] "=&v"(r.v[0]), [d1] "=&v"(r.v[1]), [d2] "=&v"(r.v[2]) \
+                 : [yo] "v"(ra.yoff), [c1] "v"(ra.coff[1]), [r0] "s"(ry0), [r1] "s"(ry1), [ub] "s"(pu + oB))
+#define MPCVR_UNSEEN4(YOP, COP) \
+    asm volatile("s_nop 4" MPCVR_LD_(YOP, "d0", "yo", "r0") MPCVR_LD_(YOP, "d1", "yo", "r1") MPCVR_LD_(COP, "d2", "c1", "ub") MPCVR_LD_(COP, "d3", "c1", "ua") \
+                 : [d0] "=&v"(r.v[0]), [d1] "=&v"(r.v[1]), [d2] "=&v"(r.v[2]), [d3] "=&v"(r.v[3]) \
+                 : [yo] "v"(ra.yoff), [c1] "v"(ra.coff[1]), [r0] "s"(ry0), [r1] "s"(ry1), [ua] "s"(pu + oA), [ub] "s"(pu + oB))
+template <int SRC, bool BOTH>
+__device__ __forceinline__ void load_raw_unseen_bp(const FusedArgs &P, gcptr py, const RawAddr &ra, int y0, int y1, RawUnseenBp &r)
+{
+    static_assert(SRC == SRC_P01X || SRC == SRC_NV12, "bi-planar sources");
+    const int sy0 = P.rect_t + y0, sy1 = P.rect_t + y1;
+    const gcptr ry0 = py + (uint32_t)sy0 * (uint32_t)P.pitch_y, ry1 = py + (uint32_t)sy1 * (uint32_t)P.pitch_y;
+    const int n = chroma_v4(P, sy0) >> 2;
+    const uint32_t oA = (uint32_t)clampi(n, 0, P.ch - 1) * (uint32_t)P.pitch_c, oB = (uint32_t)clampi(n + 1, 0, P.ch - 1) * (uint32_t)P.pitch_c;
+    const gcptr pu = py + P.off_u;
+    if constexpr (BOTH) {
+        if constexpr (SRC == SRC_P01X) MPCVR_UNSEEN4("global_load_dword", "global_load_dword");
+        else MPCVR_UNSEEN4("global_load_ushort", "global_load_ushort");
+    } else {
+        (void)oA;
+        if constexpr (SRC == SRC_P01X) MPCVR_UNSEEN3("global_load_dword", "global_load_dword");
+        else MPCVR_UNSEEN3("global_load_ushort", "global_load_ushort");
+    }
+}
+#undef MPCVR_UNSEEN4
+#undef MPCVR_UNSEEN3
+#undef MPCVR_LD_
+
+template <int SRC>
+__device__ __forceinline__ ChromaCarry chroma_floats(uint32_t d)
+{
+    if constexpr (SRC == SRC_P01X) return ChromaCarry{(float)(d & 0xffffu), (float)(d >> 16)};
+    else return ChromaCarry{(float)(d & 0xffu), (float)((d >> 8) & 0xffu)};
+}
+__device__ __forceinline__ float from_next_lane(float v)
+{
+    return __builtin_bit_cast(float, __builtin_amdgcn_update_dpp(0, __builtin_bit_cast(int, v), 0x130 , 0xf, 0xf, true));
+}
+__device__ __forceinline__ f2 from_next_lane(f2 v) { return f2{from_next_lane(v.x), from_next_lane(v.y)}; }
+
+template <int TAIL>
+__device__ __forceinline__ void convert_block_yuv_bp(const FusedArgs &P, const f2 (&MM)[5], const f2 (&GG)[5], const f2 (&CC)[3], const f2 (&Ycol)[2], const f2 (&Ucol)[2],
+                                                     const f2 (&Vcol)[2], const f2 *T, f2 out[2][3])
+{
+    static_assert(TAIL == TAILK_PQ_LUT || TAIL == TAILK_HLG || TAIL == TAILK_NONE, "tails the twin is planned for");
+    f2 rgbc[2][3];
+#pragma unroll
+    for (int rr = 0; rr < 2; rr++) {
+        rgbc[rr][0] = fma_k<true>(MM, 0, Ycol[rr], fma_k<false>(MM, 2, Vcol[rr], CC[0]));
+        rgbc[rr][1] = fma_k<true>(MM, 3, Ycol[rr], fma_k<false>(MM, 4, Ucol[rr], fma_k<false>(MM, 5, Vcol[rr], CC[1])));
+        rgbc[rr][2] = fma_k<true>(MM, 6, Ycol[rr], fma_k<false>(MM, 7, Ucol[rr], CC[2]));
+    }
+    if constexpr (!tail_has_table(TAIL)) {
+#pragma unroll
+        for (int rr = 0; rr < 2; rr++)
+#pragma unroll
+            for (int ch = 0; ch < 3; ch++) out[rr][ch] = rgbc[rr][ch];
+        return;
+    } else {
+        f2 linc[2][3];
+        f2 ent[2][3][2]; float frc[2][3][2];
+#pragma unroll
+        for (int rr = 0; rr < 2; rr++)
+#pragma unroll
+            for (int ch = 0; ch < 3; ch++)
+#pragma unroll
+                for (int e = 0; e < 2; e++) {
+                    const float t = rgbc[rr][ch][e] * (float)(LUT_N - 1);
+                    frc[rr][ch][e] = __builtin_amdgcn_fractf(t);
+                    ent[rr][ch][e] = T[(int)t];
+                }
+#pragma unroll
+        for (int rr = 0; rr < 2; rr++)
+#pragma unroll
+            for (int ch = 0; ch < 3; ch++)
+#pragma unroll
+                for (int e = 0; e < 2; e++) {
+                    float r;
+                    asm("v_fma_f32 %0, %1, %2, %3" : "=v"(r) : "v"(ent[rr][ch][e].y), "v"(frc[rr][ch][e]), "v"(ent[rr][ch][e].x));
+                    linc[rr][ch][e] = r;
+                }
+#pragma unroll
+        for (int rr = 0; rr < 2; rr++) {
+            const f2 *lin = linc[rr];
+            if constexpr (TAIL == TAILK_PQ_LUT) {
+#pragma unroll
+                for (int ch = 0; ch < 3; ch++) {
+                    const f2 g = fma_k<true>(GG, 3 * ch, lin[0], fma_k<false>(GG, 3 * ch + 1, lin[1], mul_k(GG, 3 * ch + 2, lin[2])));
+                    out[rr][ch] = f2{hlsl_pow(g.x, 1.0f / 2.2f), hlsl_pow(g.y, 1.0f / 2.2f)};
+                }
+            } else {
+                const f2 ys = splat(2000.0f) * pk_fma(splat(0.2627f), lin[0], pk_fma(splat(0.6780f), lin[1], splat(0.0593f) * lin[2]));
+                const float ks = P.lum_scale * (1.0f / 1000.0f);
+                const f2 gain = f2{hlsl_pow(ys.x, 0.2f) * ks, hlsl_pow(ys.y, 0.2f) * ks};
+                const float A_ = 0.15f, B_ = 0.50f, CB = 0.10f * 0.50f, DE = 0.20f * 0.02f, DF = 0.20f * 0.30f, EF = 0.02f / 0.30f;
+                const float inv_div = 1.0f / (((4.8f * (A_ * 4.8f + CB) + DE) / (4.8f * (A_ * 4.8f + B_) + DF)) - EF);
+                f2 tm[3];
+#pragma unroll
+                for (int ch = 0; ch < 3; ch++) {
+                    const f2 x = lin[ch] * gain;
+                    const f2 num = pk_fma(x, pk_fma(splat(A_), x, splat(CB)), splat(DE));
+                    const f2 den = pk_fma(x, pk_fma(splat(A_), x, splat(B_)), splat(DF));
+                    const f2 q = f2{num.x * __builtin_amdgcn_rcpf(den.x), num.y * __builtin_amdgcn_rcpf(den.y)};
+                    tm[ch] = (q - splat(EF)) * splat(inv_div);
+                }
+#pragma unroll
+                for (int ch = 0; ch < 3; ch++) {
+                    const f2 g = fma_k<true>(GG, 3 * ch, tm[0], fma_k<false>(GG, 3 * ch + 1, tm[1], mul_k(GG, 3 * ch + 2, tm[2])));
+                    out[rr][ch] = f2{hlsl_pow(g.x, 1.0f / 2.2f), hlsl_pow(g.y, 1.0f / 2.2f)};
+                }
+            }
+        }
+    }
+}
+
+template <int TAIL, int SRC, bool FIRST>
+__device__ __forceinline__ void convert_block_bp(const FusedArgs &P, const f2 (&MM)[5], const f2 (&GG)[5], const f2 (&CC)[3], const RawUnseenBp &u, ChromaCarry &keep,
+                                                 int sy0, int sy1, const f2 *T, f2 out[2][3])
+{
+    const int n4 = chroma_v4(P, sy0) & ~3;
+    const int fr0 = chroma_v4(P, sy0) - n4, fr1 = chroma_v4(P, sy1) - n4;
+    const f2 w1 = f2{quarter(fr0), quarter(fr1)}, w0 = f2{quarter(4 - fr0), quarter(4 - fr1)};
+    const ChromaCarry bot = chroma_floats<SRC>(u.v[2]);
+    ChromaCarry top = keep;
+    if constexpr (FIRST) top = chroma_floats<SRC>(u.v[3]);
+    keep = bot;
+    f2 Ucol[2], Vcol[2], Ycol[2];
+    Ucol[0] = pk_fma(splat(bot.u), w1, splat(top.u) * w0);
+    Vcol[0] = pk_fma(splat(bot.v), w1, splat(top.v) * w0);
+    const f2 Un = from_next_lane(Ucol[0]), Vn = from_next_lane(Vcol[0]);
+    if constexpr (SRC == SRC_P01X) {
+        Ycol[0] = f2{(float)(u.v[0] & 0xffffu), (float)(u.v[1] & 0xffffu)};
+        Ycol[1] = f2{(float)(u.v[0] >> 16), (float)(u.v[1] >> 16)};
+    } else {
+        Ycol[0] = f2{(float)(u.v[0] & 0xffu), (float)(u.v[1] & 0xffu)};
+        Ycol[1] = f2{(float)((u.v[0] >> 8) & 0xffu), (float)((u.v[1] >> 8) & 0xffu)};
+    }
+    const f2 cwa = splat(P.cw_own), cwb = splat(P.cw_next);
+    Ucol[1] = pk_fma(Un, cwb, Ucol[0] * cwa);
+    Vcol[1] = pk_fma(Vn, cwb, Vcol[0] * cwa);
+    convert_block_yuv_bp<TAIL>(P, MM, GG, CC, Ycol, Ucol, Vcol, T, out);
+}
+
+}
+
+}
diff --git a/videorenderer_amd/csrc/vp_fused_up2x_bp.hip b/videorenderer_amd/csrc/vp_fused_up2x_bp.hip
--- /dev/null
+++ b/videorenderer_amd/csrc/vp_fused_up2x_bp.hip
@@ -0,0 +1,45 @@
+#include "vp_fused_up2x_bp.h"
+
+#include "../../include/mpcvr.h"
+
+namespace mpcvr {
+
+bool FusedUp2xRowCarryHolds(int vk1, int vk2, int vk3, int rect_t, int H, int ch)
+{
+    if (H < 1 || ch < 1) return false;
+    int prev_a, prev_b;
+    FusedUp2xChromaRows(vk1, vk2, vk3, rect_t, H, ch, -3, &prev_a, &prev_b);
+    for (int a = -1; a <= H + 3; a += 2) {
+        int row_a, row_b;
+        FusedUp2xChromaRows(vk1, vk2, vk3, rect_t, H, ch, a, &row_a, &row_b);
+        if (row_a != prev_b) return false;
+        prev_b = row_b;
+    }
+    return true;
+}
+
+bool FusedUp2xBpTakes(const FusedArgs &a, int srck, int epik, int tailk)
+{
+    const bool planned = (srck == SRC_P01X && (epik == EPI_DITHER8 || epik == EPI_DIRECT8) && (tailk == TAILK_PQ_LUT || tailk == TAILK_HLG || tailk == TAILK_NONE)) ||
+                         (srck == SRC_NV12 && epik == EPI_DIRECT8 && tailk == TAILK_NONE);
+    if (!planned || a.exact_cv) return false;
+    if (a.sub422 || a.sub444 || a.packed422 || a.packed444 || a.gray || a.nearest || a.center_h || a.cw_own != 0.5f || a.cw_next != 0.5f) return false;
+    if (a.m[1] != 0.0f || a.m[8] != 0.0f) return false;
+    if ((a.W & 1) || (a.rect_l & 1) || a.W < 2) return false;
+    if (((a.rect_l + a.W - 2) >> 1) < a.cw - 1) return false;
+    if (a.rect_t & 1) return false;
+    return FusedUp2xRowCarryHolds(a.vk1, a.vk2, a.vk3, a.rect_t, a.H, a.ch);
+}
+
+int &FusedUp2xLastForm()
+{
+    static thread_local int form = -1;
+    return form;
+}
+
+}
+
+extern "C" int32_t mpcvr_plan_up2x_row_carry(int32_t vk1, int32_t vk2, int32_t vk3, int32_t rect_t, int32_t h, int32_t ch)
+{
+    return mpcvr::FusedUp2xRowCarryHolds(vk1, vk2, vk3, rect_t, h, ch) ? 1 : 0;
+}
diff --git a/videorenderer_amd/csrc/vp_fused_up2x_bp_launch.h b/videorenderer_amd/csrc/vp_fused_up2x_bp_launch.h
--- /dev/null
+++ b/videorenderer_amd/csrc/vp_fused_up2x_bp_launch.h
@@ -0,0 +1,40 @@
+#pragma once
+#include "vp_fused_up2x.h"
+
+namespace mpcvr {
+
+namespace {
+
+template <int NT, int TAIL, int SRC, int EPI>
+__global__ __launch_bounds__(256, MPCVR_UP2X_WAVES) void k_fused_up2x_bp(FusedArgs P, const FusedFrame *__restrict__ frames, const unsigned char *__restrict__ baked,
+                                                                         FrameTable32 tab)
+{
+    fused_up2x_body<NT, TAIL, SRC, EPI, XC_NEVER, 1>(P, frames, baked, tab);
+}
+
+}
+
+template <int NT>
+void LaunchFusedUp2xBpNT(const FusedArgs &a, dim3 grid, size_t lds, int tailk, int srck, int epik, const FusedFrame *frames_dev, const unsigned char *baked,
+                         const FrameTable32 &tab, hipStream_t s)
+{
+    const dim3 block(256, 1, 1);
+#define MPCVR_LAUNCH_BP(TK, SK, EK) hipLaunchKernelGGL((k_fused_up2x_bp<NT, TK, SK, EK>), grid, block, lds, s, a, frames_dev, baked, tab)
+#ifdef MPCVR_UP2X_BP_HEADLINE_ONLY
+    MPCVR_LAUNCH_BP(TAILK_PQ_LUT, SRC_P01X, EPI_DITHER8);
+#else
+    if (srck == SRC_NV12) MPCVR_LAUNCH_BP(TAILK_NONE, SRC_NV12, EPI_DIRECT8);
+    else if (epik == EPI_DITHER8) {
+        if (tailk == TAILK_PQ_LUT) MPCVR_LAUNCH_BP(TAILK_PQ_LUT, SRC_P01X, EPI_DITHER8);
+        else if (tailk == TAILK_HLG) MPCVR_LAUNCH_BP(TAILK_HLG, SRC_P01X, EPI_DITHER8);
+        else MPCVR_LAUNCH_BP(TAILK_NONE, SRC_P01X, EPI_DITHER8);
+    } else {
+        if (tailk == TAILK_PQ_LUT) MPCVR_LAUNCH_BP(TAILK_PQ_LUT, SRC_P01X, EPI_DIRECT8);
+        else if (tailk == TAILK_HLG) MPCVR_LAUNCH_BP(TAILK_HLG, SRC_P01X, EPI_DIRECT8);
+        else MPCVR_LAUNCH_BP(TAILK_NONE, SRC_P01X, EPI_DIRECT8);
+    }
+#endif
+#undef MPCVR_LAUNCH_BP
+}
+
+}
diff --git a/videorenderer_amd/csrc/vp_fused_up2x_bp_nt4.hip b/videorenderer_amd/csrc/vp_fused_up2x_bp_nt4.hip
--- /dev/null
+++ b/videorenderer_amd/csrc/vp_fused_up2x_bp_nt4.hip
@@ -0,0 +1,5 @@
+#include "vp_fused_up2x_bp_launch.h"
+
+namespace mpcvr {
+template void LaunchFusedUp2xBpNT<4>(const FusedArgs &, dim3, size_t, int, int, int, const FusedFrame *, const unsigned char *, const FrameTable32 &, hipStream_t);
+}
diff --git a/videorenderer_amd/csrc/vp_fused_up2x_bp_nt5.hip b/videorenderer_amd/csrc/vp_fused_up2x_bp_nt5.hip
--- /dev/null
+++ b/videorenderer_amd/csrc/vp_fused_up2x_bp_nt5.hip
@@ -0,0 +1,5 @@
+#include "vp_fused_up2x_bp_launch.h"
+
+namespace mpcvr {
+template void LaunchFusedUp2xBpNT<5>(const FusedArgs &, dim3, size_t, int, int, int, const FusedFrame *, const unsigned char *, const FrameTable32 &, hipStream_t);
+}
diff --git a/videorenderer_amd/csrc/vp_fused_up2x_bp_nt6.hip b/videorenderer_amd/csrc/vp_fused_up2x_bp_nt6.hip
--- /dev/null
+++ b/videorenderer_amd/csrc/vp_fused_up2x_bp_nt6.hip
@@ -0,0 +1,5 @@
+#include "vp_fused_up2x_bp_launch.h"
+
+namespace mpcvr {
+template void LaunchFusedUp2xBpNT<6>(const FusedArgs &, dim3, size_t, int, int, int, const FusedFrame *, const unsigned char *, const FrameTable32 &, hipStream_t);
+}
diff --git a/videorenderer_amd/csrc/vp_launch.h b/videorenderer_amd/csrc/vp_launch.h
--- a/videorenderer_amd/csrc/vp_launch.h
+++ b/videorenderer_amd/csrc/vp_launch.h
@@ -106,6 +106,7 @@
 inline int FusedUp2xByValueMax(const FusedParams &P) { return P.jinc_tab ? 0 : TableRows<FrameTable32>(); }
 hipError_t LaunchConvertBlocks(const FusedParams &P, const LaunchFrames &F, hipStream_t s, size_t batch_stride = 0);
 hipError_t LaunchFusedUp2x(const FusedParams &P, const LaunchFrames &F, hipStream_t s);
+int &FusedUp2xLastForm();
 
 struct FusedStripParams {
     FusedParams fp;
```

Measured after the change: 24280 (median of 6 runs). 1.02x the previous value.
